# heihachi78/NascarGymnasium

Measured on AMD Instinct MI355X. Metric: env-steps/sec (cars x envs), daytona 10-car, higher is better.
Workload: dtype f32+f64; 1 GPU; daytona 10-car: 8192 envs x 10 cars per GPU, on-device noisy rule driver (BaseController._fallback_control, 15% of car-steps uniform), closed loop, steady state after 10800 settle steps (env ages staggered over the 180 s episode), auto-reset; envs_per_gpu=8192, cars_per_env=10, policy=noisy, car_contact=off (reference), track=daytona.track, parallelism=dp1 (env shards, no collective)

## Files before the change

include/nascar.h:

```cpp
#ifndef NASCAR_H
#define NASCAR_H
#include <stdint.h>
#ifdef __cplusplus
extern "C" {
#endif

typedef struct NascarHandle NascarHandle;

typedef struct NascarConfig {
    int32_t num_envs;
    int32_t num_cars;
    int32_t reset_on_lap;
    int32_t device;
    double start_x, start_y, start_angle;
} NascarConfig;

int nascar_create(const NascarConfig* cfg, NascarHandle** out);
void nascar_destroy(NascarHandle* h);
const char* nascar_last_error(void);

int nascar_add_track(NascarHandle* h, const double* segments, int32_t nseg, double total_length,
                     const double* walls, int32_t nwall);
int nascar_set_track_cache(int32_t retain, const char* dir);
int nascar_prebuild_track(const double* segments, int32_t nseg, double total_length, const double* walls, int32_t nwall,
                          float beam_cell);

int nascar_set_env_tracks(NascarHandle* h, const int32_t* env_track);

int nascar_set_random_tracks(NascarHandle* h, const int32_t* tracks, int32_t ntracks, const uint64_t* seeds,
                             const int32_t* draws, void* stream);
int nascar_get_env_tracks(NascarHandle* h, int32_t* env_track, int32_t* draws, void* stream);
int nascar_track_draw(int32_t n, const uint64_t* seeds, const int32_t* k, const int32_t* current, const int32_t* tracks,
                      int32_t ntracks, int32_t* out);

int nascar_vec_post(NascarHandle* h, const float* reward, const uint8_t* env_flags, double* ep_ret, int64_t* ep_len,
                    uint8_t* done, double* snap_ret, int64_t* snap_len, void* stream);
int nascar_check_actions(NascarHandle* h, const void* actions, int32_t discrete, int32_t* bad, void* stream);

int nascar_reset(NascarHandle* h, const uint8_t* env_mask, float* obs, void* stream);

int nascar_step(NascarHandle* h, const void* actions, int32_t discrete, float* obs, float* reward,
                uint8_t* car_flags, uint8_t* env_flags, int32_t auto_reset, float* terminal_obs, void* stream);

int nascar_step_driven(NascarHandle* h, int32_t policy, uint64_t seed, int64_t step, float* obs, float* reward,
                       uint8_t* car_flags, uint8_t* env_flags, int32_t auto_reset, float* terminal_obs, void* stream);

#define NASCAR_TRAJ_RECORDS 1
#define NASCAR_TRAJ_OBS 2
int nascar_rollout(NascarHandle* h, int32_t policy, uint64_t seed, int64_t step0, int32_t steps, float* obs,
                   float* reward, uint8_t* car_flags, uint8_t* env_flags, int32_t auto_reset, int32_t traj, void* stream);

int nascar_set_rollout_streams(NascarHandle* h, int32_t streams);
int nascar_get_rollout_streams(NascarHandle* h);

int nascar_set_rollout_pipe(NascarHandle* h, int32_t sensor_workgroups);
int nascar_rollout_pipe_status(NascarHandle* h, void* stream);

int nascar_set_envs_per_block(NascarHandle* h, int32_t epb);
int nascar_get_envs_per_block(NascarHandle* h);

int nascar_set_sensor_lanes(NascarHandle* h, int32_t lanes);

int nascar_set_sensor_block(NascarHandle* h, int32_t threads);

int nascar_set_beam_cell(NascarHandle* h, float meters);

int nascar_set_fused_logic(NascarHandle* h, int32_t enable);
int nascar_get_fused_logic(NascarHandle* h);

int nascar_set_step_events(NascarHandle* h, void* const* events, int32_t n);

int nascar_get_info(NascarHandle* h, double* info, void* stream);

int nascar_set_car_contact(NascarHandle* h, int32_t enable);

int nascar_set_car_visibility(NascarHandle* h, int32_t enable);
int nascar_get_car_visibility(NascarHandle* h);

int nascar_set_perf_history(NascarHandle* h, int32_t enable, void* stream);

int64_t nascar_state_bytes(NascarHandle* h);
int nascar_get_state(NascarHandle* h, void* dst_device, void* stream);
int nascar_set_state(NascarHandle* h, const void* src_device, void* stream);

int nascar_policy_actions(NascarHandle* h, int32_t policy, uint64_t seed, int64_t step, const float* obs,
                          float* actions, void* stream);

int nascar_set_actor(NascarHandle* h, const float* w1, const float* b1, const float* w2, const float* b2,
                     const float* w3, const float* b3, int32_t obs_dim, int32_t hidden, int32_t act_dim);
int nascar_set_actor_precision(NascarHandle* h, int32_t fp32);
int nascar_actor_forward(NascarHandle* h, const float* obs, int32_t n, float* actions, void* stream);

typedef struct NascarMlp {
    int32_t obs_dim, h1, h2, act_dim;
    int32_t activation;
    int32_t output;
    const float *w1, *b1, *w2, *b2, *w3, *b3;
} NascarMlp;
#define NASCAR_CTRL_RULE (-1)
#define NASCAR_CTRL_UNIFORM (-2)
#define NASCAR_CTRL_NOISY (-3)
#define NASCAR_CTRL_GENOME (-4)
int nascar_check_controller(const NascarMlp* mlp);
int nascar_add_controller(NascarHandle* h, const NascarMlp* mlp);
int nascar_controller_forward(NascarHandle* h, int32_t id, const float* obs, int32_t n, float* actions, void* stream);
int nascar_set_car_controllers(NascarHandle* h, const int32_t* ctrl);
int nascar_update_controller(NascarHandle* h, int32_t id, const NascarMlp* mlp, void* stream);

int nascar_set_actor_critic(NascarHandle* h, int32_t pi_id, int32_t vf_id, const float* log_std);
int nascar_collect(NascarHandle* h, uint64_t seed, int64_t step0, int32_t steps, float* obs, float* reward,
                   uint8_t* car_flags, uint8_t* env_flags, float* actions, float* logp, float* values, float* timeout_values,
                   void* stream);
int nascar_gae(NascarHandle* h, const float* reward, const float* values, const float* timeout_values,
               const uint8_t* env_flags, int32_t steps, double gamma, double lambda, float* adv, float* ret, void* stream);

typedef struct NascarReplay {
    float *obs, *next_obs;
    float *actions;
    float *reward;
    uint8_t *done, *timeout, *live;
    int32_t capacity;
} NascarReplay;
int nascar_set_explorer(NascarHandle* h, int32_t id, const float* sigma);
int nascar_collect_transitions(NascarHandle* h, int32_t source, uint64_t seed, int64_t step0, int32_t steps, float* obs,
                               const NascarReplay* replay, int32_t pos, void* stream);
int nascar_replay_sample(NascarHandle* h, const NascarReplay* replay, int32_t size, uint64_t seed, int64_t draw,
                         int32_t batch, float* obs, float* next_obs, float* actions, float* reward, float* done,
                         uint8_t* live, void* stream);

int nascar_set_genomes(NascarHandle* h, const double* genomes, void* stream);

int nascar_set_fitness(NascarHandle* h, int32_t enable, void* stream);
int nascar_get_fitness(NascarHandle* h, double* out, void* stream);

int nascar_debug_sincosf(const float* x, float* s, float* c, int32_t n, void* stream);

int nascar_debug_f64math(const double* x, const double* y, double* out, int32_t n, int32_t fn, void* stream);

int nascar_debug_toi(const float* cases, int32_t n, float* beta, int32_t* state, int32_t* far, void* stream);
int nascar_debug_collide(const float* cases, int32_t n, float* out, void* stream);

int nascar_debug_car_contact(const float* bodies, int32_t num_envs, int32_t num_cars, float* out, int32_t* env_out,
                             void* stream);

int nascar_debug_sensors(NascarHandle* h, const float* poses, float* obs, int32_t impl, void* stream);

int nascar_debug_block_map(NascarHandle* h, int32_t* blk_track, int32_t* blk_env, int32_t cap_blocks, void* stream);

#ifdef __cplusplus
}
#endif
#endif
```

nascargymnasium_amd/_lib.py:

```python
import ctypes
import os
import subprocess

HERE = os.path.dirname(os.path.abspath(__file__))
LIB_PATH = os.environ.get("NASCAR_LIB") or os.path.join(HERE, "libnascar.so")
CSRC = os.path.join(HERE, "csrc")

INFO_FIELDS = ["x", "y", "vx", "vy", "angle", "omega", "speed", "lap_count", "last_lap_time", "best_lap_time",
               "is_timing", "current_lap_time", "total_distance_traveled", "has_crossed_startline", "disabled",
               "cumulative_reward", "cumulative_impact_force", "on_track", "engine_rpm", "simulation_time",
               "n_contacts", "error", "track_progress", "perf_count", "perf_max_speed", "perf_first_fast"]
N_INFO = len(INFO_FIELDS)
INFO_INDEX = {f: i for i, f in enumerate(INFO_FIELDS)}
OBS_DIM = 38

CF_DISABLED, CF_JUST_DISABLED, CF_COLLISION, CF_LAP, CF_ERROR = 1, 2, 4, 8, 128
EF_TERMINATED, EF_TRUNCATED, EF_RESET = 1, 2, 8
TRAJ_RECORDS, TRAJ_OBS = 1, 2
REASONS = {0: None, 1: "all_cars_disabled", 2: "all_active_cars_low_reward (threshold: -250.0)",
           3: "time_limit", 4: "truncated"}

HIPCC_FLAGS = ["--offload-arch=gfx950", "-O3", "-ffp-contract=off", "-fno-fast-math", "-fno-slp-vectorize", "-fPIC",
               "-shared", "-std=c++17", "-Wno-unused-value", "-Wno-unused-result"]


class NascarMlp(ctypes.Structure):
    _fields_ = [(n, ctypes.c_int32) for n in ("obs_dim", "h1", "h2", "act_dim", "activation", "output")] + \
               [(n, ctypes.POINTER(ctypes.c_float)) for n in ("w1", "b1", "w2", "b2", "w3", "b3")]


CTRL_BUILTIN = {"rule": -1, "uniform": -2, "noisy": -3, "genome": -4}
FITNESS_FIELDS = ["total_reward", "distance_traveled", "max_speed", "time_on_track", "lap_completed", "lap_time",
                  "steps", "disabled_at_step"]
N_FITNESS = len(FITNESS_FIELDS)
N_GENES = 12


class NascarReplay(ctypes.Structure):
    _fields_ = [(n, ctypes.c_void_p) for n in ("obs", "next_obs", "actions", "reward", "done", "timeout", "live")] + \
               [("capacity", ctypes.c_int32)]


class NascarConfig(ctypes.Structure):
    _fields_ = [("num_envs", ctypes.c_int32), ("num_cars", ctypes.c_int32), ("reset_on_lap", ctypes.c_int32),
                ("device", ctypes.c_int32), ("start_x", ctypes.c_double), ("start_y", ctypes.c_double),
                ("start_angle", ctypes.c_double)]


def build(verbose=False):
    src = os.path.join(CSRC, "nascar_kernels.hip")
    cmd = ["hipcc"] + HIPCC_FLAGS + ["-o", LIB_PATH, src]
    r = subprocess.run(cmd, capture_output=True, text=True)
    if r.returncode != 0:
        raise RuntimeError("hipcc failed:\n" + r.stderr[-4000:])
    if verbose:
        print(" ".join(cmd))
    return LIB_PATH


_lib = None


def lib():
    global _lib
    if _lib is not None:
        return _lib
    if not os.path.exists(LIB_PATH):
        raise RuntimeError(f"{LIB_PATH} is missing: run `python -c 'import __graft_entry__ as g; g.build()'` "
                           "(there is no CPU fallback for the product path)")
    L = ctypes.CDLL(LIB_PATH)
    vp, i32, i64, u64 = ctypes.c_void_p, ctypes.c_int32, ctypes.c_int64, ctypes.c_uint64
    d_p = ctypes.POINTER(ctypes.c_double)
    L.nascar_create.argtypes = [ctypes.POINTER(NascarConfig), ctypes.POINTER(vp)]
    L.nascar_create.restype = ctypes.c_int
    L.nascar_destroy.argtypes = [vp]
    L.nascar_destroy.restype = None
    L.nascar_last_error.restype = ctypes.c_char_p
    L.nascar_add_track.argtypes = [vp, d_p, i32, ctypes.c_double, d_p, i32]
    L.nascar_add_track.restype = ctypes.c_int
    L.nascar_set_env_tracks.argtypes = [vp, ctypes.POINTER(i32)]
    L.nascar_set_env_tracks.restype = ctypes.c_int
    L.nascar_reset.argtypes = [vp, vp, vp, vp]
    L.nascar_reset.restype = ctypes.c_int
    L.nascar_step.argtypes = [vp, vp, i32, vp, vp, vp, vp, i32, vp, vp]
    L.nascar_step.restype = ctypes.c_int
    L.nascar_step_driven.argtypes = [vp, i32, u64, i64, vp, vp, vp, vp, i32, vp, vp]
    L.nascar_step_driven.restype = ctypes.c_int
    L.nascar_rollout.argtypes = [vp, i32, u64, i64, i32, vp, vp, vp, vp, i32, i32, vp]
    L.nascar_rollout.restype = ctypes.c_int
    L.nascar_set_car_contact.argtypes = [vp, i32]
    L.nascar_set_car_contact.restype = ctypes.c_int
    L.nascar_set_car_visibility.argtypes = [vp, i32]
    L.nascar_set_car_visibility.restype = ctypes.c_int
    L.nascar_get_car_visibility.argtypes = [vp]
    L.nascar_get_car_visibility.restype = ctypes.c_int
    L.nascar_set_rollout_streams.argtypes = [vp, i32]
    L.nascar_set_rollout_streams.restype = ctypes.c_int
    L.nascar_get_rollout_streams.argtypes = [vp]
    L.nascar_get_rollout_streams.restype = ctypes.c_int
    L.nascar_set_rollout_pipe.argtypes = [vp, i32]
    L.nascar_set_rollout_pipe.restype = ctypes.c_int
    L.nascar_rollout_pipe_status.argtypes = [vp, vp]
    L.nascar_rollout_pipe_status.restype = ctypes.c_int
    L.nascar_set_envs_per_block.argtypes = [vp, i32]
    L.nascar_set_envs_per_block.restype = ctypes.c_int
    L.nascar_get_envs_per_block.argtypes = [vp]
    L.nascar_get_envs_per_block.restype = ctypes.c_int
    L.nascar_set_sensor_lanes.argtypes = [vp, i32]
    L.nascar_set_sensor_lanes.restype = ctypes.c_int
    L.nascar_set_sensor_block.argtypes = [vp, i32]
    L.nascar_set_sensor_block.restype = ctypes.c_int
    L.nascar_set_beam_cell.argtypes = [vp, ctypes.c_float]
    L.nascar_set_beam_cell.restype = ctypes.c_int
    L.nascar_set_fused_logic.argtypes = [vp, i32]
    L.nascar_set_fused_logic.restype = ctypes.c_int
    L.nascar_get_fused_logic.argtypes = [vp]
    L.nascar_get_fused_logic.restype = ctypes.c_int
    L.nascar_set_perf_history.argtypes = [vp, i32, vp]
    L.nascar_set_perf_history.restype = ctypes.c_int
    L.nascar_get_info.argtypes = [vp, vp, vp]
    L.nascar_get_info.restype = ctypes.c_int
    L.nascar_state_bytes.argtypes = [vp]
    L.nascar_state_bytes.restype = i64
    L.nascar_get_state.argtypes = [vp, vp, vp]
    L.nascar_get_state.restype = ctypes.c_int
    L.nascar_set_state.argtypes = [vp, vp, vp]
    L.nascar_set_state.restype = ctypes.c_int
    L.nascar_policy_actions.argtypes = [vp, i32, u64, i64, vp, vp, vp]
    L.nascar_policy_actions.restype = ctypes.c_int
    fp = ctypes.POINTER(ctypes.c_float)
    L.nascar_set_actor.argtypes = [vp, fp, fp, fp, fp, fp, fp, i32, i32, i32]
    L.nascar_set_actor.restype = ctypes.c_int
    L.nascar_set_actor_precision.argtypes = [vp, i32]
    L.nascar_set_actor_precision.restype = ctypes.c_int
    L.nascar_actor_forward.argtypes = [vp, vp, i32, vp, vp]
    L.nascar_actor_forward.restype = ctypes.c_int
    L.nascar_check_controller.argtypes = [ctypes.POINTER(NascarMlp)]
    L.nascar_check_controller.restype = ctypes.c_int
    L.nascar_add_controller.argtypes = [vp, ctypes.POINTER(NascarMlp)]
    L.nascar_add_controller.restype = ctypes.c_int
    L.nascar_controller_forward.argtypes = [vp, i32, vp, i32, vp, vp]
    L.nascar_controller_forward.restype = ctypes.c_int
    L.nascar_set_car_controllers.argtypes = [vp, ctypes.POINTER(i32)]
    L.nascar_set_car_controllers.restype = ctypes.c_int
    L.nascar_update_controller.argtypes = [vp, i32, ctypes.POINTER(NascarMlp), vp]
    L.nascar_update_controller.restype = ctypes.c_int
    L.nascar_set_actor_critic.argtypes = [vp, i32, i32, fp]
    L.nascar_set_actor_critic.restype = ctypes.c_int
    L.nascar_collect.argtypes = [vp, u64, i64, i32, vp, vp, vp, vp, vp, vp, vp, vp, vp]
    L.nascar_collect.restype = ctypes.c_int
    L.nascar_gae.argtypes = [vp, vp, vp, vp, vp, i32, ctypes.c_double, ctypes.c_double, vp, vp, vp]
    L.nascar_gae.restype = ctypes.c_int
    L.nascar_set_explorer.argtypes = [vp, i32, fp]
    L.nascar_set_explorer.restype = ctypes.c_int
    L.nascar_collect_transitions.argtypes = [vp, i32, u64, i64, i32, vp, ctypes.POINTER(NascarReplay), i32, vp]
    L.nascar_collect_transitions.restype = ctypes.c_int
    L.nascar_replay_sample.argtypes = [vp, ctypes.POINTER(NascarReplay), i32, u64, i64, i32, vp, vp, vp, vp, vp, vp, vp]
    L.nascar_replay_sample.restype = ctypes.c_int
    L.nascar_set_genomes.argtypes = [vp, d_p, vp]
    L.nascar_set_genomes.restype = ctypes.c_int
    L.nascar_set_fitness.argtypes = [vp, i32, vp]
    L.nascar_set_fitness.restype = ctypes.c_int
    L.nascar_get_fitness.argtypes = [vp, vp, vp]
    L.nascar_get_fitness.restype = ctypes.c_int
    L.nascar_set_step_events.argtypes = [vp, ctypes.POINTER(vp), i32]
    L.nascar_set_step_events.restype = ctypes.c_int
    L.nascar_debug_sincosf.argtypes = [vp, vp, vp, i32, vp]
    L.nascar_debug_sincosf.restype = ctypes.c_int
    L.nascar_debug_f64math.argtypes = [vp, vp, vp, i32, i32, vp]
    L.nascar_debug_f64math.restype = ctypes.c_int
    L.nascar_debug_toi.argtypes = [vp, i32, vp, vp, vp, vp]
    L.nascar_debug_toi.restype = ctypes.c_int
    L.nascar_debug_collide.argtypes = [vp, i32, vp, vp]
    L.nascar_debug_collide.restype = ctypes.c_int
    L.nascar_debug_car_contact.argtypes = [vp, i32, i32, vp, vp, vp]
    L.nascar_debug_car_contact.restype = ctypes.c_int
    L.nascar_debug_sensors.argtypes = [vp, vp, vp, i32, vp]
    L.nascar_debug_sensors.restype = ctypes.c_int
    i32p, u64p = ctypes.POINTER(i32), ctypes.POINTER(u64)
    L.nascar_track_draw.argtypes = [i32, u64p, i32p, i32p, i32p, i32, i32p]
    L.nascar_track_draw.restype = ctypes.c_int
    L.nascar_set_random_tracks.argtypes = [vp, i32p, i32, u64p, i32p, vp]
    L.nascar_set_random_tracks.restype = ctypes.c_int
    L.nascar_get_env_tracks.argtypes = [vp, vp, vp, vp]
    L.nascar_get_env_tracks.restype = ctypes.c_int
    L.nascar_vec_post.argtypes = [vp, vp, vp, vp, vp, vp, vp, vp, vp]
    L.nascar_vec_post.restype = ctypes.c_int
    L.nascar_check_actions.argtypes = [vp, vp, i32, vp, vp]
    L.nascar_check_actions.restype = ctypes.c_int
    L.nascar_set_track_cache.argtypes = [i32, ctypes.c_char_p]
    L.nascar_set_track_cache.restype = ctypes.c_int
    L.nascar_prebuild_track.argtypes = [d_p, i32, ctypes.c_double, d_p, i32, ctypes.c_float]
    L.nascar_prebuild_track.restype = ctypes.c_int
    L.nascar_debug_block_map.argtypes = [vp, vp, vp, i32, vp]
    L.nascar_debug_block_map.restype = ctypes.c_int
    _lib = L
    set_track_cache(int(os.environ.get("NASCAR_TRACK_RETAIN", "8")), os.environ.get("NASCAR_TRACK_CACHE", ""))
    return L


EXPORTED = ["nascar_create", "nascar_destroy", "nascar_last_error", "nascar_add_track", "nascar_set_env_tracks",
            "nascar_reset", "nascar_step", "nascar_step_driven", "nascar_rollout", "nascar_get_info", "nascar_set_perf_history", "nascar_set_car_contact", "nascar_set_car_visibility", "nascar_get_car_visibility", "nascar_set_rollout_streams", "nascar_get_rollout_streams", "nascar_set_rollout_pipe", "nascar_rollout_pipe_status", "nascar_set_envs_per_block", "nascar_get_envs_per_block", "nascar_set_sensor_lanes", "nascar_set_sensor_block", "nascar_set_beam_cell", "nascar_set_fused_logic", "nascar_get_fused_logic", "nascar_state_bytes", "nascar_get_state",
            "nascar_set_state", "nascar_policy_actions", "nascar_set_step_events", "nascar_set_actor", "nascar_set_actor_precision", "nascar_actor_forward",
            "nascar_check_controller", "nascar_add_controller", "nascar_controller_forward", "nascar_set_car_controllers",
            "nascar_set_genomes", "nascar_set_fitness", "nascar_get_fitness",
            "nascar_update_controller", "nascar_set_actor_critic", "nascar_collect", "nascar_gae",
            "nascar_set_explorer", "nascar_collect_transitions", "nascar_replay_sample",
            "nascar_debug_sincosf", "nascar_debug_f64math", "nascar_debug_toi", "nascar_debug_collide", "nascar_debug_car_contact", "nascar_debug_sensors", "nascar_track_draw", "nascar_set_random_tracks",
            "nascar_get_env_tracks", "nascar_vec_post", "nascar_check_actions", "nascar_set_track_cache",
            "nascar_prebuild_track", "nascar_debug_block_map"]


def check(rc):
    if rc < 0:
        raise RuntimeError("libnascar: " + lib().nascar_last_error().decode())
    return rc


def mlp_struct(ctrl, output=None):
    import numpy as np
    arrs = [np.ascontiguousarray(a, np.float32) for a in ctrl.arrays]
    fp = ctypes.POINTER(ctypes.c_float)
    m = NascarMlp(38, int(ctrl.h1), int(ctrl.h2), int(arrs[4].shape[0]), int(ctrl.activation),
                  int(ctrl.output if output is None else output), *[a.ctypes.data_as(fp) for a in arrs])
    return m, arrs


def check_controller(ctrl):
    m, _keep = mlp_struct(ctrl)
    check(lib().nascar_check_controller(ctypes.byref(m)))


def track_draw(seeds, k, current, tracks):
    import numpy as np
    seeds = np.ascontiguousarray(seeds, np.uint64).ravel()
    n = seeds.size
    k = np.ascontiguousarray(np.broadcast_to(np.asarray(k, np.int32), (n,)))
    cur = np.ascontiguousarray(np.broadcast_to(np.asarray(current, np.int32), (n,)))
    tr = np.ascontiguousarray(tracks, np.int32)
    out = np.empty(n, np.int32)
    i32p, u64p = ctypes.POINTER(ctypes.c_int32), ctypes.POINTER(ctypes.c_uint64)
    check(lib().nascar_track_draw(n, seeds.ctypes.data_as(u64p), k.ctypes.data_as(i32p), cur.ctypes.data_as(i32p),
                                  tr.ctypes.data_as(i32p), tr.size, out.ctypes.data_as(i32p)))
    return out


def set_track_cache(retain=8, directory=""):
    check(lib().nascar_set_track_cache(int(retain), (directory or "").encode()))


def prebuild_track(path, beam_cell=1.0):
    import numpy as np
    from .track import build_walls, load_track, track_path
    t = load_track(track_path(path))
    seg = np.ascontiguousarray(t.segment_table())
    walls = np.ascontiguousarray(build_walls(t)[:, :4])
    dp = ctypes.POINTER(ctypes.c_double)
    return bool(check(lib().nascar_prebuild_track(seg.ctypes.data_as(dp), seg.shape[0], float(t.total_length),
                                                  walls.ctypes.data_as(dp), walls.shape[0], float(beam_cell))))
```

nascargymnasium_amd/csrc/nascar_car_io.h:

```cpp
#pragma once
#include "nascar_params.h"

enum {
  G_BODY = 1,
  G_IMP = 2,
  G_MODEL = 4,
  G_BANK = 8,
  G_TYRES = 16,
  G_ACC = 32,
  G_DIS = 64,
  G_LOGIC = 128,
  G_ALL = 255
};
#define CAR_F32_TABLE(X) \
  X(F32, cx, c.c.x, G_BODY) X(F32, cy, c.c.y, G_BODY) X(F32, a, c.a, G_BODY) \
  X(F32, vx, c.v.x, G_BODY) X(F32, vy, c.v.y, G_BODY) X(F32, w, c.w, G_BODY) \
  X(F32, qs, c.xf.q.s, G_BODY) X(F32, qc, c.xf.q.c, G_BODY) X(F32, xpx, c.xf.p.x, G_BODY) X(F32, xpy, c.xf.p.y, G_BODY) \
  X(F32, sleep, c.sleep, G_BODY) X(F32, invdt0, c.invdt0, G_BODY) \
  X(F32, flox, c.fat.lo.x, G_BODY) X(F32, floy, c.fat.lo.y, G_BODY) X(F32, fhix, c.fat.hi.x, G_BODY) X(F32, fhiy, c.fat.hi.y, G_BODY) \
  X(F32, cum_reward, c.cum_reward, G_LOGIC) X(F32, cum_reward_info, c.cum_reward_info, G_LOGIC)
#define CAR_F64_TABLE(X) \
  X(F64, rpm, c.rpm, G_MODEL) X(F64, pvx, c.pvx, G_MODEL) X(F64, pvy, c.pvy, G_MODEL) \
  X(F64, lfm, c.lfm, G_MODEL) X(F64, slip, c.slip, G_MODEL) X(F64, bank, c.bank, G_BANK) \
  X(F64, load0, c.load[0], G_TYRES) X(F64, load1, c.load[1], G_TYRES) X(F64, load2, c.load[2], G_TYRES) X(F64, load3, c.load[3], G_TYRES) \
  X(F64, temp0, c.temp[0], G_TYRES) X(F64, temp1, c.temp[1], G_TYRES) X(F64, temp2, c.temp[2], G_TYRES) X(F64, temp3, c.temp[3], G_TYRES) \
  X(F64, wear0, c.wear[0], G_TYRES) X(F64, wear1, c.wear[1], G_TYRES) X(F64, wear2, c.wear[2], G_TYRES) X(F64, wear3, c.wear[3], G_TYRES) \
  X(F64, imp, c.imp, G_IMP) \
  X(F64, lt_start, c.lt_start, G_LOGIC) X(F64, lt_cur, c.lt_cur, G_LOGIC) X(F64, lt_last, c.lt_last, G_LOGIC) \
  X(F64, lt_best, c.lt_best, G_LOGIC) X(F64, lt_px, c.lt_px, G_LOGIC) X(F64, lt_py, c.lt_py, G_LOGIC) X(F64, lt_dist, c.lt_dist, G_LOGIC) \
  X(F64, cum_impact, c.cum_impact, G_LOGIC) X(F64, stuck_dur, c.stuck_dur, G_LOGIC) \
  X(F64, stuck_sx, c.stuck_sx, G_LOGIC) X(F64, stuck_sy, c.stuck_sy, G_LOGIC) \
  X(F64, prev_px, c.prev_px, G_LOGIC) X(F64, prev_py, c.prev_py, G_LOGIC) \
  X(F64, prog_hist, c.prog_hist, G_LOGIC) X(F64, back, c.back, G_LOGIC) X(F64, prev_back, c.prev_back, G_LOGIC) \
  X(F64, imp_at_obs, c.imp_at_obs, G_LOGIC)
#define CAR_I32_TABLE(X) \
  X(I32, awake, c.awake, G_BODY) X(I32, nct, c.nct, G_BODY) X(I32, overflow, c.overflow, G_BODY) \
  X(I32, acc_len, c.acc_len, G_ACC) X(I32, acc_head, c.acc_head, G_ACC) \
  X(I32, imp_present, c.imp_present, G_IMP) X(I32, nact, c.nact, G_BODY) \
  X(I32, lt_timing, c.lt_timing, G_LOGIC) X(I32, lt_has_last, c.lt_has_last, G_LOGIC) X(I32, lt_has_best, c.lt_has_best, G_LOGIC) \
  X(I32, lt_crossed, c.lt_crossed, G_LOGIC) X(I32, lt_has_pos, c.lt_has_pos, G_LOGIC) X(I32, lt_laps, c.lt_laps, G_LOGIC) \
  X(I32, disabled, c.disabled, G_DIS) X(I32, has_stuck_start, c.has_stuck_start, G_LOGIC) \
  X(I32, first_step, c.first_step, G_LOGIC) X(I32, prev_laps, c.prev_laps, G_LOGIC)

#define CAR_ROW_ENUM(T, f, m, g) CAR_ROW_##T##_##f,
#define CAR_ROW_CHECK(T, f, m, g) \
  static_assert((int)CAR_ROW_##T##_##f == (int)T##_##f, "car field table: row " #f " is not at its nascar_layout.h index");
enum { CAR_F32_TABLE(CAR_ROW_ENUM) CAR_ROWS_F32 };
enum { CAR_F64_TABLE(CAR_ROW_ENUM) CAR_ROWS_F64 };
enum { CAR_I32_TABLE(CAR_ROW_ENUM) CAR_ROWS_I32 };
CAR_F32_TABLE(CAR_ROW_CHECK) CAR_F64_TABLE(CAR_ROW_CHECK) CAR_I32_TABLE(CAR_ROW_CHECK)
static_assert((int)CAR_ROWS_F32 == (int)N_F32 && (int)CAR_ROWS_F64 == (int)N_F64 && (int)CAR_ROWS_I32 == (int)N_I32,
              "car field table: row count differs from nascar_layout.h");

template <int MASK>
__device__ __forceinline__ void car_load_groups(const Params& P, int n, Car& c) {
#define CAR_ROW_LOAD(T, f, m, g) if (MASK & (g)) m = T##P(P, f)[n];
  CAR_F32_TABLE(CAR_ROW_LOAD) CAR_F64_TABLE(CAR_ROW_LOAD) CAR_I32_TABLE(CAR_ROW_LOAD)
#undef CAR_ROW_LOAD
}
template <int MASK>
__device__ __forceinline__ void car_store_groups(const Params& P, int n, const Car& c) {
#define CAR_ROW_STORE(T, f, m, g) if (MASK & (g)) T##P(P, f)[n] = m;
  CAR_F32_TABLE(CAR_ROW_STORE) CAR_F64_TABLE(CAR_ROW_STORE) CAR_I32_TABLE(CAR_ROW_STORE)
#undef CAR_ROW_STORE
}
__device__ __forceinline__ void car_init_step(const Params& P, int n, Car& c) {
  c.just_disabled = 0;
  c.force = zero2(); c.torque = 0.0f; c.c0 = c.c; c.a0 = c.a; c.alpha0 = 0.0f; c.moved = 0;
  c.ct = P.ct + (size_t)n * MAXC; c.act_key = P.act_key + (size_t)n * MAXC; c.act_n = P.act_n + (size_t)n * MAXC * 2;
  c.acc = nullptr;
}

__device__ inline void car_load(const Params& P, int n, Car& c) { car_load_groups<G_ALL>(P, n, c); car_init_step(P, n, c); }
__device__ inline void car_store(const Params& P, int n, const Car& c) { car_store_groups<G_ALL>(P, n, c); }

__device__ inline void car_load_phys(const Params& P, int n, Car& c) {
  car_load_groups<G_BODY | G_IMP | G_MODEL | G_BANK | G_TYRES | G_ACC | G_DIS>(P, n, c);
  car_init_step(P, n, c);
}
__device__ inline void car_store_model(const Params& P, int n, const Car& c) { car_store_groups<G_MODEL | G_TYRES | G_ACC>(P, n, c); }
__device__ inline void car_reload_tyres(const Params& P, int n, Car& c) { car_load_groups<G_TYRES>(P, n, c); }
__device__ inline void car_load_logic(const Params& P, int n, Car& c) { car_load_groups<G_LOGIC>(P, n, c); }

__device__ inline void car_store_body(const Params& P, int n, const Car& c) { car_store_groups<G_BODY | G_IMP>(P, n, c); }
__device__ inline void car_load_body(const Params& P, int n, Car& c) {
  car_load_groups<G_BODY | G_IMP | G_DIS>(P, n, c);
  car_init_step(P, n, c);
}
__device__ inline void car_store_logic(const Params& P, int n, const Car& c) {
  car_store_groups<G_LOGIC | G_BANK | G_IMP | G_DIS>(P, n, c);
}
```

nascargymnasium_amd/csrc/nascar_device.h:

```cpp
#pragma once
#include "nascar_math.h"
#include "nascar_layout.h"

#pragma clang fp contract(off)

#define BLOCK 256
#define SBLOCK 128

#ifdef NASCAR_PROFILE
__device__ unsigned long long* g_prof = nullptr;
__shared__ int s_prof_b0;
#define PROF_B0(v) (s_prof_b0 = (v))
#define PROF_BLK ((size_t)((blockIdx.x + (unsigned)s_prof_b0) & 16383u))
#define PROF(ph) do { unsigned long long _t = __builtin_amdgcn_s_memtime(); \
    if (g_prof && (threadIdx.x & 63) == 0) g_prof[(PROF_BLK * (BLOCK / 64) + threadIdx.x / 64) * 16 + (ph)] = _t; } while (0)
#define PROFS(ph) do { unsigned long long _t = __builtin_amdgcn_s_memtime(); \
    if (g_prof && (threadIdx.x & 63) == 0) g_prof[(65536 + PROF_BLK * (BLOCK / 64) + threadIdx.x / 64) * 16 + (ph)] = _t; } while (0)
#define PROFR(ph) do { unsigned long long _t = __builtin_amdgcn_s_memtime(); \
    if (g_prof && (threadIdx.x & 63) == 0) g_prof[(65536 + PROF_BLK * (blockDim.x >> 6) + threadIdx.x / 64) * 16 + (ph)] = _t; } while (0)
#define PROF_XCC(ph) do { const unsigned long long _x = (__builtin_amdgcn_s_getreg((3 << 11) | 20) & 15) + 1; \
    if (g_prof && (threadIdx.x & 63) == 0) g_prof[(PROF_BLK * (BLOCK / 64) + threadIdx.x / 64) * 16 + (ph)] = _x; } while (0)
#define PROFR_XCC(ph) do { const unsigned long long _x = (__builtin_amdgcn_s_getreg((3 << 11) | 20) & 15) + 1; \
    if (g_prof && (threadIdx.x & 63) == 0) g_prof[(65536 + PROF_BLK * (blockDim.x >> 6) + threadIdx.x / 64) * 16 + (ph)] = _x; } while (0)
#define PROFR_RT(ph) do { unsigned long long _t = __builtin_amdgcn_s_memrealtime(); \
// ... 65 lines not shown
#define MAX_TRANSLATION 2.0f
#define MAX_ROTATION (0.5f * B2_PI)
#define BAUMGARTE 0.2f
#define TOI_BAUMGARTE 0.75f
#define MAX_LINEAR_CORRECTION 0.2f
#define VELOCITY_THRESHOLD 1.0f
#define TIME_TO_SLEEP 0.5f
#define LINEAR_SLEEP_TOL 0.01f
#define ANGULAR_SLEEP_TOL (2.0f / 180.0f * B2_PI)
#define MAX_SUBSTEPS 8
#define MAX_TOI_CONTACTS 32
#define FLT_EPS 1.1920928955078125e-07f
#define FLT_BIG 3.402823466e+38f

#define CAR_HX ((float)(5.042 / 2.0))
#define CAR_HY ((float)(1.996 / 2.0))
#define CAR_INV_MASS (1.0f / 1500.0f)
#define CAR_I_F ((float)(1500.0 * (5.042 * 5.042 + 1.996 * 1.996) * 0.5 / 12.0))
#define CAR_INV_I (1.0f / CAR_I_F)
#define MIX_RESTITUTION 0.25f

#define CAR_MASS 1500.0
#define GRAVITY_MS2 9.81
#define CAR_WHEELBASE 2.794
#define CAR_MAX_TORQUE 820.0
#define CAR_MAX_POWER (670.0 * 745.7)
#define CAR_MAX_SPEED_MS (200.0 * 0.44704)
#define DRAG_CONSTANT (0.5 * 1.225 * 0.38 * 2.5)
#define ROLLING_RESISTANCE_FORCE (0.015 * CAR_MASS * GRAVITY_MS2)
#define MAX_TYRE_LOAD (CAR_MASS * GRAVITY_MS2 * 2.0)
#define STATIC_LOAD_PER_TYRE (CAR_MASS * GRAVITY_MS2 / 4.0)
#define PI_D 3.141592653589793
#define RAD_PER_DEG (PI_D / 180.0)
#define DEG_PER_RAD (180.0 / PI_D)

typedef unsigned int gu4 __attribute__((ext_vector_type(4)));
typedef unsigned int gu2 __attribute__((ext_vector_type(2)));
template <typename T> __device__ __forceinline__ T ldg(const T* p) {
  if constexpr (sizeof(T) % 16 == 0) {
    T r;
    const __attribute__((address_space(1))) gu4* q = (const __attribute__((address_space(1))) gu4*)p;
#pragma unroll
    for (int i = 0; i < (int)(sizeof(T) / 16); ++i) { const gu4 v = q[i]; __builtin_memcpy((char*)&r + 16 * i, &v, 16); }
    return r;
  } else if constexpr (sizeof(T) % 8 == 0) {
    T r;
    const __attribute__((address_space(1))) gu2* q = (const __attribute__((address_space(1))) gu2*)p;
#pragma unroll
    for (int i = 0; i < (int)(sizeof(T) / 8); ++i) { const gu2 v = q[i]; __builtin_memcpy((char*)&r + 8 * i, &v, 8); }
    return r;
  } else {
    return *(const __attribute__((address_space(1))) T*)p;
  }
}

struct V2 { float x, y; };
struct Rot { float s, c; };
struct Xf { V2 p; Rot q; };
struct Aabb { V2 lo, hi; };

__device__ __forceinline__ V2 V(float x, float y) { V2 r; r.x = x; r.y = y; return r; }
__device__ __forceinline__ V2 vadd(V2 a, V2 b) { return V(a.x + b.x, a.y + b.y); }
__device__ __forceinline__ V2 vsub(V2 a, V2 b) { return V(a.x - b.x, a.y - b.y); }
__device__ __forceinline__ V2 vmul(float s, V2 a) { return V(s * a.x, s * a.y); }
__device__ __forceinline__ V2 vneg(V2 a) { return V(-a.x, -a.y); }
__device__ __forceinline__ float vdot(V2 a, V2 b) { return a.x * b.x + a.y * b.y; }
__device__ __forceinline__ float vcross(V2 a, V2 b) { return a.x * b.y - a.y * b.x; }
__device__ __forceinline__ V2 vcross_vs(V2 a, float s) { return V(s * a.y, -s * a.x); }
__device__ __forceinline__ V2 vcross_sv(float s, V2 a) { return V(-s * a.y, s * a.x); }
__device__ __forceinline__ float vlen(V2 a) { return fsqrt_cr(a.x * a.x + a.y * a.y); }
__device__ __forceinline__ float vnormalize(V2* a) {
  float length = vlen(*a);
  if (length < FLT_EPS) return 0.0f;
  float inv = fdiv_cr(1.0f, length);
  a->x *= inv; a->y *= inv;
  return length;
}
__device__ __forceinline__ V2 rmul(Rot q, V2 v) { return V(q.c * v.x - q.s * v.y, q.s * v.x + q.c * v.y); }
__device__ __forceinline__ V2 rmulT(Rot q, V2 v) { return V(q.c * v.x + q.s * v.y, -q.s * v.x + q.c * v.y); }
__device__ __forceinline__ V2 xmul(Xf T, V2 v) {
  return V((T.q.c * v.x - T.q.s * v.y) + T.p.x, (T.q.s * v.x + T.q.c * v.y) + T.p.y);
}
__device__ __forceinline__ V2 xmulT(Xf T, V2 v) {
  float px = v.x - T.p.x, py = v.y - T.p.y;
  return V(T.q.c * px + T.q.s * py, -T.q.s * px + T.q.c * py);
}
__device__ __forceinline__ Xf xmulT_xx(Xf A, Xf B) {
  Xf C;
  C.q.s = A.q.c * B.q.s - A.q.s * B.q.c;
  C.q.c = A.q.c * B.q.c + A.q.s * B.q.s;
  C.p = rmulT(A.q, vsub(B.p, A.p));
  return C;
}
__device__ __forceinline__ float fminb(float a, float b) { return a < b ? a : b; }
__device__ __forceinline__ float fmaxb(float a, float b) { return a > b ? a : b; }
__device__ __forceinline__ float fclamp(float a, float lo, float hi) { return fmaxb(lo, fminb(a, hi)); }
__device__ __forceinline__ V2 vmin(V2 a, V2 b) { return V(fminb(a.x, b.x), fminb(a.y, b.y)); }
__device__ __forceinline__ V2 vmax(V2 a, V2 b) { return V(fmaxb(a.x, b.x), fmaxb(a.y, b.y)); }
__device__ __forceinline__ Rot rot_set(float a) { Rot q; glibc_sincosf(a, &q.s, &q.c); return q; }
__device__ __forceinline__ V2 zero2() { return V(0.0f, 0.0f); }

struct Poly { float hx, hy, radius; };
__device__ __forceinline__ void make_box(Poly* p, float hx, float hy) { p->hx = hx; p->hy = hy; p->radius = POLY_RADIUS; }
__device__ __forceinline__ float with_sign(float m, uint32_t neg) { return __uint_as_float(__float_as_uint(m) | (neg << 31)); }
__device__ __forceinline__ V2 pv(const Poly* p, int i) {
  const uint32_t u = (uint32_t)i;
  return V(with_sign(p->hx, (((u + 1u) >> 1) & 1u) ^ 1u), with_sign(p->hy, ((u >> 1) & 1u) ^ 1u));
}
__device__ __forceinline__ V2 pn(const Poly* p, int i) {
  const uint32_t u = (uint32_t)i, odd = u & 1u, hi = (u >> 1) & 1u;
  return V(with_sign((float)odd, hi & odd), with_sign((float)(odd ^ 1u), (hi ^ 1u) & (odd ^ 1u)));
}
__device__ __forceinline__ Aabb poly_aabb(const Poly* p, Xf xf) {
  V2 lower = xmul(xf, pv(p, 0)), upper = lower;
#pragma unroll
  for (int i = 1; i < 4; ++i) { V2 v = xmul(xf, pv(p, i)); lower = vmin(lower, v); upper = vmax(upper, v); }
  V2 r = V(p->radius, p->radius);
  Aabb a; a.lo = vsub(lower, r); a.hi = vadd(upper, r);
  return a;
}
__device__ __forceinline__ bool overlap(Aabb a, Aabb b) {
  V2 d1 = vsub(b.lo, a.hi), d2 = vsub(a.lo, b.hi);
  if (d1.x > 0.0f || d1.y > 0.0f) return false;
  if (d2.x > 0.0f || d2.y > 0.0f) return false;
  return true;
}
__device__ __forceinline__ bool contains(Aabb a, Aabb b) {
  bool r = true;
  r = r && a.lo.x <= b.lo.x; r = r && a.lo.y <= b.lo.y;
  r = r && b.hi.x <= a.hi.x; r = r && b.hi.y <= a.hi.y;
  return r;
}

struct LWall {
  float px, py, qs, qc;
  float hx, hy, ang;
  int key;
};
__device__ __forceinline__ Xf wall_xf(const LWall& w) { Xf t; t.p = V(w.px, w.py); t.q.s = w.qs; t.q.c = w.qc; return t; }
__device__ __forceinline__ Aabb fat_box(float4 f) { Aabb a; a.lo = V(f.x, f.y); a.hi = V(f.z, f.w); return a; }

struct WallGrid {
  float ox, oy, inv_cell, reach;
  int nx, ny;
  const int* start;
  const uint16_t* idx;
  const float4* box;
};
#define BP_BATCH 4
struct WallSet {
  const LWall* W; int nw;
  WallGrid bp, sn;
  const float4* fat;
  DContact* ct_all = nullptr;
};

__device__ __forceinline__ bool grid_list(const WallGrid& g, float x, float y, int& beg, int& end) {
  if (!g.start) return false;
  const float fx = (x - g.ox) * g.inv_cell, fy = (y - g.oy) * g.inv_cell;
  if (!(fx >= 0.0f && fy >= 0.0f && fx < (float)g.nx && fy < (float)g.ny)) return false;
  const int cell = (int)fy * g.nx + (int)fx;
  beg = ldg(g.start + cell); end = ldg(g.start + cell + 1);
  return true;
}

struct Car {
  V2 c; float a; V2 v; float w; Xf xf; float sleep; int awake;
  V2 force; float torque; V2 c0; float a0; float alpha0;
  Aabb fat; int moved; float invdt0;
  int nct, overflow;
  int pid;
  double thr_in, brk_in, str_in, thr, brk, steer;
  double rpm, pvx, pvy, lfm, slip, bank;
  double load[4], temp[4], wear[4], fric[4];
  int acc_len, acc_head;
  int imp_present, nact; double imp;
  int lt_timing, lt_has_last, lt_has_best, lt_crossed, lt_has_pos, lt_laps;
  double lt_start, lt_cur, lt_last, lt_best, lt_px, lt_py, lt_dist;
  int disabled, just_disabled, has_stuck_start, first_step, prev_laps;
  double cum_impact, stuck_dur, stuck_sx, stuck_sy, prev_px, prev_py, prog_hist, back, prev_back, imp_at_obs;
  float cum_reward, cum_reward_info;
  DContact* ct;
  int ct_hw;
  int* act_key;
  float* act_n;
  double* acc;
};

#ifndef CT_LDS_CAP
#define CT_LDS_CAP 4
#endif
__device__ __forceinline__ bool ct_in_lds(const Car& c) {
  return __builtin_amdgcn_is_shared((const __attribute__((address_space(0))) void*)c.ct);
}
__device__ __forceinline__ void ct_make_room(Car& c, const WallSet& S) {
  if (S.ct_all && ct_in_lds(c)) {
    if (c.nct >= CT_LDS_CAP) {
      DContact* g = S.ct_all + (size_t)c.pid * MAXC;
      const int nrec = max(c.nct, c.ct_hw);
      for (int i = 0; i < nrec; ++i) g[i] = c.ct[i];
      c.ct = g;
    } else {
      c.ct_hw = max(c.ct_hw, c.nct + 1);
    }
  }
}

__device__ inline void lis_begin(Car& c, int key, V2 n) {
  int found = -1;
  for (int i = 0; i < c.nact; ++i) if (c.act_key[i] == key) { found = i; break; }
  if (found >= 0) { c.act_n[found * 2] = n.x; c.act_n[found * 2 + 1] = n.y; }
  else if (c.nact < MAXC) { c.act_key[c.nact] = key; c.act_n[c.nact * 2] = n.x; c.act_n[c.nact * 2 + 1] = n.y; c.nact++; }
  if (!c.imp_present) { c.imp_present = 1; c.imp = 0.0; }
}
__device__ inline void lis_end(Car& c, int key) {
  for (int i = 0; i < c.nact; ++i) if (c.act_key[i] == key) {
    for (int j = i; j < c.nact - 1; ++j) { c.act_key[j] = c.act_key[j + 1]; c.act_n[j * 2] = c.act_n[j * 2 + 2]; c.act_n[j * 2 + 1] = c.act_n[j * 2 + 3]; }
    c.nact--; break;
  }
  if (c.nact == 0) { c.imp_present = 1; c.imp = 0.0; }
}
__device__ inline void lis_post(Car& c, int count, float n0, float n1) {
  if (count <= 0) return;
  double total = 0.0;
  total += (double)n0;
  if (count > 1) total += (double)n1;
  if (c.imp_present) c.imp = pymax(c.imp, total);
}

__device__ __forceinline__ void set_awake(Car& c) { if (!c.awake) { c.awake = 1; c.sleep = 0.0f; } }
__device__ __forceinline__ void sync_transform(Car& c) { c.xf.q = rot_set(c.a); c.xf.p = vsub(c.c, rmul(c.xf.q, zero2())); }
__device__ __forceinline__ void apply_force(Car& c, V2 f, V2 point) {
  set_awake(c); c.force = vadd(c.force, f); c.torque += vcross(vsub(point, c.c), f);
}
__device__ __forceinline__ void apply_force_center(Car& c, V2 f) { set_awake(c); c.force = vadd(c.force, f); }
__device__ __forceinline__ void apply_torque(Car& c, float t) { set_awake(c); c.torque += t; }

__device__ __forceinline__ void move_proxy(Car& c, Xf xf1, Xf xf2) {
  Poly cp; make_box(&cp, CAR_HX, CAR_HY);
  Aabb a1 = poly_aabb(&cp, xf1), a2 = poly_aabb(&cp, xf2), aabb;
  aabb.lo = vmin(a1.lo, a2.lo); aabb.hi = vmax(a1.hi, a2.hi);
  V2 disp = vsub(xf2.p, xf1.p);
  if (contains(c.fat, aabb)) return;
  Aabb b = aabb; V2 r = V(AABB_EXT, AABB_EXT);
  b.lo = vsub(b.lo, r); b.hi = vadd(b.hi, r);
  V2 d = vmul(AABB_MULT, disp);
  if (d.x < 0.0f) b.lo.x += d.x; else b.hi.x += d.x;
  if (d.y < 0.0f) b.lo.y += d.y; else b.hi.y += d.y;
  c.fat = b; c.moved = 1;
}
__device__ __forceinline__ void sync_fixtures(Car& c) {
  Xf xf1; xf1.q = rot_set(c.a0); xf1.p = vsub(c.c0, rmul(xf1.q, zero2()));
  move_proxy(c, xf1, c.xf);
}

__device__ inline void add_pair(Car& c, const WallSet& S, int j) {
    bool exists = false;
    for (int i = 0; i < c.nct; ++i) if (c.ct[i].wall == j) { exists = true; break; }
    if (exists) return;
    if (c.nct >= MAXC) { c.overflow = 1; return; }
    ct_make_room(c, S);
    for (int i = c.nct; i > 0; --i) c.ct[i] = c.ct[i - 1];
    DContact z;
    z.wall = j; z.flags = CT_ENABLED; z.mtype = 0; z.pointCount = 0;
    z.lnx = z.lny = z.lpx = z.lpy = 0.0f;
    for (int q = 0; q < 2; ++q) { z.pt[q].lx = z.pt[q].ly = z.pt[q].ni = z.pt[q].ti = 0.0f; z.pt[q].id = 0u; }
    z.toi = 1.0f; z.toiCount = 0;
    c.ct[0] = z;
    c.nct++;
    set_awake(c);
}
__device__ inline void find_new_contacts(Car& c, const WallSet& S) {
  if (!c.moved) return;
  c.moved = 0;
  const LWall* W = S.W;
  int beg = 0, end = S.nw;
  const uint16_t* list = nullptr;
  {
    const float hx = 0.5f * (c.fat.hi.x - c.fat.lo.x), hy = 0.5f * (c.fat.hi.y - c.fat.lo.y);
    const float cx = 0.5f * (c.fat.hi.x + c.fat.lo.x), cy = 0.5f * (c.fat.hi.y + c.fat.lo.y);
    if (hx <= S.bp.reach - 0.05f && hy <= S.bp.reach - 0.05f && grid_list(S.bp, cx, cy, beg, end)) list = S.bp.idx;
    else { beg = 0; end = S.nw; CCOUNT(c, 8, 1); }
  }
  if (list && S.bp.box) {
    const float4* __restrict__ box = S.bp.box;
    for (int k = beg; k < end; k += BP_BATCH) {
      float4 b[BP_BATCH];
#pragma unroll
      for (int u = 0; u < BP_BATCH; ++u) b[u] = ldg(box + k + u);
#pragma unroll
      for (int u = 0; u < BP_BATCH; ++u) {
        if (k + u >= end) break;
        Aabb a; a.lo = V(b[u].x, b[u].y); a.hi = V(b[u].z, b[u].w);
        if (overlap(c.fat, a)) add_pair(c, S, (int)ldg(list + k + u));
      }
    }
    return;
  }
  for (int k = beg; k < end; ++k) {
    const int j = list ? (int)ldg(list + k) : k;
    if (!overlap(c.fat, fat_box(ldg(S.fat + j)))) continue;
    bool exists = false;
    for (int i = 0; i < c.nct; ++i) if (c.ct[i].wall == j) { exists = true; break; }
    if (exists) continue;
    if (c.nct >= MAXC) { c.overflow = 1; continue; }
    ct_make_room(c, S);
    for (int i = c.nct; i > 0; --i) c.ct[i] = c.ct[i - 1];
    DContact z;
    z.wall = j; z.flags = CT_ENABLED; z.mtype = 0; z.pointCount = 0;
    z.lnx = z.lny = z.lpx = z.lpy = 0.0f;
    for (int q = 0; q < 2; ++q) { z.pt[q].lx = z.pt[q].ly = z.pt[q].ni = z.pt[q].ti = 0.0f; z.pt[q].id = 0u; }
    z.toi = 1.0f; z.toiCount = 0;
    c.ct[0] = z;
    c.nct++;
    set_awake(c);
  }
}
__device__ inline void remove_contact(Car& c, int i) {
  for (int j = i; j < c.nct - 1; ++j) c.ct[j] = c.ct[j + 1];
  c.nct--;
}

struct Clip { V2 v; uint32_t id; };
__device__ __forceinline__ uint32_t cf_key(int ia, int ib, int ta, int tb) {
  return (uint32_t)(ia & 255) | ((uint32_t)(ib & 255) << 8) | ((uint32_t)(ta & 255) << 16) | ((uint32_t)(tb & 255) << 24);
}
__device__ inline float find_max_separation(int* edgeIndex, const Poly* p1, Xf xf1, const Poly* p2, Xf xf2) {
  Xf xf = xmulT_xx(xf2, xf1);
  int best = 0; float maxSep = -FLT_BIG;
  for (int i = 0; i < 4; ++i) {
    V2 n = rmul(xf.q, pn(p1, i));
    V2 v1 = xmul(xf, pv(p1, i));
    float si = FLT_BIG;
    for (int j = 0; j < 4; ++j) { float sij = vdot(n, vsub(pv(p2, j), v1)); if (sij < si) si = sij; }
    if (si > maxSep) { maxSep = si; best = i; }
  }
  *edgeIndex = best;
  return maxSep;
}
__device__ inline void find_incident_edge(Clip& c0, Clip& c1, const Poly* p1, Xf xf1, int edge1, const Poly* p2, Xf xf2) {
  V2 normal1 = rmulT(xf2.q, rmul(xf1.q, pn(p1, edge1)));
  int index = 0; float minDot = FLT_BIG;
  for (int i = 0; i < 4; ++i) { float d = vdot(normal1, pn(p2, i)); if (d < minDot) { minDot = d; index = i; } }
  int i1 = index, i2 = i1 + 1 < 4 ? i1 + 1 : 0;
  c0.v = xmul(xf2, pv(p2, i1)); c0.id = cf_key(edge1, i1, 1, 0);
  c1.v = xmul(xf2, pv(p2, i2)); c1.id = cf_key(edge1, i2, 1, 0);
}
__device__ inline int clip_segment(Clip& o0, Clip& o1, const Clip& i0, const Clip& i1, V2 normal, float offset, int vertexIndexA) {
  int numOut = 0;
  float d0 = vdot(normal, i0.v) - offset;
  float d1 = vdot(normal, i1.v) - offset;
  if (d0 <= 0.0f) { o0 = i0; numOut = 1; }
  if (d1 <= 0.0f) { if (numOut == 0) o0 = i1; else o1 = i1; ++numOut; }
  if (d0 * d1 < 0.0f) {
    float interp = fdiv_cr(d0, d0 - d1);
    Clip cv;
    cv.v = vadd(i0.v, vmul(interp, vsub(i1.v, i0.v)));
    cv.id = cf_key(vertexIndexA, (int)((i0.id >> 8) & 255), 0, 1);
    if (numOut == 0) o0 = cv; else o1 = cv;
    ++numOut;
  }
  return numOut;
}
__device__ inline void collide_polygons(DContact& m, const Poly* pA, Xf xfA, const Poly* pB, Xf xfB) {
  m.pointCount = 0;
  float totalRadius = pA->radius + pB->radius;
  int edgeA = 0; float sepA = find_max_separation(&edgeA, pA, xfA, pB, xfB);
  if (sepA > totalRadius) return;
  int edgeB = 0; float sepB = find_max_separation(&edgeB, pB, xfB, pA, xfA);
  if (sepB > totalRadius) return;
  const Poly *poly1, *poly2; Xf xf1, xf2; int edge1; int flip;
  const float k_tol = 0.1f * LINEAR_SLOP;
  if (sepB > sepA + k_tol) { poly1 = pB; poly2 = pA; xf1 = xfB; xf2 = xfA; edge1 = edgeB; m.mtype = 2; flip = 1; }
  else { poly1 = pA; poly2 = pB; xf1 = xfA; xf2 = xfB; edge1 = edgeA; m.mtype = 1; flip = 0; }
  Clip inc0, inc1;
  find_incident_edge(inc0, inc1, poly1, xf1, edge1, poly2, xf2);
  int iv1 = edge1, iv2 = edge1 + 1 < 4 ? edge1 + 1 : 0;
  V2 v11 = pv(poly1, iv1), v12 = pv(poly1, iv2);
  V2 localTangent = vsub(v12, v11);
  vnormalize(&localTangent);
  V2 localNormal = vcross_vs(localTangent, 1.0f);
  V2 planePoint = vmul(0.5f, vadd(v11, v12));
  V2 tangent = rmul(xf1.q, localTangent);
  V2 normal = vcross_vs(tangent, 1.0f);
  v11 = xmul(xf1, v11); v12 = xmul(xf1, v12);
  float frontOffset = vdot(normal, v11);
  float sideOffset1 = -vdot(tangent, v11) + totalRadius;
  float sideOffset2 = vdot(tangent, v12) + totalRadius;
  Clip a0, a1, b0, b1;
  int np = clip_segment(a0, a1, inc0, inc1, vneg(tangent), sideOffset1, iv1);
  if (np < 2) return;
  np = clip_segment(b0, b1, a0, a1, tangent, sideOffset2, iv2);
  if (np < 2) return;
  m.lnx = localNormal.x; m.lny = localNormal.y; m.lpx = planePoint.x; m.lpy = planePoint.y;
  int pc = 0;
#pragma unroll
  for (int i = 0; i < 2; ++i) {
    const Clip& cq = i == 0 ? b0 : b1;
    float separation = vdot(normal, cq.v) - frontOffset;
    if (separation <= totalRadius) {
      V2 lp = xmulT(xf2, cq.v);
      uint32_t id = cq.id;
      if (flip) {
        uint32_t ia = id & 255, ib = (id >> 8) & 255, ta = (id >> 16) & 255, tb = (id >> 24) & 255;
        id = cf_key((int)ib, (int)ia, (int)tb, (int)ta);
      }
      DPoint q; q.lx = lp.x; q.ly = lp.y; q.id = id; q.ni = 0.0f; q.ti = 0.0f;
      if (pc == 0) m.pt[0] = q; else m.pt[1] = q;
      ++pc;
    }
  }
  m.pointCount = pc;
}

__device__ inline void world_manifold(const DContact& m, Xf xfA, Xf xfB, V2* normal, V2 pts[2]) {
  const float rA = POLY_RADIUS, rB = POLY_RADIUS;
  if (m.pointCount == 0) return;
  V2 ln = V(m.lnx, m.lny), lp = V(m.lpx, m.lpy);
  if (m.mtype == 1) {
    V2 n = rmul(xfA.q, ln), planePoint = xmul(xfA, lp);
#pragma unroll
    for (int i = 0; i < 2; ++i) {
      if (i >= m.pointCount) break;
      V2 clipPoint = xmul(xfB, V(m.pt[i].lx, m.pt[i].ly));
      V2 cA = vadd(clipPoint, vmul(rA - vdot(vsub(clipPoint, planePoint), n), n));
      V2 cB = vsub(clipPoint, vmul(rB, n));
      pts[i] = vmul(0.5f, vadd(cA, cB));
    }
    *normal = n;
  } else {
    V2 n = rmul(xfB.q, ln), planePoint = xmul(xfB, lp);
#pragma unroll
    for (int i = 0; i < 2; ++i) {
      if (i >= m.pointCount) break;
      V2 clipPoint = xmul(xfA, V(m.pt[i].lx, m.pt[i].ly));
      V2 cB = vadd(clipPoint, vmul(rB - vdot(vsub(clipPoint, planePoint), n), n));
      V2 cA = vsub(clipPoint, vmul(rA, n));
      pts[i] = vmul(0.5f, vadd(cA, cB));
    }
    *normal = vneg(n);
  }
}

__device__ inline void contact_update(Car& c, int ci, const LWall* W) {
  PCOUNT(14, 1); CCOUNT(c, 5, 1);
  DContact ct = c.ct[ci];
  const DContact old = ct;
  ct.flags |= CT_ENABLED;
  bool was = (ct.flags & CT_TOUCH) != 0;
  Poly pa, pb; make_box(&pa, CAR_HX, CAR_HY);
  const LWall wl = ldg(W + ct.wall);
  make_box(&pb, wl.hx, wl.hy);
  Xf xfB = wall_xf(wl);
  collide_polygons(ct, &pa, c.xf, &pb, xfB);
  bool touching = ct.pointCount > 0;
#pragma unroll
  for (int i = 0; i < 2; ++i) {
    if (i >= ct.pointCount) break;
    ct.pt[i].ni = 0.0f; ct.pt[i].ti = 0.0f;
    if (old.pointCount > 0 && old.pt[0].id == ct.pt[i].id) { ct.pt[i].ni = old.pt[0].ni; ct.pt[i].ti = old.pt[0].ti; }
    else if (old.pointCount > 1 && old.pt[1].id == ct.pt[i].id) { ct.pt[i].ni = old.pt[1].ni; ct.pt[i].ti = old.pt[1].ti; }
  }
  if (touching != was) set_awake(c);
  if (touching) ct.flags |= CT_TOUCH; else ct.flags &= ~CT_TOUCH;
  c.ct[ci] = ct;
  if (!was && touching) {
    V2 n = zero2(), pts[2];
    world_manifold(ct, c.xf, xfB, &n, pts);
    lis_begin(c, wl.key, n);
  }
  if (was && !touching) lis_end(c, wl.key);
}

struct ManiRes { float4 a, b, c; };
#define MANI_UNSET 0x7fc0deadu
__device__ inline ManiRes contact_manifold(Xf xfA, const LWall& wl) {
  Poly pa, pb; make_box(&pa, CAR_HX, CAR_HY); make_box(&pb, wl.hx, wl.hy);
  DContact m;
  m.mtype = -1; m.lnx = __uint_as_float(MANI_UNSET); m.pointCount = 0;
  m.lny = m.lpx = m.lpy = 0.0f;
  for (int q = 0; q < 2; ++q) { m.pt[q].lx = m.pt[q].ly = 0.0f; m.pt[q].id = 0u; }
  collide_polygons(m, &pa, xfA, &pb, wall_xf(wl));
  const int stage = __float_as_uint(m.lnx) != MANI_UNSET ? 2 : (m.mtype >= 0 ? 1 : 0);
  ManiRes r;
  r.a = make_float4(__int_as_float(stage | (m.pointCount << 2) | ((m.mtype & 3) << 4)), m.lnx, m.lny, m.lpx);
  r.b = make_float4(m.lpy, m.pt[0].lx, m.pt[0].ly, __uint_as_float(m.pt[0].id));
  r.c = make_float4(m.pt[1].lx, m.pt[1].ly, __uint_as_float(m.pt[1].id), 0.0f);
  return r;
}
__device__ inline void contact_apply(Car& c, int ci, const LWall* W, const ManiRes& r) {
  PCOUNT(14, 1); CCOUNT(c, 5, 1);
  DContact ct = c.ct[ci];
  const DContact old = ct;
  ct.flags |= CT_ENABLED;
  bool was = (ct.flags & CT_TOUCH) != 0;
  const int h = __float_as_int(r.a.x), stage = h & 3, pc = (h >> 2) & 3;
  ct.pointCount = 0;
  if (stage >= 1) ct.mtype = (h >> 4) & 3;
  if (stage == 2) {
    ct.lnx = r.a.y; ct.lny = r.a.z; ct.lpx = r.a.w; ct.lpy = r.b.x;
    if (pc > 0) { ct.pt[0].lx = r.b.y; ct.pt[0].ly = r.b.z; ct.pt[0].id = __float_as_uint(r.b.w); ct.pt[0].ni = 0.0f; ct.pt[0].ti = 0.0f; }
    if (pc > 1) { ct.pt[1].lx = r.c.x; ct.pt[1].ly = r.c.y; ct.pt[1].id = __float_as_uint(r.c.z); ct.pt[1].ni = 0.0f; ct.pt[1].ti = 0.0f; }
    ct.pointCount = pc;
  }
  bool touching = ct.pointCount > 0;
#pragma unroll
  for (int i = 0; i < 2; ++i) {
    if (i >= ct.pointCount) break;
    ct.pt[i].ni = 0.0f; ct.pt[i].ti = 0.0f;
    if (old.pointCount > 0 && old.pt[0].id == ct.pt[i].id) { ct.pt[i].ni = old.pt[0].ni; ct.pt[i].ti = old.pt[0].ti; }
    else if (old.pointCount > 1 && old.pt[1].id == ct.pt[i].id) { ct.pt[i].ni = old.pt[1].ni; ct.pt[i].ti = old.pt[1].ti; }
  }
  if (touching != was) set_awake(c);
  if (touching) ct.flags |= CT_TOUCH; else ct.flags &= ~CT_TOUCH;
  c.ct[ci] = ct;
  if (!was && touching) {
    const LWall wl = ldg(W + ct.wall);
    V2 n = zero2(), pts[2];
    world_manifold(ct, c.xf, wall_xf(wl), &n, pts);
    lis_begin(c, wl.key, n);
  }
  if (was && !touching) lis_end(c, ldg(&W[ct.wall].key));
}

#ifndef TOI_JOBCAP
#define TOI_JOBCAP 64
#endif
struct ToiWaveLDS { float4 sw0[64], sw1[64]; int2 job[TOI_JOBCAP]; float res[TOI_JOBCAP]; };
#ifndef MANI_JOBCAP
#define MANI_JOBCAP 32
#endif
struct ManiWaveLDS { float4 xf[64]; int2 job[MANI_JOBCAP]; ManiRes res[MANI_JOBCAP]; };
struct VCP { V2 rA, rB; float ni, ti, nm, tm, vb; };
struct VC {
  VCP p[2]; V2 normal; float nm[4]; float K[4]; int pointCount;
  V2 cB; float aB; V2 vB; float wB;
  V2 ln, lp, lps[2]; int pcount, type, ci;
  Rot qB; uint32_t aB0;
};
struct IslandWaveLDS { VC vc[MAX_ISLAND]; };
union WaveLDS { ToiWaveLDS toi; ManiWaveLDS mani; IslandWaveLDS island; float4 floor[160]; };
static_assert(sizeof(IslandWaveLDS) <= sizeof(ToiWaveLDS), "the island area must not grow the wave's LDS work area");
__shared__ WaveLDS g_wave_lds[SBLOCK / 64];
__device__ __forceinline__ void wave_lds_sync() {
  __builtin_amdgcn_fence(__ATOMIC_RELEASE, "wavefront");
  __builtin_amdgcn_wave_barrier();
  __builtin_amdgcn_fence(__ATOMIC_ACQUIRE, "wavefront");
}
__device__ __forceinline__ int popc64(unsigned long long x) { return __popcll(x); }
__device__ __forceinline__ int rank_in(unsigned long long m) {
  const unsigned long long below = __lane_id() == 0 ? 0ull : (~0ull >> (64 - __lane_id()));
  return popc64(m & below);
}

__device__ inline void collide(Car& c, const WallSet& S) {
  const LWall* W = S.W;
  int i = 0;
  while (i < c.nct) {
    if (!c.awake) { ++i; continue; }
    const int wall = c.ct[i].wall;
    if (!overlap(c.fat, fat_box(ldg(S.fat + wall)))) {
      bool touching = (c.ct[i].flags & CT_TOUCH) != 0;
      remove_contact(c, i);
      if (touching) lis_end(c, ldg(&W[wall].key));
      continue;
    }
    contact_update(c, i, W);
    ++i;
  }
}

__device__ __forceinline__ Rot rot_static(float a, uint32_t a0bits, Rot q0) {
  return __float_as_uint(a) == a0bits ? q0 : rot_set(a);
}
struct BodyState { V2 c; float a; V2 v; float w; };
#define UNROLL_SMALL NMAX <= 2 ? NMAX : 1
#define SOLVER_ITER_LOOP _Pragma("unroll 1")

template <int NMAX> __device__ __forceinline__ void cs_init(VC* vc, int n, const Car& c, const int* cidx, const LWall* W, bool warm, float dtRatio) {
#pragma unroll UNROLL_SMALL
  for (int i = 0; i < NMAX; ++i) {
    if (i >= n) break;
    const DContact& ct = c.ct[cidx[i]];
    VC& v = vc[i];
    v.ci = cidx[i];
    v.pointCount = ct.pointCount;
    const LWall wl = ldg(W + ct.wall);
    v.cB = V(wl.px, wl.py); v.aB = wl.ang; v.vB = zero2(); v.wB = 0.0f;
    v.qB.s = wl.qs; v.qB.c = wl.qc; v.aB0 = __float_as_uint(wl.ang);
    v.ln = V(ct.lnx, ct.lny); v.lp = V(ct.lpx, ct.lpy); v.pcount = ct.pointCount; v.type = ct.mtype;
    v.K[0] = v.K[1] = v.K[2] = v.K[3] = 0.0f; v.nm[0] = v.nm[1] = v.nm[2] = v.nm[3] = 0.0f;
    for (int j = 0; j < 2; ++j) {
      v.p[j].ni = v.p[j].ti = 0.0f;
      v.p[j].rA = v.p[j].rB = zero2(); v.p[j].nm = v.p[j].tm = v.p[j].vb = 0.0f;
      v.lps[j] = zero2();
    }
    for (int j = 0; j < 2; ++j) {
      if (j >= ct.pointCount) break;
      if (warm) { v.p[j].ni = dtRatio * ct.pt[j].ni; v.p[j].ti = dtRatio * ct.pt[j].ti; }
      v.lps[j] = V(ct.pt[j].lx, ct.pt[j].ly);
    }
  }
}

template <int NMAX> __device__ __forceinline__ void cs_init_velocity(VC* vc, int n, const Car& c, const BodyState& A) {
  const float mA = CAR_INV_MASS, iA = CAR_INV_I, mB = 0.0f, iB = 0.0f;
  const float friction_unused = 0.0f; (void)friction_unused;
  const Rot qA = rot_set(A.a);
#pragma unroll UNROLL_SMALL
  for (int i = 0; i < NMAX; ++i) {
    if (i >= n) break;
    VC& v = vc[i];
    const DContact& m = c.ct[v.ci];
    V2 cA = A.c; float aA = A.a; V2 vA = A.v; float wA = A.w;
    V2 cB = v.cB; float aB = v.aB; V2 vB = v.vB; float wB = v.wB;
    Xf xfA, xfB;
    xfA.q = qA; xfB.q = rot_static(aB, v.aB0, v.qB);
    xfA.p = vsub(cA, rmul(xfA.q, zero2()));
    xfB.p = vsub(cB, rmul(xfB.q, zero2()));
    V2 normal = zero2(), pts[2];
    world_manifold(m, xfA, xfB, &normal, pts);
    v.normal = normal;
    for (int j = 0; j < 2; ++j) {
      if (j >= v.pointCount) break;
      VCP& p = v.p[j];
      p.rA = vsub(pts[j], cA); p.rB = vsub(pts[j], cB);
      float rnA = vcross(p.rA, v.normal), rnB = vcross(p.rB, v.normal);
      float kNormal = mA + mB + iA * rnA * rnA + iB * rnB * rnB;
      p.nm = kNormal > 0.0f ? fdiv_cr(1.0f, kNormal) : 0.0f;
      V2 tangent = vcross_vs(v.normal, 1.0f);
      float rtA = vcross(p.rA, tangent), rtB = vcross(p.rB, tangent);
      float kTangent = mA + mB + iA * rtA * rtA + iB * rtB * rtB;
      p.tm = kTangent > 0.0f ? fdiv_cr(1.0f, kTangent) : 0.0f;
      p.vb = 0.0f;
      float vRel = vdot(v.normal, vsub(vsub(vadd(vB, vcross_sv(wB, p.rB)), vA), vcross_sv(wA, p.rA)));
      if (vRel < -VELOCITY_THRESHOLD) p.vb = -MIX_RESTITUTION * vRel;
    }
    if (v.pointCount == 2) {
      VCP& p1 = v.p[0]; VCP& p2 = v.p[1];
      float rn1A = vcross(p1.rA, v.normal), rn1B = vcross(p1.rB, v.normal);
      float rn2A = vcross(p2.rA, v.normal), rn2B = vcross(p2.rB, v.normal);
      float k11 = mA + mB + iA * rn1A * rn1A + iB * rn1B * rn1B;
      float k22 = mA + mB + iA * rn2A * rn2A + iB * rn2B * rn2B;
      float k12 = mA + mB + iA * rn1A * rn2A + iB * rn1B * rn2B;
      if (k11 * k11 < 1000.0f * (k11 * k22 - k12 * k12)) {
        v.K[0] = k11; v.K[1] = k12; v.K[2] = k12; v.K[3] = k22;
        float a = v.K[0], b = v.K[2], cc = v.K[1], d = v.K[3];
        float det = a * d - b * cc;
        if (det != 0.0f) det = fdiv_cr(1.0f, det);
        v.nm[0] = det * d; v.nm[2] = -det * b; v.nm[1] = -det * cc; v.nm[3] = det * a;
      } else {
        v.pointCount = 1;
      }
    }
  }
}

template <int NMAX> __device__ __forceinline__ void cs_warm_start(VC* vc, int n, BodyState& A) {
  const float mA = CAR_INV_MASS, iA = CAR_INV_I, mB = 0.0f, iB = 0.0f;
#pragma unroll UNROLL_SMALL
  for (int i = 0; i < NMAX; ++i) {
    if (i >= n) break;
    VC& v = vc[i];
    V2 vA = A.v; float wA = A.w; V2 vB = v.vB; float wB = v.wB;
    V2 normal = v.normal, tangent = vcross_vs(normal, 1.0f);
    for (int j = 0; j < 2; ++j) {
      if (j >= v.pointCount) break;
      VCP& p = v.p[j];
      V2 P = vadd(vmul(p.ni, normal), vmul(p.ti, tangent));
      wA -= iA * vcross(p.rA, P);
      vA = vsub(vA, vmul(mA, P));
      wB += iB * vcross(p.rB, P);
      vB = vadd(vB, vmul(mB, P));
    }
    A.v = vA; A.w = wA; v.vB = vB; v.wB = wB;
  }
}

__device__ __forceinline__ V2 rel_vel(V2 vA, float wA, V2 vB, float wB, const VCP& p) {
  return vsub(vsub(vadd(vB, vcross_sv(wB, p.rB)), vA), vcross_sv(wA, p.rA));
}

template <int NMAX> __device__ __forceinline__ void cs_solve_velocity(VC* vc, int n, BodyState& A, float friction) {
  const float mA = CAR_INV_MASS, iA = CAR_INV_I, mB = 0.0f, iB = 0.0f;
#pragma unroll UNROLL_SMALL
  for (int i = 0; i < NMAX; ++i) {
    if (i >= n) break;
    VC& v = vc[i];
    V2 vA = A.v; float wA = A.w; V2 vB = v.vB; float wB = v.wB;
    V2 normal = v.normal, tangent = vcross_vs(normal, 1.0f);
    for (int j = 0; j < 2; ++j) {
      if (j >= v.pointCount) break;
      VCP& p = v.p[j];
      V2 dv = rel_vel(vA, wA, vB, wB, p);
      float vt = vdot(dv, tangent) - 0.0f;
      float lambda = p.tm * (-vt);
      float maxFriction = friction * p.ni;
      float newImpulse = fclamp(p.ti + lambda, -maxFriction, maxFriction);
      lambda = newImpulse - p.ti;
      p.ti = newImpulse;
      V2 P = vmul(lambda, tangent);
      vA = vsub(vA, vmul(mA, P)); wA -= iA * vcross(p.rA, P);
      vB = vadd(vB, vmul(mB, P)); wB += iB * vcross(p.rB, P);
    }
    if (v.pointCount == 1) {
      VCP& p = v.p[0];
      V2 dv = rel_vel(vA, wA, vB, wB, p);
      float vn = vdot(dv, normal);
      float lambda = -p.nm * (vn - p.vb);
      float newImpulse = fmaxb(p.ni + lambda, 0.0f);
      lambda = newImpulse - p.ni;
      p.ni = newImpulse;
      V2 P = vmul(lambda, normal);
      vA = vsub(vA, vmul(mA, P)); wA -= iA * vcross(p.rA, P);
      vB = vadd(vB, vmul(mB, P)); wB += iB * vcross(p.rB, P);
    } else {
      VCP& cp1 = v.p[0]; VCP& cp2 = v.p[1];
      V2 a = V(cp1.ni, cp2.ni);
      V2 dv1 = rel_vel(vA, wA, vB, wB, cp1), dv2 = rel_vel(vA, wA, vB, wB, cp2);
      float vn1 = vdot(dv1, normal), vn2 = vdot(dv2, normal);
      V2 b = V(vn1 - cp1.vb, vn2 - cp2.vb);
      V2 Ka = V(v.K[0] * a.x + v.K[2] * a.y, v.K[1] * a.x + v.K[3] * a.y);
      b = vsub(b, Ka);
      V2 x;
      bool ok = false;
      x = vneg(V(v.nm[0] * b.x + v.nm[2] * b.y, v.nm[1] * b.x + v.nm[3] * b.y));
      if (x.x >= 0.0f && x.y >= 0.0f) ok = true;
      if (!ok) {
        x.x = -cp1.nm * b.x; x.y = 0.0f;
        vn2 = v.K[1] * x.x + b.y;
        if (x.x >= 0.0f && vn2 >= 0.0f) ok = true;
      }
      if (!ok) {
        x.x = 0.0f; x.y = -cp2.nm * b.y;
        vn1 = v.K[2] * x.y + b.x;
        if (x.y >= 0.0f && vn1 >= 0.0f) ok = true;
      }
      if (!ok) {
        x.x = 0.0f; x.y = 0.0f; vn1 = b.x; vn2 = b.y;
        if (vn1 >= 0.0f && vn2 >= 0.0f) ok = true;
      }
      if (ok) {
        V2 d = vsub(x, a);
        V2 P1 = vmul(d.x, normal), P2 = vmul(d.y, normal);
        vA = vsub(vA, vmul(mA, vadd(P1, P2)));
        wA -= iA * (vcross(cp1.rA, P1) + vcross(cp2.rA, P2));
        vB = vadd(vB, vmul(mB, vadd(P1, P2)));
        wB += iB * (vcross(cp1.rB, P1) + vcross(cp2.rB, P2));
        cp1.ni = x.x; cp2.ni = x.y;
      }
    }
    A.v = vA; A.w = wA; v.vB = vB; v.wB = wB;
  }
}

template <int NMAX> __device__ __forceinline__ void cs_store(const VC* vc, int n, Car& c) {
#pragma unroll UNROLL_SMALL
  for (int i = 0; i < NMAX; ++i) {
    if (i >= n) break;
    DContact& m = c.ct[vc[i].ci];
    for (int j = 0; j < 2; ++j) {
      if (j >= vc[i].pointCount) break; m.pt[j].ni = vc[i].p[j].ni; m.pt[j].ti = vc[i].p[j].ti; }
  }
}

struct RotCache { uint32_t bits; Rot q; };
__device__ __forceinline__ Rot rot_cached(RotCache& rc, float a) {
  if (__float_as_uint(a) != rc.bits) { rc.bits = __float_as_uint(a); rc.q = rot_set(a); }
  return rc.q;
}
template <int NMAX> __device__ __forceinline__ int cs_solve_position(VC* vc, int n, BodyState& A, int toi, RotCache& rcA) {
  float minSep = 0.0f;
  const float mA = CAR_INV_MASS, iA = CAR_INV_I, mB = 0.0f, iB = 0.0f;
#pragma unroll UNROLL_SMALL
  for (int i = 0; i < NMAX; ++i) {
    if (i >= n) break;
    VC& v = vc[i];
    V2 cA = A.c; float aA = A.a; V2 cB = v.cB; float aB = v.aB;
    for (int j = 0; j < 2; ++j) {
      if (j >= v.pcount) break;
      Xf xfA, xfB;
      xfA.q = rot_cached(rcA, aA); xfB.q = rot_static(aB, v.aB0, v.qB);
      xfA.p = vsub(cA, rmul(xfA.q, zero2()));
      xfB.p = vsub(cB, rmul(xfB.q, zero2()));
      V2 normal, point; float sep;
      if (v.type == 1) {
        V2 nn = rmul(xfA.q, v.ln), planePoint = xmul(xfA, v.lp), clipPoint = xmul(xfB, v.lps[j]);
        sep = vdot(vsub(clipPoint, planePoint), nn) - POLY_RADIUS - POLY_RADIUS;
        point = clipPoint; normal = nn;
      } else {
        V2 nn = rmul(xfB.q, v.ln), planePoint = xmul(xfB, v.lp), clipPoint = xmul(xfA, v.lps[j]);
        sep = vdot(vsub(clipPoint, planePoint), nn) - POLY_RADIUS - POLY_RADIUS;
        point = clipPoint; normal = vneg(nn);
      }
      V2 rA = vsub(point, cA), rB = vsub(point, cB);
      minSep = fminb(minSep, sep);
      float C = fclamp((toi ? TOI_BAUMGARTE : BAUMGARTE) * (sep + LINEAR_SLOP), -MAX_LINEAR_CORRECTION, 0.0f);
      float rnA = vcross(rA, normal), rnB = vcross(rB, normal);
      float K = mA + mB + iA * rnA * rnA + iB * rnB * rnB;
      float impulse = K > 0.0f ? fdiv_cr(-C, K) : 0.0f;
      V2 P = vmul(impulse, normal);
      cA = vsub(cA, vmul(mA, P)); aA -= iA * vcross(rA, P);
      cB = vadd(cB, vmul(mB, P)); aB += iB * vcross(rB, P);
    }
    A.c = cA; A.a = aA; v.cB = cB; v.aB = aB;
  }
  return toi ? (minSep >= -1.5f * LINEAR_SLOP) : (minSep >= -3.0f * LINEAR_SLOP);
}

template <int NMAX> __device__ __forceinline__ void report(Car& c, const VC* vc, int n) {
#pragma unroll UNROLL_SMALL
  for (int i = 0; i < NMAX; ++i) {
    if (i >= n) break;
    lis_post(c, vc[i].pointCount, vc[i].p[0].ni, vc[i].p[1].ni);
  }
}

__device__ inline void integrate_positions(BodyState& A, float h) {
  V2 cc = A.c; float a = A.a; V2 v = A.v; float w = A.w;
  V2 translation = vmul(h, v);
  if (vdot(translation, translation) > MAX_TRANSLATION * MAX_TRANSLATION) {
    float ratio = fdiv_cr(MAX_TRANSLATION, vlen(translation));
    v = vmul(ratio, v);
  }
  float rotation = h * w;
  if (rotation * rotation > MAX_ROTATION * MAX_ROTATION) {
    float ratio = fdiv_cr(MAX_ROTATION, fabsf(rotation));
    w *= ratio;
  }
  cc = vadd(cc, vmul(h, v));
  a += h * w;
  A.c = cc; A.a = a; A.v = v; A.w = w;
}

__device__ __forceinline__ void island_push(int cidx[MAX_ISLAND], int& n, int i) {
#pragma unroll
  for (int j = 0; j < MAX_ISLAND; ++j) cidx[j] = j == n ? i : cidx[j];
  ++n;
}
template <int NMAX>
__device__ __forceinline__ int solve_island_buf(Car& c, const LWall* W, const int* cidx, int n, float dt, float dtRatio,
                                                float friction, VC* vc) {
  float h = dt;
  BodyState A;
  c.c0 = c.c; c.a0 = c.a;
  {
    V2 v = c.v; float wv = c.w;
    V2 g = vadd(vmul(1.0f, zero2()), vmul(CAR_INV_MASS, c.force));
    v = vadd(v, vmul(h, g));
    wv += h * CAR_INV_I * c.torque;
    A.c = c.c; A.a = c.a; A.v = v; A.w = wv;
  }
  cs_init<NMAX>(vc, n, c, cidx, W, true, dtRatio);
  cs_init_velocity<NMAX>(vc, n, c, A);
  cs_warm_start<NMAX>(vc, n, A);
  SOLVER_ITER_LOOP
  for (int it = 0; it < 6; ++it) cs_solve_velocity<NMAX>(vc, n, A, friction);
  cs_store<NMAX>(vc, n, c);
  integrate_positions(A, h);
  int positionSolved = 0;
  RotCache rcA; rcA.bits = __float_as_uint(A.a) ^ 1u; rcA.q.s = 0.0f; rcA.q.c = 1.0f;
  SOLVER_ITER_LOOP
  for (int it = 0; it < 4; ++it) { if (cs_solve_position<NMAX>(vc, n, A, 0, rcA)) { positionSolved = 1; break; } }
  c.c = A.c; c.a = A.a; c.v = A.v; c.w = A.w;
  c.xf.q = rot_cached(rcA, c.a); c.xf.p = vsub(c.c, rmul(c.xf.q, zero2()));
  report<NMAX>(c, vc, n);
  return positionSolved;
}
template <int NMAX>
__device__ __forceinline__ int solve_island(Car& c, const LWall* W, const int* cidx, int n, float dt, float dtRatio,
                                            float friction) {
  VC vc[NMAX];
  return solve_island_buf<NMAX>(c, W, cidx, n, dt, dtRatio, friction, vc);
}
template <typename F>
__device__ __forceinline__ void wave_lds_one_at_a_time(F&& body) {
  unsigned long long pending = __ballot(1);
  wave_lds_sync();
  while (pending) {
    const int leader = __ffsll((long long)pending) - 1;
    if ((int)__lane_id() == leader) body((VC*)g_wave_lds[threadIdx.x >> 6].island.vc);
    pending &= pending - 1;
    wave_lds_sync();
  }
}
__device__ __forceinline__ int solve_island_general(Car& c, const LWall* W, const int* cidx, int n, float dt,
                                                   float dtRatio, float friction) {
  int r = 0;
  wave_lds_one_at_a_time([&](VC* vc) { r = solve_island_buf<MAX_ISLAND>(c, W, cidx, n, dt, dtRatio, friction, vc); });
  return r;
}

__device__ inline void solve(Car& c, const WallSet& S, float dt, float dtRatio, float friction) {
  const LWall* W = S.W;
  if (!c.awake) return;
  int cidx[MAX_ISLAND] = {0, 0, 0, 0, 0, 0, 0, 0}; int n = 0;
  for (int i = 0; i < c.nct; ++i) {
    int fl = c.ct[i].flags;
    if (!(fl & CT_ENABLED) || !(fl & CT_TOUCH)) continue;
    if (n == MAX_ISLAND) { c.overflow = 2; break; }
    island_push(cidx, n, i);
  }
  const float h = dt;
  CCOUNT(c, 26, n);
  CTIME_BEGIN();
  const int positionSolved = n <= 2 ? solve_island<2>(c, W, cidx, n, dt, dtRatio, friction)
                                  : solve_island_general(c, W, cidx, n, dt, dtRatio, friction);
  CTIME_END(c, 25);
  {
    float minSleepTime = FLT_BIG;
    const float linTolSqr = LINEAR_SLEEP_TOL * LINEAR_SLEEP_TOL;
    const float angTolSqr = ANGULAR_SLEEP_TOL * ANGULAR_SLEEP_TOL;
    if (c.w * c.w > angTolSqr || vdot(c.v, c.v) > linTolSqr) { c.sleep = 0.0f; minSleepTime = 0.0f; }
    else { c.sleep += h; minSleepTime = fminb(minSleepTime, c.sleep); }
    if (minSleepTime >= TIME_TO_SLEEP && positionSolved) {
      c.awake = 0; c.sleep = 0.0f; c.v = zero2(); c.w = 0.0f; c.force = zero2(); c.torque = 0.0f;
    }
  }
  PROFB(12);
  {
  CTIME_BEGIN();
  sync_fixtures(c);
  CTIME_END(c, 22);
  }
  {
  CTIME_BEGIN();
  if (c.moved) CCOUNT(c, 24, 1);
  find_new_contacts(c, S);
  CTIME_END(c, 21);
  }
}

struct SCache { float metric; int count; int iA0, iA1, iA2, iB0, iB1, iB2;
#ifdef NASCAR_PROFILE
  int iters = 0;
#endif
};

__device__ __forceinline__ int support(const Poly* p, V2 d) {
  const float a = p->hx * d.x, b = p->hy * d.y;
  const float v1 = a + (-b), v2 = a + b, v3 = (-a) + b;
  int best = 0; float bestValue = (-a) + (-b);
  if (v1 > bestValue) { best = 1; bestValue = v1; }
  if (v2 > bestValue) { best = 2; bestValue = v2; }
  if (v3 > bestValue) { best = 3; }
  return best;
}
__device__ __forceinline__ V2 gjk_w(int ip, const Poly* pA, Xf tA, const Poly* pB, Xf tB) {
  return vsub(xmul(tB, pv(pB, ip >> 2)), xmul(tA, pv(pA, ip & 3)));
}
__device__ inline float gjk_distance(SCache& cache, const Poly* pA, Xf tA, const Poly* pB, Xf tB) {
  V2 w0 = zero2(), w1 = zero2(), w2 = zero2();
  int i0 = 0, i1 = 0, i2 = 0;
  float a0 = 0.0f, a1 = 0.0f, a2 = 0.0f;
  int count = cache.count;
  if (count > 0) { i0 = cache.iA0 | (cache.iB0 << 2); w0 = gjk_w(i0, pA, tA, pB, tB); }
  if (count > 1) { i1 = cache.iA1 | (cache.iB1 << 2); w1 = gjk_w(i1, pA, tA, pB, tB); }
  if (count > 2) { i2 = cache.iA2 | (cache.iB2 << 2); w2 = gjk_w(i2, pA, tA, pB, tB); }
  if (count > 1) {
    const float metric1 = cache.metric;
    const float metric2 = count == 2 ? vlen(vsub(w0, w1)) : (count == 3 ? vcross(vsub(w1, w0), vsub(w2, w0)) : 0.0f);
    if (metric2 < 0.5f * metric1 || 2.0f * metric1 < metric2 || metric2 < FLT_EPS) count = 0;
  }
  if (count == 0) { i0 = 0; w0 = gjk_w(0, pA, tA, pB, tB); a0 = 1.0f; count = 1; }
  int iter = 0;
  while (iter < 20) {
    const int saveCount = count, s0 = i0, s1 = i1, s2 = i2;
    if (count == 2) {
      const V2 e12 = vsub(w1, w0);
      const float d12_2 = -vdot(w0, e12), d12_1 = vdot(w1, e12);
      const bool c1 = d12_2 <= 0.0f, c2 = !c1 && d12_1 <= 0.0f, c3 = !c1 && !c2;
      const float inv = fdiv_cr(1.0f, c3 ? d12_1 + d12_2 : 1.0f);
      if (c2) { w0 = w1; i0 = i1; }
      a0 = c3 ? d12_1 * inv : 1.0f;
      a1 = c3 ? d12_2 * inv : (c2 ? 1.0f : a1);
      count = c3 ? 2 : 1;
    } else if (count == 3) {
      const V2 e12 = vsub(w1, w0);
      const float d12_1 = vdot(w1, e12), d12_2 = -vdot(w0, e12);
      const V2 e13 = vsub(w2, w0);
      const float d13_1 = vdot(w2, e13), d13_2 = -vdot(w0, e13);
      const V2 e23 = vsub(w2, w1);
      const float d23_1 = vdot(w2, e23), d23_2 = -vdot(w1, e23);
      const float n123 = vcross(e12, e13);
      const float d123_1 = n123 * vcross(w1, w2), d123_2 = n123 * vcross(w2, w0), d123_3 = n123 * vcross(w0, w1);
      const bool cA = d12_2 <= 0.0f && d13_2 <= 0.0f;
      const bool cB = !cA && d12_1 > 0.0f && d12_2 > 0.0f && d123_3 <= 0.0f;
      const bool cC = !cA && !cB && d13_1 > 0.0f && d13_2 > 0.0f && d123_2 <= 0.0f;
      const bool cD = !cA && !cB && !cC && d12_1 <= 0.0f && d23_2 <= 0.0f;
      const bool cE = !cA && !cB && !cC && !cD && d13_1 <= 0.0f && d23_1 <= 0.0f;
      const bool cF = !cA && !cB && !cC && !cD && !cE && d23_1 > 0.0f && d23_2 > 0.0f && d123_1 <= 0.0f;
      const bool cG = !cA && !cB && !cC && !cD && !cE && !cF;
      const float den = cB ? d12_1 + d12_2 : cC ? d13_1 + d13_2 : cF ? d23_1 + d23_2 : cG ? d123_1 + d123_2 + d123_3 : 1.0f;
      const float inv = fdiv_cr(1.0f, den);
      const V2 n0 = cD ? w1 : (cE || cF) ? w2 : w0;
      const int j0 = cD ? i1 : (cE || cF) ? i2 : i0;
      const float b0 = cB ? d12_1 * inv : cC ? d13_1 * inv : cF ? d23_2 * inv : cG ? d123_1 * inv : 1.0f;
      const float b1 = cB ? d12_2 * inv : cC ? d13_2 * inv : cF ? d23_1 * inv : cG ? d123_2 * inv : cD ? 1.0f : a1;
      if (cC) { w1 = w2; i1 = i2; }
      w0 = n0; i0 = j0; a0 = b0; a1 = b1;
      if (cG) a2 = d123_3 * inv;
      else if (cE) a2 = 1.0f;
      else if (cC) a2 = d13_2 * inv;
      else if (cF) a2 = d23_2 * inv;
      count = cG ? 3 : (cB || cC || cF) ? 2 : 1;
    }
    if (count == 3) break;
    V2 d;
    if (count == 1) d = vneg(w0);
    else {
      const V2 e12 = vsub(w1, w0);
      const float sgn = vcross(e12, vneg(w0));
      d = sgn > 0.0f ? vcross_sv(1.0f, e12) : vcross_vs(e12, 1.0f);
    }
    if (vdot(d, d) < FLT_EPS * FLT_EPS) break;
    const int ia = support(pA, rmulT(tA.q, vneg(d)));
    const int ib = support(pB, rmulT(tB.q, d));
    const int ix = ia | (ib << 2);
    const V2 wx = vsub(xmul(tB, pv(pB, ib)), xmul(tA, pv(pA, ia)));
    ++iter;
#ifdef NASCAR_PROFILE
    ++cache.iters;
#endif
    const bool dup = ix == s0 || (saveCount > 1 && ix == s1) || (saveCount > 2 && ix == s2);
    if (dup) break;
    if (count == 1) { w1 = wx; i1 = ix; a1 = 0.0f; } else { w2 = wx; i2 = ix; a2 = 0.0f; }
    ++count;
  }
  V2 wa = zero2(), wb = zero2();
  const V2 wA0 = xmul(tA, pv(pA, i0 & 3)), wB0 = xmul(tB, pv(pB, i0 >> 2));
  if (count == 1) { wa = wA0; wb = wB0; }
  else {
    const V2 wA1 = xmul(tA, pv(pA, i1 & 3)), wB1 = xmul(tB, pv(pB, i1 >> 2));
    if (count == 2) {
      wa = vadd(vmul(a0, wA0), vmul(a1, wA1));
      wb = vadd(vmul(a0, wB0), vmul(a1, wB1));
    } else if (count == 3) {
      const V2 wA2 = xmul(tA, pv(pA, i2 & 3));
      wa = vadd(vadd(vmul(a0, wA0), vmul(a1, wA1)), vmul(a2, wA2));
      wb = wa;
    }
  }
  cache.metric = count == 2 ? vlen(vsub(w0, w1)) : (count == 3 ? vcross(vsub(w1, w0), vsub(w2, w0)) : 0.0f);
  cache.count = count;
  cache.iA0 = i0 & 3; cache.iB0 = i0 >> 2; cache.iA1 = i1 & 3; cache.iB1 = i1 >> 2; cache.iA2 = i2 & 3; cache.iB2 = i2 >> 2;
  return vlen(vsub(wa, wb));
}

struct Sweep { V2 c0, c; float a0, a, alpha0; };
__device__ __forceinline__ Xf sweep_xf(const Sweep& s, float beta) {
  Xf xf;
// ... 124 lines not shown
      if (s1 < target - tolerance) { *state = TOI_FAILED; out_t = t1; done = true; break; }
      if (s1 <= target + tolerance) { *state = TOI_TOUCHING; out_t = t1; done = true; break; }
      int rootIterCount = 0;
      float a1 = t1, a2 = t2;
      for (;;) {
        float t;
        if (rootIterCount & 1) t = a1 + fdiv_cr((target - s1) * (a2 - a1), s2 - s1);
        else t = 0.5f * (a1 + a2);
        ++rootIterCount;
#ifdef NASCAR_PROFILE
        if (prof_iters) ++prof_iters[1];
#endif
        const Xf xa = sweep_xf(sA, t), xb = sweep_xf_static(sB, t, qB);
        float s = sep_eval(fcn, pA, pB, indexA, indexB, xa, xb);
        if (fabsf(s - target) < tolerance) { t2 = t; xfA2 = xa; xfB2 = xb; break; }
        if (s > target) { a1 = t; s1 = s; } else { a2 = t; s2 = s; }
        if (rootIterCount == 50) break;
      }
      ++pushBackIter;
      if (pushBackIter == 8) break;
    }
    ++iter;
#ifdef NASCAR_PROFILE
    if (prof_iters) ++prof_iters[0];
    if (prof_cyc) prof_cyc[1] += __builtin_amdgcn_s_memtime() - ts0;
#endif
    if (done) break;
    if (iter == 20) { *state = TOI_FAILED; out_t = t1; break; }
  }
#ifdef NASCAR_PROFILE
  if (prof_iters) prof_iters[2] += cache.iters;
#endif
  return out_t;
}

template <int NMAX>
__device__ __forceinline__ void island_solve_toi_buf(Car& c, const LWall* W, const int* cidx, int n, float subdt, float friction,
                                                     VC* vc) {
  BodyState A; A.c = c.c; A.a = c.a; A.v = c.v; A.w = c.w;
  {
  CTIME_BEGIN();
  cs_init<NMAX>(vc, n, c, cidx, W, false, 1.0f);
  CTIME_END(c, 34);
  }
  RotCache rcA; rcA.bits = __float_as_uint(c.a) ^ 1u; rcA.q.s = 0.0f; rcA.q.c = 1.0f;
  {
  CTIME_BEGIN();
  int it = 0;
  for (; it < 20; ++it) { if (cs_solve_position<NMAX>(vc, n, A, 1, rcA)) break; }
  CCOUNT(c, 19, it + 1); CCOUNT(c, 18, n);
  CTIME_END(c, 20);
  }
  c.c0 = A.c; c.a0 = A.a;
  {
  CTIME_BEGIN();
  cs_init_velocity<NMAX>(vc, n, c, A);
  CTIME_END(c, 35);
  }
  {
  CTIME_BEGIN();
  SOLVER_ITER_LOOP
  for (int it = 0; it < 6; ++it) cs_solve_velocity<NMAX>(vc, n, A, friction);
  CTIME_END(c, 36);
  }
  CTIME_BEGIN();
  integrate_positions(A, subdt);
  c.c = A.c; c.a = A.a; c.v = A.v; c.w = A.w;
  c.xf.q = rot_cached(rcA, c.a); c.xf.p = vsub(c.c, rmul(c.xf.q, zero2()));
  report<NMAX>(c, vc, n);
  CTIME_END(c, 37);
}
template <int NMAX>
__device__ __forceinline__ void island_solve_toi_n(Car& c, const LWall* W, const int* cidx, int n, float subdt, float friction) {
  VC vc[NMAX];
  island_solve_toi_buf<NMAX>(c, W, cidx, n, subdt, friction, vc);
}
__device__ inline void island_solve_toi(Car& c, const LWall* W, const int* cidx, int n, float subdt, float friction) {
  if (n <= 2) island_solve_toi_n<2>(c, W, cidx, n, subdt, friction);
  else wave_lds_one_at_a_time([&](VC* vc) { island_solve_toi_buf<MAX_ISLAND>(c, W, cidx, n, subdt, friction, vc); });
}

#define TOI_CULL_DIST (0.005f + 0.00125f + 0.003f)
__device__ __forceinline__ float toi_gap_bound(V2 u, V2 d, V2 dc, V2 cx, V2 cy, V2 wx, V2 wy, float whx, float why) {
  const float s = vdot(u, d);
  const float gap = fabsf(s) - (CAR_HX * fabsf(vdot(u, cx)) + CAR_HY * fabsf(vdot(u, cy)))
                             - (whx * fabsf(vdot(u, wx)) + why * fabsf(vdot(u, wy)));
  const float away = s >= 0.0f ? vdot(u, dc) : -vdot(u, dc);
  return gap - fmaxb(0.0f, away);
}
__device__ __forceinline__ float toi_gap2(V2 u, V2 d1, V2 d0, V2 cx1, V2 cy1, V2 cx0, V2 cy0, float wext) {
  const float s1 = vdot(u, d1), s0 = vdot(u, d0);
  const float g1 = fabsf(s1) - (CAR_HX * fabsf(vdot(u, cx1)) + CAR_HY * fabsf(vdot(u, cy1))) - wext;
  const float g0 = (s1 >= 0.0f ? s0 : -s0) - (CAR_HX * fabsf(vdot(u, cx0)) + CAR_HY * fabsf(vdot(u, cy0))) - wext;
  return fminb(g0, g1);
}
__device__ __forceinline__ bool toi_far_rot2(const Car& c, const LWall& wl, V2 d1, float da, float) {
  if (!(fabsf(da) <= 0.1f)) return false;
  const float R_CAR = 2.80389f;
  const float d2 = da * da;
  const float cd = 1.0f - 0.5f * d2 + d2 * d2 * (1.0f / 24.0f), sd = da * (1.0f - d2 * (1.0f / 6.0f) + d2 * d2 * (1.0f / 120.0f));
  const float qc = c.xf.q.c, qs = c.xf.q.s;
  const float c0c = qc * cd + qs * sd, c0s = qs * cd - qc * sd;
  const V2 cx1 = V(qc, qs), cy1 = V(-qs, qc), cx0 = V(c0c, c0s), cy0 = V(-c0s, c0c);
  const V2 wx = V(wl.qc, wl.qs), wy = V(-wl.qs, wl.qc);
  const V2 d0 = vsub(c.c0, V(wl.px, wl.py));
  float b = toi_gap2(wx, d1, d0, cx1, cy1, cx0, cy0, wl.hx);
  b = fmaxb(b, toi_gap2(wy, d1, d0, cx1, cy1, cx0, cy0, wl.hy));
  b = fmaxb(b, toi_gap2(cx1, d1, d0, cx1, cy1, cx0, cy0, wl.hx * fabsf(vdot(cx1, wx)) + wl.hy * fabsf(vdot(cx1, wy))));
  b = fmaxb(b, toi_gap2(cy1, d1, d0, cx1, cy1, cx0, cy0, wl.hx * fabsf(vdot(cy1, wx)) + wl.hy * fabsf(vdot(cy1, wy))));
  return b - d2 * (R_CAR * 0.125f) > TOI_CULL_DIST;
}
__device__ __forceinline__ bool toi_far(const Car& c, const Poly* pa, const LWall& wl) {
  (void)pa;
  const float R_CAR = 2.80389f;
  const V2 cx = V(c.xf.q.c, c.xf.q.s), cy = V(-c.xf.q.s, c.xf.q.c);
  const V2 wx = V(wl.qc, wl.qs), wy = V(-wl.qs, wl.qc);
  const V2 d = vsub(c.xf.p, V(wl.px, wl.py)), dc = vsub(c.c, c.c0);
  float b = toi_gap_bound(wx, d, dc, cx, cy, wx, wy, wl.hx, wl.hy);
  b = fmaxb(b, toi_gap_bound(wy, d, dc, cx, cy, wx, wy, wl.hx, wl.hy));
  b = fmaxb(b, toi_gap_bound(cx, d, dc, cx, cy, wx, wy, wl.hx, wl.hy));
  b = fmaxb(b, toi_gap_bound(cy, d, dc, cx, cy, wx, wy, wl.hx, wl.hy));
  const float da = c.a - c.a0;
  if (b - fabsf(da) * R_CAR > TOI_CULL_DIST) return true;
  return toi_far_rot2(c, wl, d, da, b);
}

__device__ __forceinline__ float toi_beta(float4 s0, float4 s1, const LWall& wl, int* state, int* iters = nullptr,
                                          unsigned long long* cyc = nullptr) {
  Poly pa; make_box(&pa, CAR_HX, CAR_HY);
  Poly pb; make_box(&pb, wl.hx, wl.hy);
  Sweep sA; sA.c0 = V(s0.x, s0.y); sA.c = V(s0.z, s0.w); sA.a0 = s1.x; sA.a = s1.y; sA.alpha0 = s1.z;
  Sweep sB; sB.c0 = V(wl.px, wl.py); sB.c = sB.c0; sB.a0 = wl.ang; sB.a = wl.ang; sB.alpha0 = 0.0f;
  Rot qw; qw.s = wl.qs; qw.c = wl.qc;
  return time_of_impact(state, &pa, sA, &pb, sB, 1.0f, qw, __float_as_uint(wl.ang), iters, cyc);
}
__device__ __forceinline__ float toi_alpha(float4 s0, float4 s1, const LWall& wl, int* iters = nullptr,
                                           unsigned long long* cyc = nullptr) {
  int state;
  const float beta = toi_beta(s0, s1, wl, &state, iters, cyc);
  return state == TOI_TOUCHING ? fminb(s1.z + (1.0f - s1.z) * beta, 1.0f) : 1.0f;
}
__device__ __forceinline__ void toi_contact_update(Car& c, int ci, const LWall* W, int moff) {
  if (moff + ci < MANI_JOBCAP) { contact_apply(c, ci, W, g_wave_lds[threadIdx.x >> 6].mani.res[moff + ci]); return; }
  contact_update(c, ci, W);
}
__device__ inline void solve_toi(Car& c, const WallSet& S, float dt, float friction) {
  ToiWaveLDS& L = g_wave_lds[threadIdx.x >> 6].toi;
  const LWall* W = S.W;
  Poly pa; make_box(&pa, CAR_HX, CAR_HY);
  const unsigned long long present = __ballot(1);
  const int prank = rank_in(present), npresent = popc64(present);
  const int lane = (int)__lane_id();
  c.alpha0 = 0.0f;
  for (int i = 0; i < c.nct; ++i) { c.ct[i].flags &= ~(CT_TOI | CT_ISLAND); c.ct[i].toiCount = 0; c.ct[i].toi = 1.0f; }
  bool active = true;
  bool had_event = false;
  for (;;) {
    uint32_t need = 0u;
    if (active && c.awake) {
      for (int i = 0; i < c.nct; ++i) {
        DContact& ct = c.ct[i];
        if (!(ct.flags & CT_ENABLED) || ct.toiCount > MAX_SUBSTEPS || (ct.flags & CT_TOI)) continue;
        if (toi_far(c, &pa, ldg(W + ct.wall))) {
          PCOUNT(13, 1); CCOUNT(c, 3, 1);
          if (had_event) CCOUNT(c, 29, 1);
#ifdef NASCAR_TOI_CULL_CHECK
          if (toi_alpha(make_float4(c.c0.x, c.c0.y, c.c.x, c.c.y), make_float4(c.a0, c.a, c.alpha0, 0.0f),
                        ldg(W + ct.wall)) < 1.0f) PCOUNT(11, 1);
#endif
          ct.toi = 1.0f; ct.flags |= CT_TOI;
          continue;
        }
        need |= 1u << i;
        if (had_event) CCOUNT(c, 27, 1);
      }
    }
    const int m = __popc(need);
    int off = 0, total = 0;
#pragma unroll
    for (int bit = 0; bit < 5; ++bit) {
      const unsigned long long b = __ballot((m >> bit) & 1);
      off += rank_in(b) << bit;
      total += popc64(b) << bit;
    }
    if (m) { L.sw0[lane] = make_float4(c.c0.x, c.c0.y, c.c.x, c.c.y); L.sw1[lane] = make_float4(c.a0, c.a, c.alpha0, 0.0f); }
    CCOUNT(c, 14, 1);
#ifdef NASCAR_PROFILE
    const unsigned long long tj0 = __builtin_amdgcn_s_memtime();
#endif
    for (int r0 = 0; r0 < total; r0 += TOI_JOBCAP) {
      {
        uint32_t nb = need; int k = off;
        while (nb) {
          const int i = __ffs(nb) - 1; nb &= nb - 1;
          if (k >= r0 && k < r0 + TOI_JOBCAP) L.job[k - r0] = make_int2(lane | (i << 8), c.ct[i].wall);
          ++k;
        }
      }
      wave_lds_sync();
      const int cnt = min(TOI_JOBCAP, total - r0);
      for (int j = prank; j < cnt; j += npresent) {
        const int2 jb = L.job[j];
        const int owner = jb.x & 0xFF;
        PCOUNT(12, 1); CCOUNT(c, 2, 1);
#ifdef NASCAR_PROFILE
        int it2[3] = {0, 0, 0}; unsigned long long cy2[2] = {0ull, 0ull};
        L.res[j] = toi_alpha(L.sw0[owner], L.sw1[owner], ldg(W + jb.y), it2, cy2);
        CCOUNT(c, 6, it2[0]); CCOUNT(c, 7, it2[1]); CCOUNT(c, 9, cy2[0]); CCOUNT(c, 10, cy2[1]);
#else
        L.res[j] = toi_alpha(L.sw0[owner], L.sw1[owner], ldg(W + jb.y));
#endif
#if defined(NASCAR_PROFILE) && defined(NASCAR_TOI_CAPTURE)
        if (g_prof) {
          const unsigned long long k = atomicAdd(&g_prof[TCAP_BASE], 1ull);
          if (k < TCAP_MAX) {
            float4* r = (float4*)&g_prof[TCAP_BASE + 8 + k * 8];
            const LWall w = ldg(W + jb.y);
            r[0] = L.sw0[owner]; r[1] = L.sw1[owner];
            r[2] = make_float4(w.px, w.py, w.qs, w.qc); r[3] = make_float4(w.hx, w.hy, w.ang, __int_as_float(w.key));
          }
        }
#endif
      }
      wave_lds_sync();
      {
        uint32_t nb = need; int k = off;
        while (nb) {
          const int i = __ffs(nb) - 1; nb &= nb - 1;
          if (k >= r0 && k < r0 + TOI_JOBCAP) {
            c.ct[i].toi = L.res[k - r0]; c.ct[i].flags |= CT_TOI;
            if (had_event && c.ct[i].toi < 1.0f) CCOUNT(c, 28, 1);
          }
          ++k;
        }
      }
      wave_lds_sync();
    }
#ifdef NASCAR_PROFILE
    CCOUNT(c, 13, __builtin_amdgcn_s_memtime() - tj0);
    const unsigned long long te0 = __builtin_amdgcn_s_memtime();
#endif
#ifdef NASCAR_PROFILE
    const unsigned long long ts3 = __builtin_amdgcn_s_memtime();
#endif
    int minC = -1; float minAlpha = 1.0f;
    bool ev = false;
    V2 bc0 = c.c0, bc = c.c; float ba0 = c.a0, ba = c.a, balpha0 = c.alpha0;
    if (active) {
      for (int i = 0; i < c.nct; ++i) {
        const DContact& ct = c.ct[i];
        if (!(ct.flags & CT_ENABLED) || ct.toiCount > MAX_SUBSTEPS || !(ct.flags & CT_TOI)) continue;
        if (ct.toi < minAlpha) { minC = i; minAlpha = ct.toi; }
      }
      if (minC < 0 || 1.0f - 10.0f * FLT_EPS < minAlpha) {
        active = false;
      } else {
        ev = true;
        PCOUNT(15, 1); CCOUNT(c, 4, 1);
        had_event = true;
        bc0 = c.c0; bc = c.c; ba0 = c.a0; ba = c.a; balpha0 = c.alpha0;
        {
          float beta = fdiv_cr(minAlpha - c.alpha0, 1.0f - c.alpha0);
          c.c0 = vadd(c.c0, vmul(beta, vsub(c.c, c.c0)));
          c.a0 += beta * (c.a - c.a0);
          c.alpha0 = minAlpha;
          c.c = c.c0; c.a = c.a0;
          sync_transform(c);
        }
      }
    }
    int moff = MANI_JOBCAP;
#ifdef NASCAR_PROFILE
    const unsigned long long tm0 = __builtin_amdgcn_s_memtime();
    if (ev) CCOUNT(c, 38, tm0 - ts3);
#endif
    if (__ballot(ev)) {
      ManiWaveLDS& M = g_wave_lds[threadIdx.x >> 6].mani;
      const int mm = ev ? c.nct : 0;
      int off2 = 0, total2 = 0;
#pragma unroll
      for (int bit = 0; bit < 5; ++bit) {
        const unsigned long long b = __ballot((mm >> bit) & 1);
        off2 += rank_in(b) << bit;
        total2 += popc64(b) << bit;
      }
      if (ev) {
        moff = off2;
        M.xf[lane] = make_float4(c.xf.p.x, c.xf.p.y, c.xf.q.s, c.xf.q.c);
        for (int i = 0; i < c.nct && off2 + i < MANI_JOBCAP; ++i) M.job[off2 + i] = make_int2(lane | (i << 8), c.ct[i].wall);
      }
      wave_lds_sync();
      const int cnt = min(MANI_JOBCAP, total2);
      for (int j = prank; j < cnt; j += npresent) {
        const int2 jb = M.job[j];
        const float4 x = M.xf[jb.x & 0xFF];
        Xf xfA; xfA.p = V(x.x, x.y); xfA.q.s = x.z; xfA.q.c = x.w;
        M.res[j] = contact_manifold(xfA, ldg(W + jb.y));
      }
      wave_lds_sync();
    }
#ifdef NASCAR_PROFILE
    if (ev) CCOUNT(c, 32, __builtin_amdgcn_s_memtime() - tm0);
#endif
    if (ev) {
      {
        {
        CTIME_BEGIN();
        toi_contact_update(c, minC, W, moff);
        CTIME_END(c, 12);
        CTIME_END(c, 33);
        }
        c.ct[minC].flags &= ~CT_TOI;
        ++c.ct[minC].toiCount;
        if (!(c.ct[minC].flags & CT_ENABLED) || !(c.ct[minC].flags & CT_TOUCH)) {
          c.ct[minC].flags &= ~CT_ENABLED;
          c.c0 = bc0; c.c = bc; c.a0 = ba0; c.a = ba; c.alpha0 = balpha0;
          sync_transform(c);
        } else {
          set_awake(c);
          int cidx[MAX_ISLAND] = {0, 0, 0, 0, 0, 0, 0, 0}; int n = 0;
          island_push(cidx, n, minC); c.ct[minC].flags |= CT_ISLAND;
          {
          CTIME_BEGIN();
          for (int i = 0; i < c.nct; ++i) {
            if (n == MAX_TOI_CONTACTS) break;
            if (n == MAX_ISLAND) {
              if (!(c.ct[i].flags & CT_ISLAND)) { c.overflow = 2; }
              break;
            }
            if (c.ct[i].flags & CT_ISLAND) continue;
            toi_contact_update(c, i, W, moff);
            if (!(c.ct[i].flags & CT_ENABLED)) continue;
            if (!(c.ct[i].flags & CT_TOUCH)) continue;
            c.ct[i].flags |= CT_ISLAND;
            island_push(cidx, n, i);
          }
          CTIME_END(c, 12);
          }
          float subdt = (1.0f - minAlpha) * dt;
          {
          CTIME_BEGIN();
          island_solve_toi(c, W, cidx, n, subdt, friction);
          CTIME_END(c, 11);
          }
          {
          CTIME_BEGIN();
          sync_fixtures(c);
          for (int i = 0; i < c.nct; ++i) c.ct[i].flags &= ~(CT_TOI | CT_ISLAND);
          CTIME_END(c, 17);
          }
          {
          CTIME_BEGIN();
          find_new_contacts(c, S);
          CTIME_END(c, 16);
          }
        }
      }
    }
    wave_lds_sync();
#ifdef NASCAR_PROFILE
    CCOUNT(c, 15, __builtin_amdgcn_s_memtime() - te0);
#endif
    if (!__any(active)) break;
  }
}

__device__ inline void b2_step(Car& c, const WallSet& S, float dt, float friction) {
  const LWall* W = S.W;
  float inv_dt = dt > 0.0f ? fdiv_cr(1.0f, dt) : 0.0f;
  float dtRatio = c.invdt0 * dt;
#ifdef NASCAR_PROFILE
  const unsigned long long t0 = __builtin_amdgcn_s_memtime();
  CCOUNT(c, 1, c.nct);
#endif
  {
  CTIME_BEGIN();
  collide(c, S);
  CTIME_END(c, 23);
  }
  PROFB(11);
  solve(c, S, dt, dtRatio, friction);
  PROFB(13);
#ifdef NASCAR_PROFILE
  const unsigned long long t1 = __builtin_amdgcn_s_memtime();
#endif
  solve_toi(c, S, dt, friction);
#ifdef NASCAR_PROFILE
  const unsigned long long t2 = __builtin_amdgcn_s_memtime();
  CCOUNT(c, 0, t2 - t0); (void)t1;
#endif
  c.invdt0 = inv_dt;
  c.force = zero2(); c.torque = 0.0f;
}

__device__ inline void set_transform(Car& c, const WallSet& S, V2 pos, float angle) {
  c.xf.q = rot_set(angle);
  c.xf.p = pos;
  c.c = xmul(c.xf, zero2()); c.a = angle;
  c.c0 = c.c; c.a0 = angle;
  move_proxy(c, c.xf, c.xf);
  find_new_contacts(c, S);
}

}
```

nascargymnasium_amd/csrc/nascar_kernels.hip:

```cpp
#include <hip/hip_runtime.h>
#include <math.h>
#include <stdarg.h>
#include <stdio.h>
#include <stdlib.h>
#include <string.h>

#include <algorithm>
#include <chrono>
#include <thread>
#include <cmath>
#include <string>
#include <memory>
#include <mutex>
#include <unordered_map>
#include <deque>
#include <fcntl.h>
#include <sys/file.h>
#include <sys/stat.h>
#include <unistd.h>
#include <vector>

#include "../../include/nascar.h"
#include "nascar_device.h"
#include "nascar_actor.h"
// ... 434 lines not shown
__device__ inline bool lap_update(const TrackDev& T, const ChordScreen& S, Car& c, double px, double py, double sim) {
  if (c.lt_timing) c.lt_cur = sim - c.lt_start;
  if (c.lt_has_pos) {
    double dx = px - c.lt_px, dy = py - c.lt_py, d = sqrt(dx * dx + dy * dy);
    if (d < 50.0) c.lt_dist += d;
  }
  bool done = false;
  const bool now = T.startline >= 0 && on_startline_screened(T, S, px, py);
  if (T.startline >= 0 && c.lt_has_pos) {
    const bool before = (c.lt_has_pos & 2) != 0;
    if (now && !before) {
      if (c.lt_crossed && c.lt_timing) {
        double minlap = T.total_length > 0 ? T.total_length * 0.95 : 100.0;
        if (c.lt_cur < 10.0) {
        } else if (c.lt_dist < minlap) {
        } else {
          double ct = c.lt_cur;
          c.lt_last = ct; c.lt_has_last = 1;
          if (!c.lt_has_best || ct < c.lt_best) { c.lt_best = ct; c.lt_has_best = 1; }
          c.lt_start = sim; c.lt_cur = 0.0; c.lt_timing = 1;
          c.lt_laps += 1; c.lt_dist = 0.0;
          done = true;
        }
      } else if (!c.lt_crossed) {
        c.lt_crossed = 1; c.lt_timing = 1; c.lt_start = sim; c.lt_cur = 0.0; c.lt_dist = 0.0;
      }
    }
  }
  c.lt_px = px; c.lt_py = py; c.lt_has_pos = now ? 3 : 1;
  return done;
}

__device__ __forceinline__ float atan2_approx(float y, float x) {
  float ax = fabsf(x), ay = fabsf(y);
  float mx = fmaxf(ax, ay), mn = fminf(ax, ay);
  float t = mx > 0.0f ? mn * __builtin_amdgcn_rcpf(mx) : 0.0f;
  float s2 = t * t;
  float r = ((((0.0208351f * s2 - 0.0851330f) * s2 + 0.1801410f) * s2 - 0.3302995f) * s2 + 0.9998660f) * t;
  if (ay > ax) r = 1.57079637f - r;
  if (x < 0.0f) r = 3.14159274f - r;
  return y < 0.0f ? -r : r;
}

__device__ inline bool query_on_wall(const WallSet& S, double px, double py, double radius) {
  const LWall* W = S.W;
  Aabb q; q.lo = V((float)(px - radius), (float)(py - radius)); q.hi = V((float)(px + radius), (float)(py + radius));
  V2 center = V((float)px, (float)py);
  int beg = 0, end = S.nw;
  const uint16_t* list = nullptr;
  if (radius <= (double)S.bp.reach - 0.1 && grid_list(S.bp, 0.5f * (q.lo.x + q.hi.x), 0.5f * (q.lo.y + q.hi.y), beg, end))
    list = S.bp.idx;
  else { beg = 0; end = S.nw; }
  for (int kk = beg; kk < end; ++kk) {
    const int jw = list ? (int)ldg(list + kk) : kk;
    if (!overlap(fat_box(ldg(S.fat + jw)), q)) continue;
    const LWall wl = ldg(W + jw);
    Xf xf = wall_xf(wl);
    Poly p; make_box(&p, wl.hx, wl.hy);
    V2 pl = rmulT(xf.q, vsub(center, xf.p));
    bool inside = true;
    for (int i = 0; i < 4; ++i) { if (vdot(pn(&p, i), vsub(pl, pv(&p, i))) > 0.0f) { inside = false; break; } }
    if (inside) return true;
    for (int i = 0; i < 4; ++i) {
      V2 v = xmul(xf, pv(&p, i));
      double dx = px - (double)v.x, dy = py - (double)v.y;
      if (PH(dx * dx + dy * dy) < radius) return true;
    }
  }
  return false;
}

__device__ inline void car_obs(const Car& c, float* o) {
  double px = c.xf.p.x, py = c.xf.p.y, vx = c.v.x, vy = c.v.y, ang = c.a, av = c.w;
  o[0] = (float)npclip(px / 10000.0, -1, 1); o[1] = (float)npclip(py / 10000.0, -1, 1);
  o[2] = (float)npclip(vx / 111.1, -1, 1); o[3] = (float)npclip(vy / 111.1, -1, 1);
  o[4] = (float)npclip(PH(P2(vx) + P2(vy)) / 111.1, 0, 1);
  o[5] = (float)npclip(ang / PI_D, -1, 1); o[6] = (float)npclip(av / 10.0, -1, 1);
#pragma unroll
  for (int i = 0; i < 4; ++i) {
    o[7 + i] = (float)npclip(c.load[i] / MAX_TYRE_LOAD, 0, 1);
    o[11 + i] = (float)npclip(c.temp[i] / 200.0, 0, 1);
    o[15 + i] = (float)npclip(c.wear[i] / 100.0, 0, 1);
  }
  double ci = c.imp_present ? c.imp : 0.0, imp = 0.0, ca = 0.0;
  if (!(ci < 100.0)) {
    imp = ci;
    if (c.nact > 0) {
      double na = atan2((double)c.act_n[1], (double)c.act_n[0]);
      double a = na - (double)c.a;
      while (a > PI_D) a -= 2 * PI_D;
      while (a < -PI_D) a += 2 * PI_D;
      ca = a;
    }
  }
  o[19] = (float)npclip(imp / 50000.0, 0, 1); o[20] = (float)npclip(ca / PI_D, -1, 1);
  o[21] = (float)npclip(c.cum_impact / 250000.0, 0, 1);
}
#define PM_A_OBS 1
#define PM_A_TERM 2
#define PM_B_OBS 4
__device__ __forceinline__ float4 car_pose(const Car& c, int mode) {
  return make_float4(c.xf.p.x, c.xf.p.y, c.a, __int_as_float(mode));
}
__device__ __forceinline__ void set_pose(const Params& P, size_t k, const Car& c, int mode) {
  P.pose[k] = car_pose(c, mode);
  double s0, c0;
  sincos((double)c.a, &s0, &c0);
  P.pose_cs[k] = make_double2(c0, s0);
}

__device__ inline void car_reset(const Params& P, Car& c, int n, bool fresh, const WallSet& S, const TrackDev& T) {
  V2 p = OV(P.start_x, P.start_y); float a = P.start_angle;
  if (P.car_contact) {
    const int i = n % P.C;
    const Rot q = rot_set(a);
    p = vadd(p, rmul(q, V(-8.0f * (float)(i >> 1), (i & 1) ? -3.0f : 3.0f)));
    if (P.C == 1) p = OV(P.start_x, P.start_y);
  }
  if (fresh) {
    c.xf.q = rot_set(a); c.xf.p = p;
    c.c = xmul(c.xf, zero2()); c.a = a; c.c0 = c.c; c.a0 = a;
    c.v = zero2(); c.w = 0.0f; c.sleep = 0.0f; c.awake = 1; c.invdt0 = 0.0f;
    c.force = zero2(); c.torque = 0.0f; c.alpha0 = 0.0f;
    Poly cp; make_box(&cp, CAR_HX, CAR_HY);
    Aabb ab = poly_aabb(&cp, c.xf);
    V2 r = V(AABB_EXT, AABB_EXT);
    c.fat.lo = vsub(ab.lo, r); c.fat.hi = vadd(ab.hi, r);
    c.nct = 0; c.overflow = 0; c.moved = 1;
    find_new_contacts(c, S);
    c.bank = 0.0;
  } else {
    c.overflow = 0;
    set_transform(c, S, p, c.a);
    set_transform(c, S, c.xf.p, a);
    set_transform(c, S, p, c.a);
    set_transform(c, S, c.xf.p, a);
    c.v = zero2(); c.w = 0.0f;
  }
  c.rpm = 1000.0;
#pragma unroll
  for (int i = 0; i < 4; ++i) { c.temp[i] = 80.0; c.wear[i] = 0.0; c.load[i] = (CAR_MASS * GRAVITY_MS2 * 0.5) / 2.0; }
  c.pvx = c.pvy = 0.0; c.acc_len = 0; c.acc_head = 0; c.lfm = 0.0; c.slip = 0.0;
  c.nact = 0; c.imp_present = 0; c.imp = 0.0;
  c.lt_timing = 0; c.lt_start = 0.0; c.lt_cur = 0.0; c.lt_has_last = c.lt_has_best = 0; c.lt_last = c.lt_best = 0.0;
  c.lt_crossed = 0; c.lt_has_pos = 0; c.lt_px = c.lt_py = 0.0; c.lt_laps = 0; c.lt_dist = 0.0;
  c.disabled = 0; c.just_disabled = 0; c.cum_impact = 0.0; c.stuck_dur = 0.0; c.has_stuck_start = 0;
  c.stuck_sx = c.stuck_sy = 0.0;
  c.prev_px = c.xf.p.x; c.prev_py = c.xf.p.y;
  c.back = c.prev_back = 0.0; c.first_step = 1; c.prev_laps = 0; c.cum_reward = 0.0f; c.cum_reward_info = 0.0f;
  c.prog_hist = track_progress(T, c.xf.p.x, c.xf.p.y);
  c.imp_at_obs = 0.0;
}

extern __shared__ __attribute__((aligned(16))) unsigned char smem[];


#define SENSOR_LPC 4
__device__ __forceinline__ float sensor_value(float best) {
  double hd = best <= 1.0f ? (double)best * 250.0 : 250.0;
  float d32 = (float)hd;
  float v = fdiv_cr(d32, 250.0f);
  return v < 0.0f ? 0.0f : (v > 1.0f ? 1.0f : v);
}

static const double h_ray_cs[16][2] = NASCAR_RAY_CS_INIT;
__device__ __forceinline__ V2 ray_end(const Params& P, double px, double py, double ang, double c0, double s0, int i,
                                      double& dx, double& dy) {
  float fx, fy;
  ray_end_f32(px, py, ang, c0, s0, i, (const double (*)[2])P.ray_cs, dx, dy, fx, fy);
  return V(fx, fy);
}
__device__ __forceinline__ V2 ray_end_k(double px, double py, double ang, double c0, double s0, int i, double2 rk,
                                        double& dx, double& dy) {
  float fx, fy;
  ray_end_f32_k(px, py, ang, c0, s0, i, rk.x, rk.y, dx, dy, fx, fy);
  return V(fx, fy);
}

__device__ __forceinline__ unsigned ray_mask(float rx, float ry, float d, float R, float angf) {
  if (d <= R * 1.0001f + 0.01f) return 0xFFFFu;
  const float K = 2.54647909f;
  const float x = R * __builtin_amdgcn_rcpf(d) * 1.0001f;
  const float half = fminf(x * (1.0f + 0.5708f * x * x), 1.5708f) + 2e-3f;
  float u = (angf - atan2_approx(ry, rx)) * K;
  u = u - 16.0f * floorf(u * 0.0625f);
  const float w = half * K;
  const int lo = (int)ceilf(u - w), hi = (int)floorf(u + w);
  const int cnt = hi - lo + 1;
  if (cnt <= 0) return 0u;
  if (cnt >= 16) return 0xFFFFu;
  const unsigned m = (1u << cnt) - 1u;
  return ((m << (lo & 15)) | (m >> (16 - (lo & 15)))) & 0xFFFFu;
}

__device__ __forceinline__ unsigned seg_ray_mask(float ax, float ay, float bx, float by, float rr, float angf, float& dseg) {
  const float sx = bx - ax, sy = by - ay;
  const float ll = sx * sx + sy * sy;
  float tt = ll > 0.0f ? -(ax * sx + ay * sy) * __builtin_amdgcn_rcpf(ll) : 0.0f;
  tt = fminf(1.0f, fmaxf(0.0f, tt));
  const float qx = ax + tt * sx, qy = ay + tt * sy;
  dseg = __builtin_amdgcn_sqrtf(qx * qx + qy * qy);
  if (dseg <= rr * 1.0001f + 0.05f) return 0xFFFFu;
  const float K = 2.54647909f;
  const float x = rr * __builtin_amdgcn_rcpf(dseg) * 1.0001f;
  const float half = fminf(x * (1.0f + 0.5708f * x * x), 1.5708f) + 2e-3f;
  float ua = (angf - atan2_approx(ay, ax)) * K, ub = (angf - atan2_approx(by, bx)) * K;
  ua = ua - 16.0f * floorf(ua * 0.0625f);
  ub = ub - 16.0f * floorf(ub * 0.0625f);
  if (ub < ua) { const float tmp = ua; ua = ub; ub = tmp; }
  if (ub - ua > 8.0f) { const float tmp = ua + 16.0f; ua = ub; ub = tmp; }
  const float w = half * K;
  const int lo = (int)ceilf(ua - w), hi = (int)floorf(ub + w);
  const int cnt = hi - lo + 1;
  if (cnt <= 0) return 0u;
  if (cnt >= 16) return 0xFFFFu;
  const unsigned m = (1u << cnt) - 1u;
  return ((m << (lo & 15)) | (m >> (16 - (lo & 15)))) & 0xFFFFu;
}

__device__ __forceinline__ float wall_cast(const float4 wa, const float4 wb, V2 p1, float p2x, float p2y, float dx,
                                           float dy, float bi) {
  const float rx = wa.x - p1.x, ry = wa.y - p1.y;
  const float R = wa.z;
  const float tc = rx * dx + ry * dy, perp = fabsf(rx * dy - ry * dx);
  if (perp > R || tc < -R || (tc - R) > 250.0f * bi) return bi;
  Rot q; q.s = wb.x; q.c = wb.y;
  const float hx = wa.w, hy = wb.z;
  if (perp > hx * fabsf(q.c * dy - q.s * dx) + hy * fabsf(q.s * dy + q.c * dx) + 0.02f) return bi;
  const V2 l1 = rmulT(q, V(p1.x - wa.x, p1.y - wa.y));
  const float n0 = l1.y - (-hy);
  const float n1 = hx - l1.x;
  const float n2 = hy - l1.y;
  const float n3 = l1.x - (-hx);
  const V2 l2 = rmulT(q, V(p2x - wa.x, p2y - wa.y));
  const V2 dd = vsub(l2, l1);
  float lower = 0.0f, upper = 1.0f; int index = -1; bool ok = true;
  const float num[4] = {n0, n1, n2, n3};
  const float den[4] = {-dd.y, dd.x, dd.y, -dd.x};
#pragma unroll
  for (int f = 0; f < 4; ++f) {
    const float n = num[f], d = den[f];
    const float q = fdiv_cr(n, d);
    const bool z = d == 0.0f;
    const bool lo = !z && d < 0.0f && n < lower * d;
    const bool up = !z && !lo && d > 0.0f && n < upper * d;
    const bool kill = z && n < 0.0f;
    lower = ok && lo ? q : lower;
    index = ok && lo ? f : index;
    upper = ok && up ? q : upper;
    ok = ok && !kill && !(upper < lower);
  }
  return (ok && index >= 0 && lower < bi) ? lower : bi;
}

#define CAR_RAY_R 2.81f
#define CAR_RAY_CHUNK 4
__device__ __forceinline__ float car_casts(const Params& P, int n, int pass, V2 p1, float p2x, float p2y, float dx, float dy,
                                           float bi) {
  const int C = P.C;
  const int first = (int)((unsigned)n / (unsigned)C) * C, self = n - first;
  const float4* __restrict__ rec = P.pose + (pass == 0 ? (size_t)0 : (size_t)P.N) + first;
  unsigned long long cand = 0ull;
#pragma unroll 1
  for (int j0 = 0; j0 < C; j0 += CAR_RAY_CHUNK) {
    float2 o[CAR_RAY_CHUNK];
#pragma unroll
    for (int u = 0; u < CAR_RAY_CHUNK; ++u) o[u] = *(const float2*)(rec + min(j0 + u, C - 1));
#pragma unroll
    for (int u = 0; u < CAR_RAY_CHUNK; ++u) {
      const int j = j0 + u;
      const float rx = o[u].x - p1.x, ry = o[u].y - p1.y;
      const float tc = rx * dx + ry * dy, perp = fabsf(rx * dy - ry * dx);
      const bool out = perp > CAR_RAY_R || tc < -CAR_RAY_R || (tc - CAR_RAY_R) > 250.0f * bi;
      if (j < C && j != self && !out) cand |= 1ull << (j & 63);
    }
  }
  while (cand) {
    const int j = __builtin_ctzll(cand);
    cand &= cand - 1ull;
    const float4 o = rec[j];
    const Rot q = rot_set(o.z);
    bi = wall_cast(make_float4(o.x, o.y, CAR_RAY_R, CAR_HX), make_float4(q.s, q.c, CAR_HY, 0.0f), p1, p2x, p2y, dx, dy, bi);
  }
  return bi;
}

#define SENSOR_WPE 6
template <int LPC, bool VIS = false>
__global__ void __launch_bounds__(BLOCK) __attribute__((amdgpu_waves_per_eu(SENSOR_WPE))) sensor_kernel(Params P, float* obs,
                                                                                                        float* terminal_obs, int passes) {
  constexpr int CPW = BLOCK / LPC;
  constexpr int RPL = 16 / LPC;
  PROF_B0(P.blk0 * ((SBLOCK + CPW - 1) / CPW));
  PROFS_RT(14);
  PROFS(0);
  __shared__ float s_p2[CPW * 32];
  __shared__ unsigned s_best[CPW * 16];
  float4* swa = (float4*)smem;
  constexpr int SUB = (SBLOCK + CPW - 1) / CPW;
  const int bx = blockIdx.x, b = bx / SUB + P.blk0, sub = bx % SUB;
  const int t = threadIdx.x, lc = t / LPC, r = t - lc * LPC;
  const int C = P.C;
  const int slot = sub * CPW + lc;
  const int el = slot / C, car = slot - el * C;
  const int env = blk_env_of(P, el, b * P.epb + el);
  if (blk_empty(P, b)) return;
  const TrackDev T = P.tracks[blk_track_of(P, b)];
// ... 458 lines not shown
      if (base[j].x >= 0) {
        const int sl = (slot0[j] & ~15) | ((slot0[j] - i) & 15);
        bi = ray_walk<false>(G, sw, base[j].x + sl, h0, p1, e, dx, dy);
      } else {
        bi = ray_fallback(T, p1, e.x, e.y, dx, dy, pa[j].z, i);
      }
      put4(v, q, sensor_value(bi));
      h0 = h1; h1 = h2; h2 = h3; e0 = e1; e1 = e2; e2 = e3;
    }
    float o[4];
    quad_transpose(v, o, r);
    const size_t at = (size_t)n[j] * 38 + 22 + 4 * r;
    *(float2*)(obs + at) = make_float2(o[0], o[1]); *(float2*)(obs + at + 2) = make_float2(o[2], o[3]);
  }
  if (passes & 2) {
#pragma unroll 1
    for (int j = 0; j < NJ; ++j) {
      const int lc = (t >> 2) + CPR * j, el = lc / C, car = lc - el * C;
      const int env = blk_env_of(P, el, blockIdx.x * P.epb + el);
      if (env >= 0 && P.reset_env[env]) ray_lane(P, T, sw, env * C + car, r, obs, nullptr, 2);
    }
  }
}
template <int LPC, int RB = BLOCK, bool GW = false, bool VIS = false>
__global__ void __launch_bounds__(RB) __attribute__((amdgpu_waves_per_eu(RSENSOR_WPE)))
ray_sensor_kernel(Params P, float* obs, float* terminal_obs, int passes, int SUB) {
  constexpr int CPW = RB / LPC;
  const int bx = blockIdx.x, b = bx / SUB + P.blk0, sub = bx % SUB;
  const int t = threadIdx.x, lc = t / LPC, r = t - lc * LPC;
  const int C = P.C;
  const int slot = sub * CPW + lc;
  const int el = slot / C, car = slot - el * C;
  const int env = blk_env_of(P, el, b * P.epb + el);
  if (blk_empty(P, b)) return;
  const TrackDev& T = P.tracks[blk_track_of(P, b)];
  PROF_B0(P.blk0 * SUB);
  PROFR_RT(14); PROFR(0); PROFR_XCC(8);
  if constexpr (GW) {
    PROFR(1);
    if (env < 0) return;
    ray_lane<LPC, true, true, VIS>(P, T, T.swall, env * C + car, r, obs, terminal_obs, passes);
    PROFR(7); PROFR_RT(15);
    return;
  }
  {
    float4* s_w = (float4*)smem;
    const int nw2 = 2 * T.nwall;
    for (int k = t; k < nw2; k += RB) s_w[k] = ldg(T.swall + k);
    __syncthreads();
  }
  PROFR(1);
  if (env < 0) return;
  ray_lane<LPC, false, true, VIS>(P, T, (const float4*)smem, env * C + car, r, obs, terminal_obs, passes);
  PROFR(7); PROFR_RT(15);
}

#define NOISE_P16 9830u
__device__ __forceinline__ void policy_car(int policy, uint64_t seed, int64_t step, int n, const float* obs, double* ctl,
                                           float& a0, float& a1) {
  const uint64_t key = policy_key(seed, step, (size_t)n);
  const float u0 = (float)(mix32(key) >> 8) * (2.0f / 16777216.0f) - 1.0f;
  const float u1 = (float)(mix32(key ^ 0xABCDEF12345ull) >> 8) * (2.0f / 16777216.0f) - 1.0f;
  if (policy == 0) { a0 = u0; a1 = u1; return; }
  const float* o = obs + (size_t)n * 38;
  double* s = ctl + 4 * (size_t)n;
  const float fwd = o[22], spd = o[4];
  float steer = (float)s[1], last = (float)s[2], lim = (float)s[3];
  double tb = s[0];
  if (last >= fwd) lim = fwd;
  if (last < fwd) lim = 1.0f;
  if (spd < lim * 0.95f) tb += 0.1;
  if (spd > lim * 1.05f) tb -= 0.1;
  const float r = o[22 + 15], l = o[22 + 1];
  if (r > l) steer = 1.0f - (l / r);
  else if (l > r) steer = (1.0f - (r / l)) * -1.0f;
  else steer *= 0.9f;
  if (fabsf(steer) > 0.25f) tb *= 0.5;
  tb = tb > 1.0 ? 1.0 : tb;  tb = tb < -1.0 ? -1.0 : tb;
  steer = steer > 1.0f ? 1.0f : steer;  steer = steer < -1.0f ? -1.0f : steer;
  s[0] = tb; s[1] = steer; s[2] = fwd; s[3] = lim;
  if (policy == 3 && (mix32(key ^ 0x5DEECE66Dull) >> 16) < NOISE_P16) { a0 = u0; a1 = u1; }
  else { a0 = (float)tb; a1 = steer; }
}
__global__ void policy_kernel(int N, int policy, uint64_t seed, int64_t step, const float* obs, float* act, double* ctl) {
  const int n = blockIdx.x * blockDim.x + threadIdx.x;
  if (n >= N) return;
  float a0, a1;
  policy_car(policy, seed, step, n, obs, ctl, a0, a1);
  act[2 * n] = a0; act[2 * n + 1] = a1;
}
struct FieldCodes { signed char code[MLP_MAX_CARS]; };
__global__ void field_policy_kernel(int n0, int n1, int C, FieldCodes F, uint64_t seed, int64_t step, const float* obs,
                                    float* act, double* ctl) {
  const int n = n0 + blockIdx.x * blockDim.x + threadIdx.x;
  if (n >= n1) return;
  const int code = F.code[n % C];
  if (code >= 0 || code == NASCAR_CTRL_GENOME) return;
  float a0, a1;
  policy_car(code == NASCAR_CTRL_RULE ? 1 : code == NASCAR_CTRL_UNIFORM ? 0 : 3, seed, step, n, obs, ctl, a0, a1);
  act[2 * n] = a0; act[2 * n + 1] = a1;
}

#include "nascar_replay.h"

struct alignas(16) GenomeRec { double g[12]; unsigned long long py_steer, pad; };
__global__ void __launch_bounds__(256) genome_policy_kernel(Params P, int slot0, int nslot, int n0, int n1, uint64_t slots,
                                                            const float* obs, float* act, double* ctl, GenomeRec* rec) {
  const int i = blockIdx.x * 256 + threadIdx.x, C = P.C;
  int n;
  if (slot0 < 0) {
    n = n0 + i;
    if (n >= n1) return;
  } else {
    const int sl = i / C, car = i - sl * C, s = slot0 + sl;
    if (sl >= nslot || blk_empty(P, s / P.epb)) return;
    const int env = blk_env_of(P, 0, s);
    if (env < 0) return;
    n = env * C + car;
  }
  if (!((slots >> (n % C)) & 1)) return;
  const GenomeRec G = ldg(rec + n);
  const float g0 = (float)G.g[0], g1 = (float)G.g[1], g4 = (float)G.g[4], g6 = (float)G.g[6], g7 = (float)G.g[7],
              g10 = (float)G.g[10];
  const float* o = obs + (size_t)n * 38;
  double* s = ctl + 4 * (size_t)n;
  const float fwd = o[22], spd = o[4];
  const float last = (float)s[2];
  float lim = (float)s[3];
  double tb = s[0], st = s[1];
  if (last >= fwd) lim = fwd * g10;
  if (last < fwd) lim = 1.0f;
  if (spd < lim * g0) tb += G.g[2];
  if (spd > lim * g1) tb -= G.g[3];
  const float r = o[22 + 15], l = o[22 + 1];
  const bool was_py = G.py_steer != 0;
  bool py = false;
  if (r > l) st = (double)((1.0f - (l / r)) * g4);
  else if (l > r) st = (double)(((1.0f - (r / l)) * -1.0f) * g4);
  else if (was_py) { st = st * G.g[6]; py = true; }
  else st = (double)((float)st * g6);
  if (py ? fabs(st) > G.g[7] : fabsf((float)st) > g7) tb *= G.g[5];
  tb = tb > 1.0 ? 1.0 : tb;  tb = tb < -1.0 ? -1.0 : tb;
  if (st > 1.0) { st = 1.0; py = true; }
  if (st < -1.0) { st = -1.0; py = true; }
  s[0] = tb; s[1] = st; s[2] = fwd; s[3] = lim;
  if (py != was_py) rec[n].py_steer = py;
  act[2 * n] = (float)tb; act[2 * n + 1] = (float)st;
}



__device__ __forceinline__ void model_car(const Params& P, Car& c, int n, const TrackDev& T, float tb, float st, int want_term,
                                          bool logic_ahead = false) {
  const WallSet S{T.walls, T.nwall, T.bp, T.sn, T.wfat, P.ct};
  float a0, a1, a2 = st;
  if (tb >= 0) { a0 = tb; a1 = 0.0f; } else { a0 = 0.0f; a1 = -tb; }
  if (c.disabled) { a0 = 0.0f; a1 = 0.0f; a2 = 0.0f; }
  c.thr_in = pymax(0.0, pymin(1.0, (double)a0));
  c.brk_in = pymax(0.0, pymin(1.0, (double)a1));
  c.str_in = pymax(-1.0, pymin(1.0, (double)a2));
  car_update_physics(P, c, n, T);
  car_store_model(P, n, c);
  asm volatile("" ::: "memory");
  PROF(3);
  b2_step(c, S, P.dt_f, P.friction);
  PROF(4);
  if (logic_ahead) car_load_logic(P, n, c);
  if (ct_in_lds(c)) {
    DContact* g = P.ct + (size_t)n * MAXC;
    for (int i = 0; i < c.ct_hw; ++i) g[i] = c.ct[i];
  }
  car_store_body(P, n, c);
  set_pose(P, n, c, PM_A_OBS | (want_term ? PM_A_TERM : 0));
}

#define CT_LDS_STRIDE ((CT_LDS_CAP * sizeof(DContact) / 16) % 2 ? CT_LDS_CAP * sizeof(DContact) : CT_LDS_CAP * sizeof(DContact) + 16)
#define MODEL_CT_LDS_BYTES ((size_t)SBLOCK * CT_LDS_STRIDE)
#define MODEL_WPE 2
__shared__ DSeg g_step_segs[MAX_SEG];
struct SegReg { double prefix; float4 sg; float rll; };
__device__ __forceinline__ void seg_tables(const DSeg& sg, double prefix, SegReg& r) {
  r.prefix = prefix;
  const double dx = sg.ex - sg.sx, dy = sg.ey - sg.sy, ll = dx * dx + dy * dy;
  r.sg = make_float4((float)sg.sx, (float)sg.sy, (float)dx, (float)dy);
  r.rll = ll < 1e-6 ? 0.0f : (float)(1.0 / ll);
}
template <bool FUSED>
__device__ __forceinline__ void model_block(const Params& P, const void* actions, int discrete, int want_term, int policy,
                                            uint64_t seed, int64_t step, const float* pobs, int tid, int env, int n, Car& c,
                                            SegReg& sr) {
  PROF_B0(P.blk0);
  PROF_RT(14);
  PROF_XCC(10);
  PROF(0);
  if (env >= 0) car_load_phys(P, n, c);
  c.pid = n;
  if (env >= 0 && c.nct <= CT_LDS_CAP) {
    DContact* s_ct = (DContact*)(smem + (size_t)tid * CT_LDS_STRIDE);
    for (int i = 0; i < c.nct; ++i) s_ct[i] = c.ct[i];
    c.ct = s_ct;
    c.ct_hw = c.nct;
  }
  float tb = 0.0f, st = 0.0f;
  if (env >= 0 && policy >= 0) {
    policy_car(policy, seed, step, n, pobs, P.ctl, tb, st);
  } else if (env >= 0) {
    if (discrete) {
      int a = ((const int*)actions)[n];
      tb = a == 1 ? 1.0f : (a == 2 ? -1.0f : 0.0f);
      st = a == 3 ? -1.0f : (a == 4 ? 1.0f : 0.0f);
    } else {
      tb = ((const float*)actions)[2 * n]; st = ((const float*)actions)[2 * n + 1];
    }
  }
  TrackDev T = P.tracks[blk_track_of(P, wg_block(P))];
  if (tid < T.nseg) {
    const DSeg sg = ldg(T.segs + tid);
    g_step_segs[tid] = sg;
    if (FUSED) seg_tables(sg, ldg(T.prefix + tid), sr);
  }
  __syncthreads();
  T.segs = g_step_segs;
  PROF(1);
  if (!FUSED && env < 0) return;
  if (env >= 0) {
    PROF(2);
    model_car(P, c, n, T, tb, st, want_term, FUSED);
    PROF(5);
    PROF_RT(15);
  }
}
__global__ void __launch_bounds__(SBLOCK) __attribute__((amdgpu_waves_per_eu(MODEL_WPE))) model_kernel(Params P, const void* actions, int discrete, int want_term,
                                                                                                    int policy, uint64_t seed, int64_t step, const float* pobs) {
  const CarSlot s = car_slot(P, wg_block(P));
  if (blk_empty(P, wg_block(P))) return;
  Car c;
  SegReg sr;
  model_block<false>(P, actions, discrete, want_term, policy, seed, step, pobs, s.tid, s.env, s.n, c, sr);
}

struct LogicLDS {
  int laps_old[SBLOCK], dis_old[SBLOCK], laps_new[SBLOCK], dis_new[SBLOCK], lapdone[SBLOCK];
  int dis_final[SBLOCK], below[SBLOCK], envdone[SBLOCK];
};
struct TrackLDS { DSeg segs[MAX_SEG]; double prefix[MAX_SEG]; float4 sg[MAX_SEG]; float rll[MAX_SEG]; };
__device__ __forceinline__ void stage_track_lds(const TrackDev& T, TrackLDS& TL, int tid) {
  if (tid < T.nseg) {
    const DSeg sg = ldg(T.segs + tid);
    TL.segs[tid] = sg; TL.prefix[tid] = ldg(T.prefix + tid);
    const double dx = sg.ex - sg.sx, dy = sg.ey - sg.sy, ll = dx * dx + dy * dy;
    TL.sg[tid] = make_float4((float)sg.sx, (float)sg.sy, (float)dx, (float)dy);
    TL.rll[tid] = ll < 1e-6 ? 0.0f : (float)(1.0 / ll);
  }
}
__device__ __forceinline__ void logic_load_env(const Params& P, int env, int car, double& sim, int& pend_in, int& reason_in) {
  sim = 0.0; pend_in = 0; reason_in = 0;
  if (env >= 0) {
    if (car == 0) {
      pend_in = P.env_i32[E_PENDING * P.E + env];
      reason_in = P.env_i32[E_REASON * P.E + env] | (P.env_i32[E_CREATED * P.E + env] == 0 ? 0x100 : 0);
    }
    sim = P.env_time[env];
  }
}
__device__ __forceinline__ void logic_load(const Params& P, int env, int car, int n, Car& c, double& sim, int& pend_in,
                                           int& reason_in) {
  if (env >= 0) {
    car_load_body(P, n, c);
    car_load_logic(P, n, c);
    car_reload_tyres(P, n, c);
  }
  logic_load_env(P, env, car, sim, pend_in, reason_in);
}
__device__ __forceinline__ void logic_from_model(const Params& P, int n, Car& c) {
  car_reload_tyres(P, n, c);
  if (P.car_contact) {
    car_load_body(P, n, c);
    return;
  }
  c.just_disabled = 0;
  c.force = zero2(); c.torque = 0.0f; c.c0 = c.c; c.a0 = c.a; c.alpha0 = 0.0f; c.moved = 0;
  c.ct = P.ct + (size_t)n * MAXC; c.act_key = P.act_key + (size_t)n * MAXC; c.act_n = P.act_n + (size_t)n * MAXC * 2;
  c.acc = nullptr;
}
__device__ __forceinline__ void logic_run(const Params& P, const TrackDev& T, const TrackLDS& TL, LogicLDS& L, int tid,
                                          int el, int car, int env, int n, Car& c, double sim, int pend_in, int reason_in,
                                          float* obs, float* reward, uint8_t* car_flags, uint8_t* env_flags, int auto_reset,
                                          float* terminal_obs) {
  const int C = P.C;
  const ChordScreen CS{TL.sg, TL.rll, T.nseg};
  double prog_now = 0.0;
  const int nw = T.nwall;
  const WallSet S{T.walls, nw, T.bp, T.sn, T.wfat};
  bool lapdone = false;
  if (env >= 0) {
    L.dis_old[tid] = c.disabled;
    LPROF(1);
    L.laps_old[tid] = c.lt_laps;
    const uint64_t cand = screen_candidates(CS, c.xf.p.x, c.xf.p.y);
    if (T.has_banking) c.bank = bank_and_progress_screened(T, cand, c.xf.p.x, c.xf.p.y, prog_now);
    else { c.bank = 0.0; prog_now = track_progress_screened(T, cand, c.xf.p.x, c.xf.p.y); }
    if (!c.disabled) {
      double imp = c.imp_present ? c.imp : 0.0;
      if (imp > 50000.0) { c.disabled = 1; c.just_disabled = 1; }
      if (imp > 100.0) c.cum_impact += imp;
      if (c.cum_impact > 250000.0 && !c.disabled) { c.disabled = 1; c.just_disabled = 1; }
      double speed = (double)vlen(c.v);
      if (speed < 0.5) c.stuck_dur = c.stuck_dur + P.dt_d;
      else { c.stuck_dur = 0.0; c.has_stuck_start = 0; }
    }
    lapdone = lap_update(T, CS, c, c.xf.p.x, c.xf.p.y, sim);
    L.laps_new[tid] = c.lt_laps; L.dis_new[tid] = c.disabled; L.lapdone[tid] = lapdone;
  }
  LPROF(2);
  __syncthreads();
  int pend_env = 0;
  if (env >= 0 && car == 0) {
    int pend = pend_in;
    if (P.reset_on_lap) {
      const int b = tid;
      for (int i = 0; i < C; ++i) {
        if (!L.lapdone[b + i]) continue;
        bool any = false, all = true;
        for (int j = 0; j < C; ++j) {
          int dis = j <= i ? L.dis_new[b + j] : L.dis_old[b + j];
          int laps = j <= i ? L.laps_new[b + j] : L.laps_old[b + j];
          if (dis) continue;
          any = true;
          if (laps < 1) all = false;
        }
        if (any && all) pend = 1;
      }
    }
    P.env_i32[E_PENDING * P.E + env] = pend;
    pend_env = pend;
  }
  float o[22];
  float rew = 0.0f;
  if (env >= 0) {
    if (!c.disabled) {
      double speed = (double)vlen(c.v);
      if (speed < 0.5 && c.stuck_dur > 0) {
        double px = c.xf.p.x, py = c.xf.p.y;
        if (!c.has_stuck_start) { c.has_stuck_start = 1; c.stuck_sx = px; c.stuck_sy = py; }
        double dx = px - c.stuck_sx, dy = py - c.stuck_sy;
        double moved = PH(P2(dx) + P2(dy));
        if (c.stuck_dur > 10.0) {
          bool dis = false;
          if (moved < 1.0) dis = true;
          else if (c.stuck_dur > 15.0) dis = true;
          if (dis) { c.disabled = 1; c.just_disabled = 1; }
        }
      } else { c.stuck_dur = 0.0; c.has_stuck_start = 0; }
    }
    LPROF(3);
    car_obs(c, o);
    LPROF(4);
    if (c.disabled && !c.just_disabled) rew = 0.0f;
    else {
      double r = c.just_disabled ? 10.0 : 0.0;
      if (!c.disabled) r -= 0.05;
      if (!c.disabled) { double imp = c.imp_present ? c.imp : 0.0; if (fabs(imp) > 0) r -= 0.5; }
      double px = c.xf.p.x, py = c.xf.p.y;
      double dx = px - c.prev_px, dy = py - c.prev_py;
      r += PH(P2(dx) + P2(dy)) * 0.15;
      c.prev_px = px; c.prev_py = py;
      if (!c.first_step) {
        double prog = prog_now;
        double L = T.total_length, pd = prog - c.prog_hist;
        if (pd > L / 2) pd -= L; else if (pd < -L / 2) pd += L;
        if (pd < 0) {
          c.back += fabs(pd);
          if (c.back > 200.0 && !c.disabled) { c.disabled = 1; c.just_disabled = 1; }
          if (c.back > 25.0) {
            double ce = pymax(0.0, c.back - 25.0), pe = pymax(0.0, c.prev_back - 25.0);
            double nb = ce - pe;
            if (nb > 0) r -= nb * 0.05;
          }
        } else { c.back = 0.0; c.prev_back = 0.0; }
        c.prog_hist = prog;
      } else {
        c.prog_hist = prog_now;
        c.first_step = 0;
      }
      if (c.lt_laps > c.prev_laps) { r += 0.0 * (c.lt_laps - c.prev_laps); c.prev_laps = c.lt_laps; }
      if (!c.disabled) c.prev_back = c.back;
      rew = (float)r;
    }
    L.dis_final[tid] = c.disabled;
    L.below[tid] = (!c.disabled && c.cum_reward < -250.0f) ? 1 : 0;
  }
  LPROF(5);
  __syncthreads();
  if (env >= 0 && car == 0) {
    const double st = sim + P.dt_d;
    P.env_time[env] = st;
    int ndis = 0, active = 0, below = 0, term = 0, trunc = 0, reason = reason_in & 0xFF;
    for (int j0 = 0; j0 < C; j0 += 8) {
#pragma unroll
      for (int u = 0; u < 8; ++u) {
        if (j0 + u >= C) break;
        const int d = L.dis_final[tid + j0 + u], b = L.below[tid + j0 + u];
        ndis += d;
        if (!d) { active++; below += b; }
      }
    }
    if (ndis >= C) { term = 1; reason = 1; }
    else if (active > 0 && below == active) { term = 1; reason = 2; }
    else if (P.reset_on_lap && st > 60.0) { term = 1; reason = 3; }
    else if (st > 180.0) { trunc = 1; reason = 4; }
    if (pend_env) { P.env_i32[E_PENDING * P.E + env] = 0; term = 1; }
    P.env_i32[E_REASON * P.E + env] = reason;
    P.env_i32[E_TERMINATED * P.E + env] = term;
    P.env_i32[E_TRUNCATED * P.E + env] = trunc;
    int done = term | trunc;
    L.envdone[el] = done | ((reason_in & 0x100) ? 2 : 0);
    if (env_flags) env_flags[env] = (uint8_t)((term ? EF_TERMINATED : 0) | (trunc ? EF_TRUNCATED : 0) |
                                              ((auto_reset && done) ? EF_RESET : 0) | ((reason & 7) << 4));
  }
  __syncthreads();
  if (env >= 0) {
    c.imp_at_obs = c.imp_present ? c.imp : 0.0;
    const bool collided = c.imp_at_obs != 0.0;
    c.cum_reward_info = c.cum_reward;
    c.imp = 0.0; c.imp_present = 1;
    c.cum_reward = c.cum_reward + rew;
    uint8_t flags = (uint8_t)((c.disabled ? CF_DISABLED : 0) | (c.just_disabled ? CF_JUST_DISABLED : 0) |
                              (collided ? CF_COLLISION : 0) | (lapdone ? CF_LAP : 0) | (c.overflow ? CF_ERROR : 0));
    c.just_disabled = 0;
    if (P.vhist) {
      const int k = (int)rint((sim + P.dt_d) * 60.0);
      P.vhist[(size_t)(k % VH_RING) * P.N + n] = vlen(c.v);
    }
    reward[n] = rew;
    if (car_flags) car_flags[n] = flags;
// ... 1989 lines not shown
  HIPCHK(hipGetLastError());
  return 0;
}

extern "C" int nascar_set_car_contact(NascarHandle* h, int32_t enable) {
  if (!h) return fail("null argument");
  h->car_contact = enable ? 1 : 0;
  return 0;
}

extern "C" int nascar_set_car_visibility(NascarHandle* h, int32_t enable) {
  if (!h) return fail("null argument");
  h->car_vis = enable ? 1 : 0;
  return 0;
}
extern "C" int nascar_get_car_visibility(NascarHandle* h) { return h ? h->car_vis : -1; }

extern "C" int nascar_set_perf_history(NascarHandle* h, int32_t enable, void* stream) {
  if (!h) return fail("null argument");
  if (!enable) { if (h->d_vhist) { HIPCHK(hipStreamSynchronize((hipStream_t)stream)); hipFree(h->d_vhist); h->d_vhist = nullptr; } return 0; }
  if (h->d_vhist) return 0;
  const size_t bytes = sizeof(float) * (size_t)VH_RING * h->N;
  HIPCHK(hipMalloc(&h->d_vhist, bytes));
  HIPCHK(hipMemsetAsync(h->d_vhist, 0xFF, bytes, (hipStream_t)stream));
  return 0;
}

extern "C" int64_t nascar_state_bytes(NascarHandle* h) { return h ? (int64_t)h->arena_bytes : -1; }
extern "C" int nascar_get_state(NascarHandle* h, void* dst, void* stream) {
  if (!h || !dst) return fail("null argument");
  HIPCHK(hipMemcpyAsync(dst, h->arena, h->arena_bytes, hipMemcpyDeviceToDevice, (hipStream_t)stream));
  return 0;
}
extern "C" int nascar_set_state(NascarHandle* h, const void* src, void* stream) {
  if (!h || !src) return fail("null argument");
  h->pristine = false;
  HIPCHK(hipMemcpyAsync(h->arena, src, h->arena_bytes, hipMemcpyDeviceToDevice, (hipStream_t)stream));
  return 0;
}

extern "C" int nascar_set_genomes(NascarHandle* h, const double* genomes, void* stream) {
  if (!h) return fail("null argument");
  if (!genomes) { h->genome_set = false; return 0; }
  const size_t N = (size_t)h->N;
  for (size_t i = 0; i < N * 12; ++i)
    if (!std::isfinite(genomes[i]))
      return fail("genome of car %zu: gene %zu is not finite (%g)", i / 12, i % 12, genomes[i]);
  DeviceGuard on(h->cfg.device);
  hipError_t e = on.err;
  if (e == hipSuccess && !h->d_genome) e = hipMalloc(&h->d_genome, sizeof(GenomeRec) * N);
  if (e == hipSuccess) e = h->genome_stage.reserve(sizeof(GenomeRec) * N);
  if (e == hipSuccess) {
    GenomeRec* st = (GenomeRec*)h->genome_stage.host;
    for (size_t n = 0; n < N; ++n) {
      memcpy(st[n].g, genomes + 12 * n, sizeof st[n].g);
      st[n].py_steer = 0; st[n].pad = 0;
    }
    e = hipMemcpyAsync(h->d_genome, st, sizeof(GenomeRec) * N, hipMemcpyHostToDevice, (hipStream_t)stream);
  }
  if (e == hipSuccess) e = h->genome_stage.record((hipStream_t)stream);
  if (e == hipSuccess) e = hipMemsetAsync(h->d_ctl, 0, sizeof(double) * 4 * N, (hipStream_t)stream);
  if (e != hipSuccess) return fail("uploading the genome table failed: %s", hipGetErrorString(e));
  h->genome_set = true;
  return 0;
}
extern "C" int nascar_set_fitness(NascarHandle* h, int32_t enable, void* stream) {
  if (!h) return fail("null argument");
  if (!enable) { h->fit_on = false; return 0; }
  const size_t acc_bytes = align256(sizeof(double) * FIT_N * (size_t)h->N), e_bytes = align256((size_t)h->E);
  if (!h->d_fit) {
    HIPCHK(hipMalloc(&h->d_fit, acc_bytes + 2 * e_bytes));
    h->d_fit_ended = (uint8_t*)h->d_fit + acc_bytes;
    h->d_fit_flags = h->d_fit_ended + e_bytes;
  }
  HIPCHK(hipMemsetAsync(h->d_fit, 0, acc_bytes + 2 * e_bytes, (hipStream_t)stream));
  h->fit_on = true;
  return 0;
}
extern "C" int nascar_get_fitness(NascarHandle* h, double* out, void* stream) {
  if (!h || !out) return fail("null argument");
  if (!h->d_fit) return fail("no fitness accumulators: enable them first (nascar_set_fitness)");
  hipLaunchKernelGGL(fitness_read_kernel, dim3((h->N + 255) / 256), dim3(256), 0, (hipStream_t)stream, h->N, h->d_fit, out);
  HIPCHK(hipGetLastError());
  return 0;
}

extern "C" int nascar_policy_actions(NascarHandle* h, int32_t policy, uint64_t seed, int64_t step, const float* obs,
                                     float* actions, void* stream) {
  if (!h || !actions) return fail("null argument");
  if (policy < 0 || policy > 7) return fail("unknown policy %d", policy);
  if (policy >= 1 && !obs) return fail("policy %d needs obs", policy);
  if (policy == 2 || policy >= 4) {
    if (policy_ready(h, policy, obs, actions)) return -1;
    return launch_actions(h, policy, make_params(h), ShardRange{-1, 0, 0, (size_t)h->N}, seed, step, obs, actions, nullptr,
                          (hipStream_t)stream);
  }
  int nb = (h->N + 255) / 256;
  hipLaunchKernelGGL(policy_kernel, dim3(nb), dim3(256), 0, (hipStream_t)stream, h->N, policy, seed, step, obs, actions, h->d_ctl);
  HIPCHK(hipGetLastError());
  return 0;
}

__global__ void sincos_kernel(const float* x, float* s, float* c, int n) {
  int i = blockIdx.x * blockDim.x + threadIdx.x;
  if (i < n) glibc_sincosf(x[i], &s[i], &c[i]);
}

__global__ void f64math_kernel(const double* x, const double* y, double* out, int n, int fn) {
  const int i = blockIdx.x * blockDim.x + threadIdx.x;
  if (i >= n) return;
  const double a = x[i], b = y ? y[i] : 0.0;
  double r;
  switch (fn) {
    case 0: r = exp(-2.0 * a); break;
    case 1: r = atan2(fabs(a), b); break;
    case 2: r = tan(a); break;
    case 3: r = PH(P2(a) + P2(b)); break;
    default: r = P2(a); break;
  }
  out[i] = r;
}

__device__ __forceinline__ LWall debug_wall(const float* w) {
  LWall wl;
  const Rot q = rot_set(w[2]);
  wl.px = w[0]; wl.py = w[1]; wl.qs = q.s; wl.qc = q.c; wl.hx = w[3]; wl.hy = w[4]; wl.ang = w[2]; wl.key = 0;
  return wl;
}
__global__ void __launch_bounds__(128) debug_toi_kernel(const float* cases, int n, float* beta, int32_t* state, int32_t* far) {
  const int i = blockIdx.x * 128 + threadIdx.x;
  if (i >= n) return;
  const float* k = cases + (size_t)i * 12;
  const LWall wl = debug_wall(k + 7);
  int st;
  beta[i] = toi_beta(make_float4(k[0], k[1], k[2], k[3]), make_float4(k[4], k[5], k[6], 0.0f), wl, &st);
  state[i] = st;
  Car c;
  c.c0 = V(k[0], k[1]); c.c = V(k[2], k[3]); c.a0 = k[4]; c.a = k[5]; c.alpha0 = k[6];
  c.xf.p = c.c; c.xf.q = rot_set(c.a);
  Poly pa; make_box(&pa, CAR_HX, CAR_HY);
  far[i] = toi_far(c, &pa, wl) ? 1 : 0;
}
__global__ void __launch_bounds__(128) debug_collide_kernel(const float* cases, int n, float* out) {
  const int i = blockIdx.x * 128 + threadIdx.x;
  if (i >= n) return;
  const float* k = cases + (size_t)i * 8;
  Xf xfA; xfA.p = V(k[0], k[1]); xfA.q = rot_set(k[2]);
  const ManiRes r = contact_manifold(xfA, debug_wall(k + 3));
  float* o = out + (size_t)i * 12;
  o[0] = r.a.x; o[1] = r.a.y; o[2] = r.a.z; o[3] = r.a.w;
  o[4] = r.b.x; o[5] = r.b.y; o[6] = r.b.z; o[7] = r.b.w;
  o[8] = r.c.x; o[9] = r.c.y; o[10] = r.c.z; o[11] = r.c.w;
}
static uint16_t f32_to_bf16_rne(float f) {
  uint32_t u; memcpy(&u, &f, 4);
  if ((u & 0x7F800000u) == 0x7F800000u && (u & 0x007FFFFFu)) return (uint16_t)((u >> 16) | 0x40);
  u += 0x7FFFu + ((u >> 16) & 1u);
  return (uint16_t)(u >> 16);
}

extern "C" int nascar_set_actor(NascarHandle* h, const float* w1, const float* b1, const float* w2, const float* b2,
                                const float* w3, const float* b3, int32_t obs_dim, int32_t hidden, int32_t act_dim) {
  if (!h || !w1 || !b1 || !w2 || !b2 || !w3 || !b3) return fail("null argument");
  if (obs_dim != ACT_OBS || hidden != ACT_H || act_dim != ACT_OUT)
    return fail("actor shape %dx%dx%d unsupported (need 38x256x2: SB3 MlpPolicy net_arch [256, 256])", obs_dim, hidden, act_dim);
  std::vector<uint16_t> w1p((size_t)ACT_H * ACT_K, 0), w2p((size_t)ACT_H * ACT_H);
  for (int o = 0; o < ACT_H; ++o) {
    for (int i = 0; i < ACT_OBS; ++i) w1p[(size_t)o * ACT_K + i] = f32_to_bf16_rne(w1[(size_t)o * ACT_OBS + i]);
    const uint16_t hi = f32_to_bf16_rne(b1[o]);
    const uint32_t hb = (uint32_t)hi << 16;
    float hf; memcpy(&hf, &hb, 4);
    w1p[(size_t)o * ACT_K + ACT_OBS] = hi;
    w1p[(size_t)o * ACT_K + ACT_OBS + 1] = f32_to_bf16_rne(b1[o] - hf);
  }
  for (int o = 0; o < 8; ++o)
    for (int q = 0; q < 8; ++q)
      for (int s = 0; s < 2; ++s)
        for (int r = 0; r < 32; ++r)
          for (int hh = 0; hh < 2; ++hh)
            for (int j = 0; j < 8; ++j) {
              const int row = 32 * o + r, col = 32 * q + 16 * s + 8 * (j >> 2) + 4 * hh + (j & 3);
              w2p[((((size_t)(o * 8 + q) * 2 + s) * 2 + hh) * 32 + r) * 8 + j] = f32_to_bf16_rne(w2[(size_t)row * ACT_H + col]);
            }
  std::vector<uint16_t> w3p((size_t)8 * 2 * 2 * 4 * 8);
  for (int o = 0; o < 8; ++o)
    for (int s = 0; s < 2; ++s)
      for (int hh = 0; hh < 2; ++hh)
        for (int r = 0; r < 4; ++r)
          for (int j = 0; j < 8; ++j) {
            const int col = 32 * o + 16 * s + 8 * (j >> 2) + 4 * hh + (j & 3);
            const float w = w3[(size_t)(r & 1) * ACT_H + col];
            const uint16_t hi = f32_to_bf16_rne(w);
            const uint32_t hb = (uint32_t)hi << 16;
            float hf; memcpy(&hf, &hb, 4);
            w3p[((((size_t)o * 2 + s) * 2 + hh) * 4 + r) * 8 + j] = r < 2 ? hi : f32_to_bf16_rne(w - hf);
          }
  const size_t o_w1 = 0, o_w2 = o_w1 + w1p.size() * 2, o_b2 = o_w2 + w2p.size() * 2,
               o_w3 = o_b2 + ACT_H * 4, o_b3 = o_w3 + w3p.size() * 2, total = o_b3 + 64;
  if (!h->d_actor) HIPCHK(hipMalloc(&h->d_actor, total));
  char* d = (char*)h->d_actor;
  HIPCHK(hipMemcpy(d + o_w1, w1p.data(), w1p.size() * 2, hipMemcpyHostToDevice));
  HIPCHK(hipMemcpy(d + o_w2, w2p.data(), w2p.size() * 2, hipMemcpyHostToDevice));
  HIPCHK(hipMemcpy(d + o_b2, b2, ACT_H * 4, hipMemcpyHostToDevice));
  HIPCHK(hipMemcpy(d + o_w3, w3p.data(), w3p.size() * 2, hipMemcpyHostToDevice));
  HIPCHK(hipMemcpy(d + o_b3, b3, ACT_OUT * 4, hipMemcpyHostToDevice));
  h->actor.w1p = (const bf16x8*)(d + o_w1); h->actor.w2p = (const bf16x8*)(d + o_w2);
  h->actor.b2 = (const float*)(d + o_b2); h->actor.w3p = (const bf16x8*)(d + o_w3); h->actor.b3 = (const float*)(d + o_b3);
  {
    std::vector<float> f((size_t)ACT_OBS * ACT_H + ACT_H + (size_t)ACT_H * ACT_H + ACT_H + 2 * ACT_H + 2);
    float* p = f.data();
    float* w1t = p; p += (size_t)ACT_OBS * ACT_H;
    float* b1c = p; p += ACT_H;
    float* w2t = p; p += (size_t)ACT_H * ACT_H;
    float* b2c = p; p += ACT_H;
    float* w3c = p; p += 2 * ACT_H;
    float* b3c = p;
    for (int o = 0; o < ACT_H; ++o)
      for (int i = 0; i < ACT_OBS; ++i) w1t[(size_t)i * ACT_H + o] = w1[(size_t)o * ACT_OBS + i];
    for (int o = 0; o < ACT_H; ++o)
      for (int i = 0; i < ACT_H; ++i) w2t[(size_t)i * ACT_H + o] = w2[(size_t)o * ACT_H + i];
    memcpy(b1c, b1, 4 * ACT_H); memcpy(b2c, b2, 4 * ACT_H); memcpy(w3c, w3, 8 * ACT_H); memcpy(b3c, b3, 8);
    if (!h->d_actor32) HIPCHK(hipMalloc(&h->d_actor32, f.size() * 4));
    HIPCHK(hipMemcpy(h->d_actor32, f.data(), f.size() * 4, hipMemcpyHostToDevice));
    const float* d32 = (const float*)h->d_actor32;
    h->actor32.w1t = d32 + (w1t - f.data()); h->actor32.b1 = d32 + (b1c - f.data());
    h->actor32.w2t = d32 + (w2t - f.data()); h->actor32.b2 = d32 + (b2c - f.data());
    h->actor32.w3 = d32 + (w3c - f.data()); h->actor32.b3 = d32 + (b3c - f.data());
  }
  return 0;
}

extern "C" int nascar_set_actor_precision(NascarHandle* h, int32_t fp32) {
  if (!h) return fail("null argument");
  if (fp32 != 0 && fp32 != 1) return fail("precision must be 0 (bf16 MFMA) or 1 (fp32)");
  h->actor_fp32 = fp32;
  return 0;
}

static void launch_actor(NascarHandle* h, int n, const float* obs, float* actions, void* stream) {
#ifdef NASCAR_AB_KNOBS
  static const int fp32_valu = getenv("NASCAR_ACTOR_FP32_VALU") != nullptr;
#else
  const int fp32_valu = 0;
#endif
  if (h->actor_fp32 && !fp32_valu) {
    const int tiles = (n + 31) / 32;
    hipLaunchKernelGGL(actor_mfma32_kernel, dim3((tiles + AM_WAVES - 1) / AM_WAVES), dim3(64 * AM_WAVES), 0,
                       (hipStream_t)stream, n, obs, actions, h->actor32);
  } else if (h->actor_fp32) {
    static int cus = 0;
    if (!cus) { int dev = 0; hipGetDevice(&dev); hipDeviceGetAttribute(&cus, hipDeviceAttributeMultiprocessorCount, dev); if (cus <= 0) cus = 256; }
    const int tiles = (n + AF_TILE - 1) / AF_TILE;
    hipLaunchKernelGGL(actor_fp32_kernel, dim3(std::max(1, std::min(tiles, 2 * cus))), dim3(256), 0, (hipStream_t)stream,
                       n, obs, actions, h->actor32);
  } else {
    hipLaunchKernelGGL(actor_kernel, dim3(actor_grid(n)), dim3(64 * ACT_WAVES), 0, (hipStream_t)stream, n, obs, actions, h->actor);
  }
}

extern "C" int nascar_actor_forward(NascarHandle* h, const float* obs, int32_t n, float* actions, void* stream) {
  if (!h || n < 0) return fail("bad argument");
  if (!h->d_actor) return fail("no actor loaded (nascar_set_actor)");
  if (n == 0) return 0;
  if (!obs || !actions) return fail("bad argument");
  if (((uintptr_t)obs | (uintptr_t)actions) & 7) return fail("actor obs/actions must be 8-byte aligned");
  launch_actor(h, n, obs, actions, stream);
  HIPCHK(hipGetLastError());
  return 0;
}

static bool mlp_shape_ok(int h1, int h2) {
#define X(A, B) if (h1 == 32 * (A) && h2 == 32 * (B)) return true;
  MLP_SHAPES(X)
#undef X
  return false;
}
extern "C" int nascar_check_controller(const NascarMlp* m) {
  if (!m) return fail("null argument");
  const bool value = m->act_dim == 1 && m->output == MLP_OUT_VALUE;
  const bool head4 = m->act_dim == 4 && m->output == MLP_OUT_SQUASH_SAMPLE;
  if (m->obs_dim != ACT_OBS || (m->act_dim != ACT_OUT && !value && !head4) || !mlp_shape_ok(m->h1, m->h2))
    return fail("controller shape %d -> %d -> %d -> %d unsupported: need obs 38, 2 actions and hidden layers 256-256, 256-128, "
                "256-32, 128-128, 64-64 or 32-256 (the SB3 checkpoints the reference ships; TD3's [400, 300] is not among them)",
                m->obs_dim, m->h1, m->h2, m->act_dim);
  if (m->activation != MLP_RELU && m->activation != MLP_TANH)
    return fail("controller activation must be 0 (ReLU) or 1 (Tanh), got %d", m->activation);
  if (m->output == MLP_OUT_VALUE && !value) return fail("controller output 3 (value) needs act_dim 1, got %d", m->act_dim);
  if (m->output == MLP_OUT_SQUASH_SAMPLE && !head4)
    return fail("controller output 5 (squashed sample) needs act_dim 4 (w3 rows: mu, then log_std), got %d", m->act_dim);
  if (m->output != MLP_OUT_RAW && m->output != MLP_OUT_CLIP && m->output != MLP_OUT_SQUASH && m->output != MLP_OUT_VALUE &&
      m->output != MLP_OUT_SAMPLE && m->output != MLP_OUT_SQUASH_SAMPLE)
    return fail("controller output must be 0 (raw), 1 (clip), 2 (squash), 3 (value, act_dim 1), 4 (sampled) or 5 (squashed "
                "sample, act_dim 4), got %d", m->output);
  return 0;
}
static int mlp_rows3(int output) { return output == MLP_OUT_SQUASH_SAMPLE ? 4 : 2; }
static size_t mlp_floats(int H1, int H2, int rows3) {
  return (size_t)ACT_OBS * H1 + H1 + (size_t)H1 * H2 + H2 + rows3 * (size_t)H2 + rows3;
}
static void mlp_pack(const NascarMlp* m, float* p) {
  const int H1 = m->h1, H2 = m->h2, A = m->act_dim, R3 = mlp_rows3(m->output);
  float* w1t = p; p += (size_t)ACT_OBS * H1;
  float* b1 = p; p += H1;
  float* w2t = p; p += (size_t)H1 * H2;
  float* b2 = p; p += H2;
  float* w3 = p; p += R3 * (size_t)H2;
// ... 86 lines not shown
  return 0;
}
static int mlp_launch(const MlpDev& K, int n, int ny, hipStream_t s, const MlpLaunch& L, bool explore = false) {
  const dim3 grid(((n + 31) / 32 + AM_WAVES - 1) / AM_WAVES, ny);
#define X(A, B)                                                                                                  \
  if (K.h1 == 32 * (A) && K.h2 == 32 * (B)) {                                                                    \
    if (explore && K.activation == MLP_RELU)                                                                     \
      hipLaunchKernelGGL((mlp_field_kernel<A, B, MLP_RELU, true>), grid, dim3(64 * AM_WAVES), 0, s, L);           \
    else if (explore) hipLaunchKernelGGL((mlp_field_kernel<A, B, MLP_TANH, true>), grid, dim3(64 * AM_WAVES), 0, s, L); \
    else if (K.activation == MLP_RELU) hipLaunchKernelGGL((mlp_field_kernel<A, B, MLP_RELU>), grid, dim3(64 * AM_WAVES), 0, s, L); \
    else hipLaunchKernelGGL((mlp_field_kernel<A, B, MLP_TANH>), grid, dim3(64 * AM_WAVES), 0, s, L);              \
    HIPCHK(hipGetLastError());                                                                                   \
    return 0;                                                                                                    \
  }
  MLP_SHAPES(X)
#undef X
  return fail("no kernel for controller shape %d-%d", K.h1, K.h2);
}
static int launch_field(NascarHandle* h, int env0, int nenv, uint64_t seed, int64_t step, const float* obs, float* act,
                        hipStream_t s) {
  if (nenv <= 0) return 0;
  const int C = h->C;
  bool done[MLP_MAX_CARS] = {};
  bool builtin = false;
  uint64_t genome_slots = 0;
  for (int c = 0; c < C; ++c) {
    if (h->field[c] == NASCAR_CTRL_GENOME) { genome_slots |= 1ull << c; continue; }
    if (h->field[c] < 0) { builtin = true; continue; }
    if (done[c]) continue;
    const MlpDev& K = h->ctrl[h->field[c]];
    MlpLaunch L{};
    L.table = h->d_ctrl; L.obs = obs; L.act = act; L.env0 = env0; L.nenv = nenv; L.C = C;
    int ns = 0;
    for (int d = c; d < C; ++d) {
      if (h->field[d] < 0 || done[d]) continue;
      const MlpDev& D = h->ctrl[h->field[d]];
      if (D.h1 != K.h1 || D.h2 != K.h2 || D.activation != K.activation) continue;
      L.slot_id[ns++] = d | (h->field[d] << 8);
      done[d] = true;
    }
    if (mlp_launch(K, nenv, ns, s, L)) return -1;
  }
  const int n0 = env0 * C, n1 = (env0 + nenv) * C;
  if (genome_slots) {
    if (!h->genome_set) return fail("a genome slot of the field needs a genome table (nascar_set_genomes)");
    if (launch_genome(h, make_params(h), -1, 0, n0, n1, genome_slots, obs, act, s)) return -1;
  }
  if (builtin) {
    FieldCodes F{};
    for (int c = 0; c < C; ++c) F.code[c] = (signed char)std::max(h->field[c], NASCAR_CTRL_GENOME);
    hipLaunchKernelGGL(field_policy_kernel, dim3((n1 - n0 + 255) / 256), dim3(256), 0, s, n0, n1, C, F, seed, step, obs, act,
                       h->d_ctl);
    HIPCHK(hipGetLastError());
  }
  return 0;
}
static int launch_ac(NascarHandle* h, int what, int c0, int n, uint64_t seed, int64_t step, const float* obs, float* act,
                     float* actions, float* logp, float* values, const uint8_t* tflags, hipStream_t s) {
  if (n <= 0) return 0;
  const MlpDev& PI = h->ctrl[h->ac_pi];
  const MlpDev& VF = h->ctrl[h->ac_vf];
  MlpLaunch L{};
  L.table = h->d_ctrl; L.obs = obs; L.act = act; L.env0 = c0; L.nenv = n; L.C = 1;
  L.values = values; L.actions = actions; L.logp = logp; L.tflags = tflags; L.tcars = h->C;
  L.log_std[0] = h->ac_log_std[0]; L.log_std[1] = h->ac_log_std[1]; L.seed = seed; L.step = step;
  const bool both = (what & AC_SAMPLE) && (what & AC_VALUE);
  const bool shared = PI.h1 == VF.h1 && PI.h2 == VF.h2 && PI.activation == VF.activation;
  if (both && shared) {
    L.slot_id[0] = h->ac_pi << 8; L.slot_id[1] = h->ac_vf << 8;
    return mlp_launch(PI, n, 2, s, L);
  }
  if (what & AC_SAMPLE) {
    L.slot_id[0] = h->ac_pi << 8;
    if (mlp_launch(PI, n, 1, s, L)) return -1;
  }
  if (what & AC_VALUE) {
    L.slot_id[0] = h->ac_vf << 8;
    if (mlp_launch(VF, n, 1, s, L)) return -1;
  }
  return 0;
}
static int launch_explorer(NascarHandle* h, int c0, int n, uint64_t seed, int64_t step, const float* obs, float* act,
                           float* s_out, hipStream_t s) {
  if (n <= 0) return 0;
  const MlpDev& K = h->ctrl[h->ex_id];
  MlpLaunch L{};
  L.table = h->d_ctrl; L.obs = obs; L.act = act; L.env0 = c0; L.nenv = n; L.C = 1;
  L.actions = s_out; L.log_std[0] = h->ex_sigma[0]; L.log_std[1] = h->ex_sigma[1]; L.seed = seed; L.step = step;
  L.slot_id[0] = h->ex_id << 8;
  return mlp_launch(K, n, 1, s, L, true);
}
extern "C" int nascar_set_explorer(NascarHandle* h, int32_t id, const float* sigma) {
  if (!h) return fail("null argument");
  if (id < 0) { h->ex_id = -1; return 0; }
  if (id >= (int)h->ctrl.size()) return fail("explorer: unknown controller id %d (%d loaded with nascar_add_controller)", id, (int)h->ctrl.size());
  const int out = h->ctrl[id].output;
  if (out != MLP_OUT_SQUASH_SAMPLE && out != MLP_OUT_SQUASH)
    return fail("explorer: controller %d has output %d; need 5 (the sampled SAC actor) or 2 (squash, with a noise sigma)", id, out);
  if (out == MLP_OUT_SQUASH_SAMPLE && sigma)
    return fail("explorer: controller %d is a sampled SAC actor (output 5): it takes no noise sigma (pass NULL)", id);
  float s0 = 0.0f, s1 = 0.0f;
  if (sigma) { s0 = sigma[0]; s1 = sigma[1]; }
  if (!std::isfinite(s0) || !std::isfinite(s1) || s0 < 0.0f || s1 < 0.0f)
    return fail("explorer: sigma (%g, %g) must be finite and >= 0", s0, s1);
  h->ex_id = id; h->ex_sigma[0] = s0; h->ex_sigma[1] = s1;
  return 0;
}
extern "C" int nascar_controller_forward(NascarHandle* h, int32_t id, const float* obs, int32_t n, float* actions,
                                         void* stream) {
  if (!h || n < 0) return fail("bad argument");
  if (id < 0 || id >= (int)h->ctrl.size()) return fail("unknown controller id %d (%d loaded)", id, (int)h->ctrl.size());
  if (h->ctrl[id].output >= MLP_OUT_VALUE)
    return fail("controller %d is a critic or a sampled actor: it runs as policy 6 (nascar_set_actor_critic) or 7 "
                "(nascar_set_explorer)", id);
  if (n == 0) return 0;
  if (!obs || !actions) return fail("bad argument");
  if ((uintptr_t)actions & 7) return fail("controller actions must be 8-byte aligned");
  const MlpDev& K = h->ctrl[id];
  MlpLaunch L{};
  L.table = h->d_ctrl; L.obs = obs; L.act = actions; L.env0 = 0; L.nenv = n; L.C = 1;
  L.slot_id[0] = id << 8;
  return mlp_launch(K, n, 1, (hipStream_t)stream, L);
}

extern "C" int nascar_debug_sincosf(const float* x, float* s, float* c, int32_t n, void* stream) {
  if (!x || !s || !c || n < 0) return fail("bad argument");
  hipLaunchKernelGGL(sincos_kernel, dim3((n + 255) / 256), dim3(256), 0, (hipStream_t)stream, x, s, c, n);
  HIPCHK(hipGetLastError());
  return 0;
}
extern "C" int nascar_debug_f64math(const double* x, const double* y, double* out, int32_t n, int32_t fn, void* stream) {
  if (!x || !out || n < 0) return fail("null argument");
  if (fn < 0 || fn > 4) return fail("unknown function %d", fn);
  if ((fn == 1 || fn == 3) && !y) return fail("function %d needs y", fn);
  if (n == 0) return 0;
  hipLaunchKernelGGL(f64math_kernel, dim3((n + 255) / 256), dim3(256), 0, (hipStream_t)stream, x, y, out, n, fn);
  HIPCHK(hipGetLastError());
  return 0;
}
extern "C" int nascar_debug_toi(const float* cases, int32_t n, float* beta, int32_t* state, int32_t* far, void* stream) {
  if (!cases || !beta || !state || !far || n < 0) return fail("bad argument");
  if (n == 0) return 0;
  hipLaunchKernelGGL(debug_toi_kernel, dim3((n + 127) / 128), dim3(128), 0, (hipStream_t)stream, cases, n, beta, state, far);
  HIPCHK(hipGetLastError());
  return 0;
}
extern "C" int nascar_debug_collide(const float* cases, int32_t n, float* out, void* stream) {
  if (!cases || !out || n < 0) return fail("bad argument");
  if (n == 0) return 0;
  hipLaunchKernelGGL(debug_collide_kernel, dim3((n + 127) / 128), dim3(128), 0, (hipStream_t)stream, cases, n, out);
  HIPCHK(hipGetLastError());
  return 0;
}
extern "C" int nascar_debug_car_contact(const float* bodies, int32_t num_envs, int32_t num_cars, float* out,
                                        int32_t* env_out, void* stream) {
  if (!bodies || !out || !env_out || num_envs < 0) return fail("bad argument");
  if (num_cars < 1 || num_cars > 64) return fail("num_cars must be in [1, 64]");
  if (num_envs == 0) return 0;
  const int epb = SBLOCK / num_cars;
  hipLaunchKernelGGL(debug_car_contact_kernel, dim3((num_envs + epb - 1) / epb), dim3(SBLOCK), CC_LDS_BYTES,
                     (hipStream_t)stream, bodies, num_envs, num_cars, out, env_out);
  HIPCHK(hipGetLastError());
  return 0;
}

__global__ void debug_pose_kernel(Params P, const float* poses) {
  const int n = blockIdx.x * blockDim.x + threadIdx.x;
  if (n >= P.N) return;
  const float a = poses[3 * n + 2];
  P.pose[n] = make_float4(poses[3 * n], poses[3 * n + 1], a, __int_as_float(PM_A_OBS));
  double s0, c0;
  sincos((double)a, &s0, &c0);
  P.pose_cs[n] = make_double2(c0, s0);
}
extern "C" int nascar_debug_sensors(NascarHandle* h, const float* poses, float* obs, int32_t impl, void* stream) {
  if (!h || !poses || !obs) return fail("null argument");
  if (prepare(h, (hipStream_t)stream)) return -1;
  Params P = make_params(h);
  hipLaunchKernelGGL(debug_pose_kernel, dim3((h->N + 255) / 256), dim3(256), 0, (hipStream_t)stream, P, poses);
  HIPCHK(hipGetLastError());
  launch_sensors_impl(h, P, h->nblocks, obs, nullptr, 1, stream, impl);
  HIPCHK(hipGetLastError());
  return 0;
}

extern "C" int nascar_debug_block_map(NascarHandle* h, int32_t* blk_track, int32_t* blk_env, int32_t cap_blocks,
                                      void* stream) {
  if (!h || !blk_track || !blk_env) return fail("null argument");
  if (prepare(h, (hipStream_t)stream)) return -1;
  if (cap_blocks < h->nblocks) return fail("block map needs %d workgroups, buffer holds %d", h->nblocks, cap_blocks);
  HIPCHK(hipMemcpyAsync(blk_track, h->d_blk_track, sizeof(int) * h->nblocks, hipMemcpyDeviceToDevice, (hipStream_t)stream));
  HIPCHK(hipMemcpyAsync(blk_env, h->d_blk_env, sizeof(int) * (size_t)h->nblocks * h->epb, hipMemcpyDeviceToDevice,
                        (hipStream_t)stream));
  return h->nblocks;
}

#ifdef NASCAR_PROFILE
extern "C" int nascar_debug_profile(unsigned long long* dev_buf) {
  HIPCHK(hipMemcpyToSymbol(HIP_SYMBOL(g_prof), &dev_buf, sizeof(dev_buf)));
  return 0;
}
#endif
#ifdef NASCAR_DEBUG
extern "C" int nascar_debug_tap(double* dev_buf, int32_t car) {
  HIPCHK(hipMemcpyToSymbol(HIP_SYMBOL(g_dbg), &dev_buf, sizeof(dev_buf)));
  HIPCHK(hipMemcpyToSymbol(HIP_SYMBOL(g_dbg_car), &car, sizeof(car)));
  return 0;
}
#endif
```

Measured before the change: 687.1 million car-steps/s.

## Use explicit LDS/global address-space accessors for per-car contact records

Replaces the generic contact pointer (`c.ct`, which could point into LDS or global memory and was tested with is_shared) with an explicit mode flag (`ct_hw`) and typed accessors. Each access now compiles to either an LDS access or a global access instead of a flat load/store. Field-level helpers read or write only the words needed (wall, flags, toi pair, impulses), and the velocity-constraint setup rebuilds the manifold from cached values instead of rereading the whole record. The aim is to remove flat-address overhead and full 80-byte record copies in the contact solver. In exchange, every access carries a branch on the mode flag, and a debug kernel plus an API entry are added for testing.

```diff
diff --git a/include/nascar.h b/include/nascar.h
--- a/include/nascar.h
+++ b/include/nascar.h
@@ -140,6 +140,9 @@
 int nascar_debug_toi(const float* cases, int32_t n, float* beta, int32_t* state, int32_t* far, void* stream);
 int nascar_debug_collide(const float* cases, int32_t n, float* out, void* stream);
 
+int nascar_debug_contact_ops(const uint32_t* init, const int32_t* nct0, const int32_t* script, int32_t nops,
+                             uint32_t* reads, uint32_t* image, int32_t* nct_out, void* stream);
+
 int nascar_debug_car_contact(const float* bodies, int32_t num_envs, int32_t num_cars, float* out, int32_t* env_out,
                              void* stream);
 
diff --git a/nascargymnasium_amd/_lib.py b/nascargymnasium_amd/_lib.py
--- a/nascargymnasium_amd/_lib.py
+++ b/nascargymnasium_amd/_lib.py
@@ -173,6 +173,8 @@
     L.nascar_debug_toi.restype = ctypes.c_int
     L.nascar_debug_collide.argtypes = [vp, i32, vp, vp]
     L.nascar_debug_collide.restype = ctypes.c_int
+    L.nascar_debug_contact_ops.argtypes = [vp, vp, vp, i32, vp, vp, vp, vp]
+    L.nascar_debug_contact_ops.restype = ctypes.c_int
     L.nascar_debug_car_contact.argtypes = [vp, i32, i32, vp, vp, vp]
     L.nascar_debug_car_contact.restype = ctypes.c_int
     L.nascar_debug_sensors.argtypes = [vp, vp, vp, i32, vp]
@@ -206,7 +208,7 @@
             "nascar_set_genomes", "nascar_set_fitness", "nascar_get_fitness",
             "nascar_update_controller", "nascar_set_actor_critic", "nascar_collect", "nascar_gae",
             "nascar_set_explorer", "nascar_collect_transitions", "nascar_replay_sample",
-            "nascar_debug_sincosf", "nascar_debug_f64math", "nascar_debug_toi", "nascar_debug_collide", "nascar_debug_car_contact", "nascar_debug_sensors", "nascar_track_draw", "nascar_set_random_tracks",
+            "nascar_debug_sincosf", "nascar_debug_f64math", "nascar_debug_toi", "nascar_debug_collide", "nascar_debug_contact_ops", "nascar_debug_car_contact", "nascar_debug_sensors", "nascar_track_draw", "nascar_set_random_tracks",
             "nascar_get_env_tracks", "nascar_vec_post", "nascar_check_actions", "nascar_set_track_cache",
             "nascar_prebuild_track", "nascar_debug_block_map"]
 
diff --git a/nascargymnasium_amd/csrc/nascar_car_io.h b/nascargymnasium_amd/csrc/nascar_car_io.h
--- a/nascargymnasium_amd/csrc/nascar_car_io.h
+++ b/nascargymnasium_amd/csrc/nascar_car_io.h
@@ -67,7 +67,8 @@
 __device__ __forceinline__ void car_init_step(const Params& P, int n, Car& c) {
   c.just_disabled = 0;
   c.force = zero2(); c.torque = 0.0f; c.c0 = c.c; c.a0 = c.a; c.alpha0 = 0.0f; c.moved = 0;
-  c.ct = P.ct + (size_t)n * MAXC; c.act_key = P.act_key + (size_t)n * MAXC; c.act_n = P.act_n + (size_t)n * MAXC * 2;
+  c.ct_g = P.ct + (size_t)n * MAXC; c.ct_hw = CT_NOT_LDS;
+  c.act_key = P.act_key + (size_t)n * MAXC; c.act_n = P.act_n + (size_t)n * MAXC * 2;
   c.acc = nullptr;
 }
 
diff --git a/nascargymnasium_amd/csrc/nascar_device.h b/nascargymnasium_amd/csrc/nascar_device.h
--- a/nascargymnasium_amd/csrc/nascar_device.h
+++ b/nascargymnasium_amd/csrc/nascar_device.h
@@ -241,7 +241,6 @@
   const LWall* W; int nw;
   WallGrid bp, sn;
   const float4* fat;
-  DContact* ct_all = nullptr;
 };
 
 __device__ __forceinline__ bool grid_list(const WallGrid& g, float x, float y, int& beg, int& end) {
@@ -269,7 +268,7 @@
   int disabled, just_disabled, has_stuck_start, first_step, prev_laps;
   double cum_impact, stuck_dur, stuck_sx, stuck_sy, prev_px, prev_py, prog_hist, back, prev_back, imp_at_obs;
   float cum_reward, cum_reward_info;
-  DContact* ct;
+  DContact* ct_g;
   int ct_hw;
   int* act_key;
   float* act_n;
@@ -279,16 +278,124 @@
 #ifndef CT_LDS_CAP
 #define CT_LDS_CAP 4
 #endif
-__device__ __forceinline__ bool ct_in_lds(const Car& c) {
-  return __builtin_amdgcn_is_shared((const __attribute__((address_space(0))) void*)c.ct);
-}
-__device__ __forceinline__ void ct_make_room(Car& c, const WallSet& S) {
-  if (S.ct_all && ct_in_lds(c)) {
+#define CT_NOT_LDS (-1)
+extern __shared__ __attribute__((aligned(16))) unsigned char smem[];
+#define CT_LDS_STRIDE ((CT_LDS_CAP * sizeof(DContact) / 16) % 2 ? CT_LDS_CAP * sizeof(DContact) : CT_LDS_CAP * sizeof(DContact) + 16)
+#define CT_AS1 __attribute__((address_space(1)))
+#define CT_AS3 __attribute__((address_space(3)))
+#define CT_OFF(f) ((int)__builtin_offsetof(DContact, f))
+static_assert(sizeof(DContact) == 80 && CT_OFF(flags) == CT_OFF(wall) + 4 && CT_OFF(toiCount) == CT_OFF(toi) + 4 &&
+              CT_OFF(wall) % 8 == 0 && CT_OFF(toi) % 8 == 0, "contact record layout the accessors rely on");
+__device__ __forceinline__ bool ct_in_lds(const Car& c) { return c.ct_hw >= 0; }
+__device__ __forceinline__ uint32_t ct_laddr(const Car&, int i) {
+  return (uint32_t)(size_t)(CT_AS3 unsigned char*)smem + threadIdx.x * (uint32_t)CT_LDS_STRIDE + (uint32_t)i * (uint32_t)sizeof(DContact);
+}
+__device__ __forceinline__ CT_AS1 unsigned char* ct_gaddr(const Car& c, int i) {
+  return (CT_AS1 unsigned char*)(c.ct_g + i);
+}
+template <typename T> __device__ __forceinline__ T ct_field(const Car& c, int i, int off) {
+  if (ct_in_lds(c)) return *(const CT_AS3 T*)(ct_laddr(c, i) + (uint32_t)off);
+  return *(const CT_AS1 T*)(ct_gaddr(c, i) + off);
+}
+template <typename T> __device__ __forceinline__ void ct_set_field(const Car& c, int i, int off, T v) {
+  if (ct_in_lds(c)) *(CT_AS3 T*)(ct_laddr(c, i) + (uint32_t)off) = v;
+  else *(CT_AS1 T*)(ct_gaddr(c, i) + off) = v;
+}
+struct CtRaw { gu4 v[sizeof(DContact) / 16]; };
+__device__ __forceinline__ CtRaw ct_raw_lds(uint32_t a) {
+  CtRaw r; const CT_AS3 gu4* q = (const CT_AS3 gu4*)a;
+#pragma unroll
+  for (int k = 0; k < (int)(sizeof(DContact) / 16); ++k) r.v[k] = q[k];
+  return r;
+}
+__device__ __forceinline__ CtRaw ct_raw_global(const CT_AS1 unsigned char* a) {
+  CtRaw r; const CT_AS1 gu4* q = (const CT_AS1 gu4*)a;
+#pragma unroll
+  for (int k = 0; k < (int)(sizeof(DContact) / 16); ++k) r.v[k] = q[k];
+  return r;
+}
+__device__ __forceinline__ void ct_raw_to_lds(uint32_t a, const CtRaw& r) {
+  CT_AS3 gu4* q = (CT_AS3 gu4*)a;
+#pragma unroll
+  for (int k = 0; k < (int)(sizeof(DContact) / 16); ++k) q[k] = r.v[k];
+}
+__device__ __forceinline__ void ct_raw_to_global(CT_AS1 unsigned char* a, const CtRaw& r) {
+  CT_AS1 gu4* q = (CT_AS1 gu4*)a;
+#pragma unroll
+  for (int k = 0; k < (int)(sizeof(DContact) / 16); ++k) q[k] = r.v[k];
+}
+__device__ __forceinline__ DContact ct_get(const Car& c, int i) {
+  const CtRaw r = ct_in_lds(c) ? ct_raw_lds(ct_laddr(c, i)) : ct_raw_global(ct_gaddr(c, i));
+  DContact d; __builtin_memcpy(&d, &r, sizeof(DContact));
+  return d;
+}
+__device__ __forceinline__ void ct_put(const Car& c, int i, const DContact& d) {
+  CtRaw r; __builtin_memcpy(&r, &d, sizeof(DContact));
+  if (ct_in_lds(c)) ct_raw_to_lds(ct_laddr(c, i), r); else ct_raw_to_global(ct_gaddr(c, i), r);
+}
+__device__ __forceinline__ void ct_move(const Car& c, int dst, int src) {
+  if (ct_in_lds(c)) ct_raw_to_lds(ct_laddr(c, dst), ct_raw_lds(ct_laddr(c, src)));
+  else ct_raw_to_global(ct_gaddr(c, dst), ct_raw_global(ct_gaddr(c, src)));
+}
+__device__ __forceinline__ int ct_wall(const Car& c, int i) { return ct_field<int>(c, i, CT_OFF(wall)); }
+__device__ __forceinline__ int ct_flags(const Car& c, int i) { return ct_field<int>(c, i, CT_OFF(flags)); }
+__device__ __forceinline__ void ct_set_flags(const Car& c, int i, int fl) { ct_set_field<int>(c, i, CT_OFF(flags), fl); }
+__device__ __forceinline__ int ct_point_count(const Car& c, int i) { return ct_field<int>(c, i, CT_OFF(pointCount)); }
+__device__ __forceinline__ float ct_toi(const Car& c, int i) { return ct_field<float>(c, i, CT_OFF(toi)); }
+__device__ __forceinline__ void ct_set_toi(const Car& c, int i, float toi) { ct_set_field<float>(c, i, CT_OFF(toi), toi); }
+__device__ __forceinline__ int ct_toi_count(const Car& c, int i) { return ct_field<int>(c, i, CT_OFF(toiCount)); }
+__device__ __forceinline__ void ct_set_toi_count(const Car& c, int i, int n) { ct_set_field<int>(c, i, CT_OFF(toiCount), n); }
+__device__ __forceinline__ void ct_set_toi_pair(const Car& c, int i, float toi, int n) {
+  gu2 v; v.x = __float_as_uint(toi); v.y = (uint32_t)n;
+  ct_set_field<gu2>(c, i, CT_OFF(toi), v);
+}
+__device__ __forceinline__ V2 ct_impulse(const Car& c, int i, int j) {
+  const int off = CT_OFF(pt) + j * (int)sizeof(DPoint) + (int)__builtin_offsetof(DPoint, ni);
+  if (ct_in_lds(c)) { const CT_AS3 float* p = (const CT_AS3 float*)(ct_laddr(c, i) + (uint32_t)off); return V(p[0], p[1]); }
+  const CT_AS1 float* p = (const CT_AS1 float*)(ct_gaddr(c, i) + off);
+  return V(p[0], p[1]);
+}
+__device__ __forceinline__ void ct_set_impulse(const Car& c, int i, int j, float ni, float ti) {
+  const int off = CT_OFF(pt) + j * (int)sizeof(DPoint) + (int)__builtin_offsetof(DPoint, ni);
+  if (ct_in_lds(c)) { CT_AS3 float* p = (CT_AS3 float*)(ct_laddr(c, i) + (uint32_t)off); p[0] = ni; p[1] = ti; }
+  else { CT_AS1 float* p = (CT_AS1 float*)(ct_gaddr(c, i) + off); p[0] = ni; p[1] = ti; }
+}
+struct CtHead { int wall, flags; float toi; int toiCount; };
+__device__ __forceinline__ CtHead ct_head(const Car& c, int i) {
+  gu2 a, b;
+  if (ct_in_lds(c)) {
+    const uint32_t p = ct_laddr(c, i);
+    a = *(const CT_AS3 gu2*)(p + (uint32_t)CT_OFF(wall)); b = *(const CT_AS3 gu2*)(p + (uint32_t)CT_OFF(toi));
+  } else {
+    const CT_AS1 unsigned char* p = ct_gaddr(c, i);
+    a = *(const CT_AS1 gu2*)(p + CT_OFF(wall)); b = *(const CT_AS1 gu2*)(p + CT_OFF(toi));
+  }
+  CtHead h; h.wall = (int)a.x; h.flags = (int)a.y; h.toi = __uint_as_float(b.x); h.toiCount = (int)b.y;
+  return h;
+}
+__device__ __forceinline__ void ct_flags_set(const Car& c, int i, int m) {
+  if (ct_in_lds(c)) { CT_AS3 int* p = (CT_AS3 int*)(ct_laddr(c, i) + (uint32_t)CT_OFF(flags)); *p = *p | m; }
+  else { CT_AS1 int* p = (CT_AS1 int*)(ct_gaddr(c, i) + CT_OFF(flags)); *p = *p | m; }
+}
+__device__ __forceinline__ void ct_flags_clear(const Car& c, int i, int m) {
+  if (ct_in_lds(c)) { CT_AS3 int* p = (CT_AS3 int*)(ct_laddr(c, i) + (uint32_t)CT_OFF(flags)); *p = *p & ~m; }
+  else { CT_AS1 int* p = (CT_AS1 int*)(ct_gaddr(c, i) + CT_OFF(flags)); *p = *p & ~m; }
+}
+__device__ __forceinline__ void ct_enter_lds(Car& c) {
+  for (int i = 0; i < c.nct; ++i) ct_raw_to_lds(ct_laddr(c, i), ct_raw_global(ct_gaddr(c, i)));
+  c.ct_hw = c.nct;
+}
+__device__ __forceinline__ void ct_lds_to_global(const Car& c, int nrec) {
+  for (int i = 0; i < nrec; ++i) ct_raw_to_global(ct_gaddr(c, i), ct_raw_lds(ct_laddr(c, i)));
+}
+__device__ __forceinline__ void ct_write_back(const Car& c) {
+  if (ct_in_lds(c)) ct_lds_to_global(c, c.ct_hw);
+}
+__device__ __forceinline__ void ct_make_room(Car& c) {
+  if (ct_in_lds(c)) {
     if (c.nct >= CT_LDS_CAP) {
-      DContact* g = S.ct_all + (size_t)c.pid * MAXC;
-      const int nrec = max(c.nct, c.ct_hw);
-      for (int i = 0; i < nrec; ++i) g[i] = c.ct[i];
-      c.ct = g;
+      ct_lds_to_global(c, max(c.nct, c.ct_hw));
+      c.ct_hw = CT_NOT_LDS;
     } else {
       c.ct_hw = max(c.ct_hw, c.nct + 1);
     }
@@ -345,17 +452,17 @@
 
 __device__ inline void add_pair(Car& c, const WallSet& S, int j) {
     bool exists = false;
-    for (int i = 0; i < c.nct; ++i) if (c.ct[i].wall == j) { exists = true; break; }
+    for (int i = 0; i < c.nct; ++i) if (ct_wall(c, i) == j) { exists = true; break; }
     if (exists) return;
     if (c.nct >= MAXC) { c.overflow = 1; return; }
-    ct_make_room(c, S);
-    for (int i = c.nct; i > 0; --i) c.ct[i] = c.ct[i - 1];
+    ct_make_room(c);
+    for (int i = c.nct; i > 0; --i) ct_move(c, i, i - 1);
     DContact z;
     z.wall = j; z.flags = CT_ENABLED; z.mtype = 0; z.pointCount = 0;
     z.lnx = z.lny = z.lpx = z.lpy = 0.0f;
     for (int q = 0; q < 2; ++q) { z.pt[q].lx = z.pt[q].ly = z.pt[q].ni = z.pt[q].ti = 0.0f; z.pt[q].id = 0u; }
     z.toi = 1.0f; z.toiCount = 0;
-    c.ct[0] = z;
+    ct_put(c, 0, z);
     c.nct++;
     set_awake(c);
 }
@@ -390,23 +497,23 @@
     const int j = list ? (int)ldg(list + k) : k;
     if (!overlap(c.fat, fat_box(ldg(S.fat + j)))) continue;
     bool exists = false;
-    for (int i = 0; i < c.nct; ++i) if (c.ct[i].wall == j) { exists = true; break; }
+    for (int i = 0; i < c.nct; ++i) if (ct_wall(c, i) == j) { exists = true; break; }
     if (exists) continue;
     if (c.nct >= MAXC) { c.overflow = 1; continue; }
-    ct_make_room(c, S);
-    for (int i = c.nct; i > 0; --i) c.ct[i] = c.ct[i - 1];
+    ct_make_room(c);
+    for (int i = c.nct; i > 0; --i) ct_move(c, i, i - 1);
     DContact z;
     z.wall = j; z.flags = CT_ENABLED; z.mtype = 0; z.pointCount = 0;
     z.lnx = z.lny = z.lpx = z.lpy = 0.0f;
     for (int q = 0; q < 2; ++q) { z.pt[q].lx = z.pt[q].ly = z.pt[q].ni = z.pt[q].ti = 0.0f; z.pt[q].id = 0u; }
     z.toi = 1.0f; z.toiCount = 0;
-    c.ct[0] = z;
+    ct_put(c, 0, z);
     c.nct++;
     set_awake(c);
   }
 }
 __device__ inline void remove_contact(Car& c, int i) {
-  for (int j = i; j < c.nct - 1; ++j) c.ct[j] = c.ct[j + 1];
+  for (int j = i; j < c.nct - 1; ++j) ct_move(c, j, j + 1);
   c.nct--;
 }
 
@@ -533,7 +640,7 @@
 
 __device__ inline void contact_update(Car& c, int ci, const LWall* W) {
   PCOUNT(14, 1); CCOUNT(c, 5, 1);
-  DContact ct = c.ct[ci];
+  DContact ct = ct_get(c, ci);
   const DContact old = ct;
   ct.flags |= CT_ENABLED;
   bool was = (ct.flags & CT_TOUCH) != 0;
@@ -552,7 +659,7 @@
   }
   if (touching != was) set_awake(c);
   if (touching) ct.flags |= CT_TOUCH; else ct.flags &= ~CT_TOUCH;
-  c.ct[ci] = ct;
+  ct_put(c, ci, ct);
   if (!was && touching) {
     V2 n = zero2(), pts[2];
     world_manifold(ct, c.xf, xfB, &n, pts);
@@ -579,7 +686,7 @@
 }
 __device__ inline void contact_apply(Car& c, int ci, const LWall* W, const ManiRes& r) {
   PCOUNT(14, 1); CCOUNT(c, 5, 1);
-  DContact ct = c.ct[ci];
+  DContact ct = ct_get(c, ci);
   const DContact old = ct;
   ct.flags |= CT_ENABLED;
   bool was = (ct.flags & CT_TOUCH) != 0;
@@ -602,7 +709,7 @@
   }
   if (touching != was) set_awake(c);
   if (touching) ct.flags |= CT_TOUCH; else ct.flags &= ~CT_TOUCH;
-  c.ct[ci] = ct;
+  ct_put(c, ci, ct);
   if (!was && touching) {
     const LWall wl = ldg(W + ct.wall);
     V2 n = zero2(), pts[2];
@@ -647,9 +754,9 @@
   int i = 0;
   while (i < c.nct) {
     if (!c.awake) { ++i; continue; }
-    const int wall = c.ct[i].wall;
+    const int wall = ct_wall(c, i);
     if (!overlap(c.fat, fat_box(ldg(S.fat + wall)))) {
-      bool touching = (c.ct[i].flags & CT_TOUCH) != 0;
+      bool touching = (ct_flags(c, i) & CT_TOUCH) != 0;
       remove_contact(c, i);
       if (touching) lis_end(c, ldg(&W[wall].key));
       continue;
@@ -670,7 +777,7 @@
 #pragma unroll UNROLL_SMALL
   for (int i = 0; i < NMAX; ++i) {
     if (i >= n) break;
-    const DContact& ct = c.ct[cidx[i]];
+    const DContact ct = ct_get(c, cidx[i]);
     VC& v = vc[i];
     v.ci = cidx[i];
     v.pointCount = ct.pointCount;
@@ -684,6 +791,7 @@
       v.p[j].rA = v.p[j].rB = zero2(); v.p[j].nm = v.p[j].tm = v.p[j].vb = 0.0f;
       v.lps[j] = zero2();
     }
+#pragma unroll
     for (int j = 0; j < 2; ++j) {
       if (j >= ct.pointCount) break;
       if (warm) { v.p[j].ni = dtRatio * ct.pt[j].ni; v.p[j].ti = dtRatio * ct.pt[j].ti; }
@@ -700,7 +808,10 @@
   for (int i = 0; i < NMAX; ++i) {
     if (i >= n) break;
     VC& v = vc[i];
-    const DContact& m = c.ct[v.ci];
+    DContact m;
+    m.pointCount = v.pcount; m.mtype = v.type; m.lnx = v.ln.x; m.lny = v.ln.y; m.lpx = v.lp.x; m.lpy = v.lp.y;
+#pragma unroll
+    for (int j = 0; j < 2; ++j) { m.pt[j].lx = v.lps[j].x; m.pt[j].ly = v.lps[j].y; }
     V2 cA = A.c; float aA = A.a; V2 vA = A.v; float wA = A.w;
     V2 cB = v.cB; float aB = v.aB; V2 vB = v.vB; float wB = v.wB;
     Xf xfA, xfB;
@@ -847,9 +958,9 @@
 #pragma unroll UNROLL_SMALL
   for (int i = 0; i < NMAX; ++i) {
     if (i >= n) break;
-    DContact& m = c.ct[vc[i].ci];
+#pragma unroll
     for (int j = 0; j < 2; ++j) {
-      if (j >= vc[i].pointCount) break; m.pt[j].ni = vc[i].p[j].ni; m.pt[j].ti = vc[i].p[j].ti; }
+      if (j >= vc[i].pointCount) break; ct_set_impulse(c, vc[i].ci, j, vc[i].p[j].ni, vc[i].p[j].ti); }
   }
 }
 
@@ -985,7 +1096,7 @@
   if (!c.awake) return;
   int cidx[MAX_ISLAND] = {0, 0, 0, 0, 0, 0, 0, 0}; int n = 0;
   for (int i = 0; i < c.nct; ++i) {
-    int fl = c.ct[i].flags;
+    int fl = ct_flags(c, i);
     if (!(fl & CT_ENABLED) || !(fl & CT_TOUCH)) continue;
     if (n == MAX_ISLAND) { c.overflow = 2; break; }
     island_push(cidx, n, i);
@@ -1416,14 +1527,14 @@
   const int prank = rank_in(present), npresent = popc64(present);
   const int lane = (int)__lane_id();
   c.alpha0 = 0.0f;
-  for (int i = 0; i < c.nct; ++i) { c.ct[i].flags &= ~(CT_TOI | CT_ISLAND); c.ct[i].toiCount = 0; c.ct[i].toi = 1.0f; }
+  for (int i = 0; i < c.nct; ++i) { ct_flags_clear(c, i, CT_TOI | CT_ISLAND); ct_set_toi_pair(c, i, 1.0f, 0); }
   bool active = true;
   bool had_event = false;
   for (;;) {
     uint32_t need = 0u;
     if (active && c.awake) {
       for (int i = 0; i < c.nct; ++i) {
-        DContact& ct = c.ct[i];
+        const CtHead ct = ct_head(c, i);
         if (!(ct.flags & CT_ENABLED) || ct.toiCount > MAX_SUBSTEPS || (ct.flags & CT_TOI)) continue;
         if (toi_far(c, &pa, ldg(W + ct.wall))) {
           PCOUNT(13, 1); CCOUNT(c, 3, 1);
@@ -1432,7 +1543,7 @@
           if (toi_alpha(make_float4(c.c0.x, c.c0.y, c.c.x, c.c.y), make_float4(c.a0, c.a, c.alpha0, 0.0f),
                         ldg(W + ct.wall)) < 1.0f) PCOUNT(11, 1);
 #endif
-          ct.toi = 1.0f; ct.flags |= CT_TOI;
+          ct_set_toi(c, i, 1.0f); ct_set_flags(c, i, ct.flags | CT_TOI);
           continue;
         }
         need |= 1u << i;
@@ -1457,7 +1568,7 @@
         uint32_t nb = need; int k = off;
         while (nb) {
           const int i = __ffs(nb) - 1; nb &= nb - 1;
-          if (k >= r0 && k < r0 + TOI_JOBCAP) L.job[k - r0] = make_int2(lane | (i << 8), c.ct[i].wall);
+          if (k >= r0 && k < r0 + TOI_JOBCAP) L.job[k - r0] = make_int2(lane | (i << 8), ct_wall(c, i));
           ++k;
         }
       }
@@ -1492,8 +1603,9 @@
         while (nb) {
           const int i = __ffs(nb) - 1; nb &= nb - 1;
           if (k >= r0 && k < r0 + TOI_JOBCAP) {
-            c.ct[i].toi = L.res[k - r0]; c.ct[i].flags |= CT_TOI;
-            if (had_event && c.ct[i].toi < 1.0f) CCOUNT(c, 28, 1);
+            const float alpha = L.res[k - r0];
+            ct_set_toi(c, i, alpha); ct_flags_set(c, i, CT_TOI);
+            if (had_event && alpha < 1.0f) CCOUNT(c, 28, 1);
           }
           ++k;
         }
@@ -1512,7 +1624,7 @@
     V2 bc0 = c.c0, bc = c.c; float ba0 = c.a0, ba = c.a, balpha0 = c.alpha0;
     if (active) {
       for (int i = 0; i < c.nct; ++i) {
-        const DContact& ct = c.ct[i];
+        const CtHead ct = ct_head(c, i);
         if (!(ct.flags & CT_ENABLED) || ct.toiCount > MAX_SUBSTEPS || !(ct.flags & CT_TOI)) continue;
         if (ct.toi < minAlpha) { minC = i; minAlpha = ct.toi; }
       }
@@ -1551,7 +1663,7 @@
       if (ev) {
         moff = off2;
         M.xf[lane] = make_float4(c.xf.p.x, c.xf.p.y, c.xf.q.s, c.xf.q.c);
-        for (int i = 0; i < c.nct && off2 + i < MANI_JOBCAP; ++i) M.job[off2 + i] = make_int2(lane | (i << 8), c.ct[i].wall);
+        for (int i = 0; i < c.nct && off2 + i < MANI_JOBCAP; ++i) M.job[off2 + i] = make_int2(lane | (i << 8), ct_wall(c, i));
       }
       wave_lds_sync();
       const int cnt = min(MANI_JOBCAP, total2);
@@ -1574,29 +1686,31 @@
         CTIME_END(c, 12);
         CTIME_END(c, 33);
         }
-        c.ct[minC].flags &= ~CT_TOI;
-        ++c.ct[minC].toiCount;
-        if (!(c.ct[minC].flags & CT_ENABLED) || !(c.ct[minC].flags & CT_TOUCH)) {
-          c.ct[minC].flags &= ~CT_ENABLED;
+        const CtHead hd = ct_head(c, minC);
+        const int fl = hd.flags & ~CT_TOI;
+        ct_set_toi_count(c, minC, hd.toiCount + 1);
+        if (!(fl & CT_ENABLED) || !(fl & CT_TOUCH)) {
+          ct_set_flags(c, minC, fl & ~CT_ENABLED);
           c.c0 = bc0; c.c = bc; c.a0 = ba0; c.a = ba; c.alpha0 = balpha0;
           sync_transform(c);
         } else {
           set_awake(c);
           int cidx[MAX_ISLAND] = {0, 0, 0, 0, 0, 0, 0, 0}; int n = 0;
-          island_push(cidx, n, minC); c.ct[minC].flags |= CT_ISLAND;
+          island_push(cidx, n, minC); ct_set_flags(c, minC, fl | CT_ISLAND);
           {
           CTIME_BEGIN();
           for (int i = 0; i < c.nct; ++i) {
             if (n == MAX_TOI_CONTACTS) break;
             if (n == MAX_ISLAND) {
-              if (!(c.ct[i].flags & CT_ISLAND)) { c.overflow = 2; }
+              if (!(ct_flags(c, i) & CT_ISLAND)) { c.overflow = 2; }
               break;
             }
-            if (c.ct[i].flags & CT_ISLAND) continue;
+            if (ct_flags(c, i) & CT_ISLAND) continue;
             toi_contact_update(c, i, W, moff);
-            if (!(c.ct[i].flags & CT_ENABLED)) continue;
-            if (!(c.ct[i].flags & CT_TOUCH)) continue;
-            c.ct[i].flags |= CT_ISLAND;
+            const int fi = ct_flags(c, i);
+            if (!(fi & CT_ENABLED)) continue;
+            if (!(fi & CT_TOUCH)) continue;
+            ct_set_flags(c, i, fi | CT_ISLAND);
             island_push(cidx, n, i);
           }
           CTIME_END(c, 12);
@@ -1610,7 +1724,7 @@
           {
           CTIME_BEGIN();
           sync_fixtures(c);
-          for (int i = 0; i < c.nct; ++i) c.ct[i].flags &= ~(CT_TOI | CT_ISLAND);
+          for (int i = 0; i < c.nct; ++i) ct_flags_clear(c, i, CT_TOI | CT_ISLAND);
           CTIME_END(c, 17);
           }
           {
diff --git a/nascargymnasium_amd/csrc/nascar_kernels.hip b/nascargymnasium_amd/csrc/nascar_kernels.hip
--- a/nascargymnasium_amd/csrc/nascar_kernels.hip
+++ b/nascargymnasium_amd/csrc/nascar_kernels.hip
@@ -610,7 +610,6 @@
   c.imp_at_obs = 0.0;
 }
 
-extern __shared__ __attribute__((aligned(16))) unsigned char smem[];
 
 
 #define SENSOR_LPC 4
@@ -1375,7 +1374,7 @@
 
 __device__ __forceinline__ void model_car(const Params& P, Car& c, int n, const TrackDev& T, float tb, float st, int want_term,
                                           bool logic_ahead = false) {
-  const WallSet S{T.walls, T.nwall, T.bp, T.sn, T.wfat, P.ct};
+  const WallSet S{T.walls, T.nwall, T.bp, T.sn, T.wfat};
   float a0, a1, a2 = st;
   if (tb >= 0) { a0 = tb; a1 = 0.0f; } else { a0 = 0.0f; a1 = -tb; }
   if (c.disabled) { a0 = 0.0f; a1 = 0.0f; a2 = 0.0f; }
@@ -1389,15 +1388,11 @@
   b2_step(c, S, P.dt_f, P.friction);
   PROF(4);
   if (logic_ahead) car_load_logic(P, n, c);
-  if (ct_in_lds(c)) {
-    DContact* g = P.ct + (size_t)n * MAXC;
-    for (int i = 0; i < c.ct_hw; ++i) g[i] = c.ct[i];
-  }
+  ct_write_back(c);
   car_store_body(P, n, c);
   set_pose(P, n, c, PM_A_OBS | (want_term ? PM_A_TERM : 0));
 }
 
-#define CT_LDS_STRIDE ((CT_LDS_CAP * sizeof(DContact) / 16) % 2 ? CT_LDS_CAP * sizeof(DContact) : CT_LDS_CAP * sizeof(DContact) + 16)
 #define MODEL_CT_LDS_BYTES ((size_t)SBLOCK * CT_LDS_STRIDE)
 #define MODEL_WPE 2
 __shared__ DSeg g_step_segs[MAX_SEG];
@@ -1418,12 +1413,7 @@
   PROF(0);
   if (env >= 0) car_load_phys(P, n, c);
   c.pid = n;
-  if (env >= 0 && c.nct <= CT_LDS_CAP) {
-    DContact* s_ct = (DContact*)(smem + (size_t)tid * CT_LDS_STRIDE);
-    for (int i = 0; i < c.nct; ++i) s_ct[i] = c.ct[i];
-    c.ct = s_ct;
-    c.ct_hw = c.nct;
-  }
+  if (env >= 0 && c.nct <= CT_LDS_CAP) ct_enter_lds(c);
   float tb = 0.0f, st = 0.0f;
   if (env >= 0 && policy >= 0) {
     policy_car(policy, seed, step, n, pobs, P.ctl, tb, st);
@@ -1503,7 +1493,7 @@
   }
   c.just_disabled = 0;
   c.force = zero2(); c.torque = 0.0f; c.c0 = c.c; c.a0 = c.a; c.alpha0 = 0.0f; c.moved = 0;
-  c.ct = P.ct + (size_t)n * MAXC; c.act_key = P.act_key + (size_t)n * MAXC; c.act_n = P.act_n + (size_t)n * MAXC * 2;
+  c.ct_g = P.ct + (size_t)n * MAXC; c.ct_hw = CT_NOT_LDS; c.act_key = P.act_key + (size_t)n * MAXC; c.act_n = P.act_n + (size_t)n * MAXC * 2;
   c.acc = nullptr;
 }
 __device__ __forceinline__ void logic_run(const Params& P, const TrackDev& T, const TrackLDS& TL, LogicLDS& L, int tid,
@@ -3799,6 +3789,79 @@
   o[4] = r.b.x; o[5] = r.b.y; o[6] = r.b.z; o[7] = r.b.w;
   o[8] = r.c.x; o[9] = r.c.y; o[10] = r.c.z; o[11] = r.c.w;
 }
+enum { CTOP_GET, CTOP_PUT, CTOP_READ, CTOP_WRITE, CTOP_FLAG_SET, CTOP_FLAG_CLEAR, CTOP_PREPEND, CTOP_REMOVE, CTOP_HEAD,
+       CTOP_TOI_PAIR, CTOP_MOVE };
+enum { CTF_WALL, CTF_FLAGS, CTF_POINT_COUNT, CTF_TOI, CTF_TOI_COUNT, CTF_IMPULSE0, CTF_IMPULSE1 };
+#define CT_WORDS ((int)(sizeof(DContact) / 4))
+__device__ __forceinline__ DContact debug_record(uint32_t seed) {
+  uint32_t w[CT_WORDS];
+#pragma unroll
+  for (int k = 0; k < CT_WORDS; ++k) w[k] = seed * 2654435761u + (uint32_t)k * 0x9E3779B9u;
+  DContact d; __builtin_memcpy(&d, w, sizeof(DContact));
+  return d;
+}
+__global__ void __launch_bounds__(SBLOCK) debug_contact_ops_kernel(const uint32_t* init, const int32_t* nct0, const int32_t* script,
+                                                                   int nops, uint32_t* reads, uint32_t* image, int32_t* nct_out) {
+  const int lane = threadIdx.x;
+  for (int k = 0; k < MAXC * CT_WORDS; ++k) image[(size_t)lane * MAXC * CT_WORDS + k] = init[(size_t)lane * MAXC * CT_WORDS + k];
+  Car c;
+  c.pid = lane; c.ct_g = (DContact*)image + (size_t)lane * MAXC; c.ct_hw = CT_NOT_LDS;
+  c.nct = min(max(nct0[lane], 0), MAXC);
+  if (c.nct <= CT_LDS_CAP) ct_enter_lds(c);
+  for (int s = 0; s < nops; ++s) {
+    const int32_t* q = script + ((size_t)lane * nops + s) * 4;
+    const int op = q[0], i = q[1]; const uint32_t a = (uint32_t)q[2], b = (uint32_t)q[3];
+    uint32_t* o = reads + ((size_t)lane * nops + s) * CT_WORDS;
+    if (op == CTOP_PREPEND) {
+      if (c.nct >= MAXC) continue;
+      ct_make_room(c);
+      for (int j = c.nct; j > 0; --j) ct_move(c, j, j - 1);
+      ct_put(c, 0, debug_record(a));
+      c.nct++;
+      continue;
+    }
+    if (i < 0 || i >= c.nct) continue;
+    switch (op) {
+      case CTOP_GET: { const DContact d = ct_get(c, i); uint32_t w[CT_WORDS]; __builtin_memcpy(w, &d, sizeof(DContact));
+                       for (int k = 0; k < CT_WORDS; ++k) o[k] = w[k]; break; }
+      case CTOP_PUT: ct_put(c, i, debug_record(a)); break;
+      case CTOP_READ:
+        switch ((int)a) {
+          case CTF_WALL: o[0] = (uint32_t)ct_wall(c, i); break;
+          case CTF_FLAGS: o[0] = (uint32_t)ct_flags(c, i); break;
+          case CTF_POINT_COUNT: o[0] = (uint32_t)ct_point_count(c, i); break;
+          case CTF_TOI: o[0] = __float_as_uint(ct_toi(c, i)); break;
+          case CTF_TOI_COUNT: o[0] = (uint32_t)ct_toi_count(c, i); break;
+          case CTF_IMPULSE0: case CTF_IMPULSE1: { const V2 p = ct_impulse(c, i, (int)a - CTF_IMPULSE0);
+                                                  o[0] = __float_as_uint(p.x); o[1] = __float_as_uint(p.y); break; }
+          default: break;
+        }
+        break;
+      case CTOP_WRITE:
+        switch ((int)a) {
+          case CTF_WALL: ct_set_field<int>(c, i, CT_OFF(wall), (int)b); break;
+          case CTF_FLAGS: ct_set_flags(c, i, (int)b); break;
+          case CTF_POINT_COUNT: ct_set_field<int>(c, i, CT_OFF(pointCount), (int)b); break;
+          case CTF_TOI: ct_set_toi(c, i, __uint_as_float(b)); break;
+          case CTF_TOI_COUNT: ct_set_toi_count(c, i, (int)b); break;
+          case CTF_IMPULSE0: case CTF_IMPULSE1:
+            ct_set_impulse(c, i, (int)a - CTF_IMPULSE0, __uint_as_float(b), __uint_as_float(~b)); break;
+          default: break;
+        }
+        break;
+      case CTOP_FLAG_SET: ct_flags_set(c, i, (int)a); break;
+      case CTOP_FLAG_CLEAR: ct_flags_clear(c, i, (int)a); break;
+      case CTOP_REMOVE: remove_contact(c, i); break;
+      case CTOP_HEAD: { const CtHead h = ct_head(c, i); o[0] = (uint32_t)h.wall; o[1] = (uint32_t)h.flags;
+                        o[2] = __float_as_uint(h.toi); o[3] = (uint32_t)h.toiCount; break; }
+      case CTOP_TOI_PAIR: ct_set_toi_pair(c, i, __uint_as_float(a), (int)b); break;
+      case CTOP_MOVE: if ((int)a >= 0 && (int)a < c.nct) ct_move(c, i, (int)a); break;
+      default: break;
+    }
+  }
+  ct_write_back(c);
+  nct_out[lane] = c.nct;
+}
 static uint16_t f32_to_bf16_rne(float f) {
   uint32_t u; memcpy(&u, &f, 4);
   if ((u & 0x7F800000u) == 0x7F800000u && (u & 0x007FFFFFu)) return (uint16_t)((u >> 16) | 0x40);
@@ -4191,6 +4254,14 @@
   HIPCHK(hipGetLastError());
   return 0;
 }
+extern "C" int nascar_debug_contact_ops(const uint32_t* init, const int32_t* nct0, const int32_t* script, int32_t nops,
+                                        uint32_t* reads, uint32_t* image, int32_t* nct_out, void* stream) {
+  if (!init || !nct0 || !script || !reads || !image || !nct_out || nops < 0) return fail("bad argument");
+  hipLaunchKernelGGL(debug_contact_ops_kernel, dim3(1), dim3(SBLOCK), MODEL_CT_LDS_BYTES, (hipStream_t)stream, init, nct0,
+                     script, nops, reads, image, nct_out);
+  HIPCHK(hipGetLastError());
+  return CT_LDS_CAP;
+}
 extern "C" int nascar_debug_car_contact(const float* bodies, int32_t num_envs, int32_t num_cars, float* out,
                                         int32_t* env_out, void* stream) {
   if (!bodies || !out || !env_out || num_envs < 0) return fail("bad argument");
```

Measured after the change: 686.7 million car-steps/s. About the same (-0.1%).
